# matthiasverstraete/3d_recognizer

Measured on AMD Instinct MI355X. Metric: training clouds/sec, N=40960 pts, bs=8, at 1/2/4/8 GPUs; mIoU parity, higher is better.
Workload: dtype f32 storage/accumulate, bf16x3 MFMA in the wide GEMMs

## Files before the change

### 3d_recognizer_amd/csrc/gemm.hip

```cpp
#include "rl_common.h"
#include <stdlib.h>
#include <string.h>

namespace {

typedef float f32x4 __attribute__((ext_vector_type(4)));

constexpr int GM_BM = 128;
constexpr int GM_BK = 16;
constexpr int GM_AS = 20;

struct AOperand {
    const float* A;
    long lda, a_bstride;
    int a_mode;
    RlLazy lazy;
    const float* xyz;
    long xyz_bstride;
    const int32_t* nbr_idx;
    const float* nbr_d2;
    int nbr_k;
    int n;
    int K;
    long M;
// ... 25 lines not shown
                const int j = a.nbr_idx[R];
                const float* xb = a.xyz + (long)b * a.xyz_bstride * 3;
                const float xi = xb[(long)i * 3 + 0], yi = xb[(long)i * 3 + 1], zi = xb[(long)i * 3 + 2];
                const float xj = xb[(long)j * 3 + 0], yj = xb[(long)j * 3 + 1], zj = xb[(long)j * 3 + 2];
                v[0] = xi; v[1] = yi; v[2] = zi;
                v[3] = xj; v[4] = yj; v[5] = zj;
                v[6] = xi - xj; v[7] = yi - yj; v[8] = zi - zj;
                v[9] = __fsqrt_rn(a.nbr_d2[R]);
            }
            float* dst = As + r * stride;
#pragma unroll
            for (int c = 0; c < 10; ++c) dst[c] = v[c];
            for (int c = 10; c < kw; ++c) dst[c] = 0.f;
        }
        return;
    }
    if (a.vec4) {
        const int qpr = kw >> 2;
        for (int e = tid; e < nrows * qpr; e += 256) {
            const int r = e / qpr, q = e - r * qpr;
            const long R = row0 + r;
            const int kc = k0 + q * 4;
            float4 v = make_float4(0.f, 0.f, 0.f, 0.f);
            if (R < row_limit && kc < a.K) {
                v = *reinterpret_cast<const float4*>(a.A + a_row_offset(a, R) + kc);
                if (a.lazy.scale) {
                    v.x = rl_lazy(a.lazy, v.x, kc + 0);
                    v.y = rl_lazy(a.lazy, v.y, kc + 1);
                    v.z = rl_lazy(a.lazy, v.z, kc + 2);
                    v.w = rl_lazy(a.lazy, v.w, kc + 3);
                }
            }
            *reinterpret_cast<float4*>(As + r * stride + q * 4) = v;
        }
        return;
    }
    for (int e = tid; e < nrows * kw; e += 256) {
        const int r = e / kw, c = e - r * kw;
        const long R = row0 + r;
        const int kc = k0 + c;
        float v = 0.f;
        if (R < row_limit && kc < a.K) v = rl_lazy(a.lazy, a.A[a_row_offset(a, R) + kc], kc);
        As[r * stride + c] = v;
    }
}

struct ConcatSrc {
    const float* A2;
    const int32_t* idx;
    const float* sc2; const float* sh2;
    long a2_bstride;
    int lda2, split, act2;
    float slope2;
};

struct GemmParams {
    AOperand a;
    int N;
    const float* W;
    long w_ks, w_ns;
    const float* bias;
    float* Y;
    long ldy, y_bstride;
    int rows_per_batch;
    int y_contig;
    int accumulate;
    double* stats;
    const float* piv_mean;
    const float* piv_bias;
    int ksplit;
    int kchunk;
    float* kslab;
    int stat_slots;
    int gx, ny;
    const float* addend;
    float* out2;
    const int32_t* out2_index;
    long out2_bstride;
    int split_col;
    const __bf16* wsplit;
    const float* bnb_Y;
    const float* bnb_scale;
    const float* bnb_shift;
    const float* bnb_mean;
    const float* bnb_invstd;
    float bnb_neg;
    int pair_ny1;
    int N2;
    float* Y2;
    double* stats2;
    const float* piv_mean2;
    const float* piv_bias2;
    const __bf16* wsplit2;
};

__device__ __forceinline__ float stat_pivot(const GemmParams& p, int c) {
    if (!p.stats || !p.piv_mean || c >= p.N) return 0.f;
    return p.piv_mean[c] - (p.piv_bias ? p.piv_bias[c] : 0.f);
}

template <int NT>
__global__ __launch_bounds__(256) void gemm_kernel(const GemmParams p) {
    constexpr int BN = 16 * NT;
    constexpr int WS = BN + ((BN % 32 == 0) ? 16 : 0);
    __shared__ __attribute__((aligned(16))) float As[GM_BM * GM_AS];
    __shared__ float Ws[GM_BK * WS];
// ... 254 lines not shown

void wgrad_split(long M, int N, int K, int* nsplit, long* rows_per_block) {
    const int T = wgrad_tile(N, K);
    const int ny = rl_cdiv(N, T), nz = rl_cdiv(K, T);
    long want = 1024 / ((long)ny * nz);
    if (want < 1) want = 1;
    long maxs = (M + 255) / 256;
    const long fill = 256 / ((long)ny * nz) + 1;
    if (maxs < fill) maxs = fill < (M + 63) / 64 ? fill : (M + 63) / 64;
    if (maxs < 1) maxs = 1;
    if (want > maxs) want = maxs;
    if (T == 128) {
        const long round = 512 / ((long)ny * nz);
        if (round >= 1 && want > round) want = round;
    }
    constexpr long share = 2;
    if (T == 128) { want /= share; if (want < 1) want = 1; }
    long rpb = (M + want - 1) / want;
    rpb = ((rpb + 63) / 64) * 64;
    *rows_per_block = rpb;
    *nsplit = (int)((M + rpb - 1) / rpb);
    if (*nsplit < 1) *nsplit = 1;
}

int fill_a(AOperand* a, const char* who, const float* A, long lda, long a_bstride, int a_mode,
           int in_act, float in_slope, const float* in_scale, const float* in_shift,
           const float* xyz, long xyz_bstride, const int32_t* nbr_idx, const float* nbr_d2, int nbr_k,
           int B, int n, int K) {
    RL_REQUIRE(B > 0 && n > 0 && K > 0, RL_ERR_ARGS, "%s: bad sizes B=%d n=%d K=%d", who, B, n, K);
    a->A = A; a->lda = lda; a->a_bstride = a_bstride; a->a_mode = a_mode;
    a->lazy.scale = in_scale; a->lazy.shift = in_shift; a->lazy.act = in_act; a->lazy.slope = in_slope;
    a->xyz = xyz; a->xyz_bstride = xyz_bstride; a->nbr_idx = nbr_idx; a->nbr_d2 = nbr_d2; a->nbr_k = nbr_k;
    a->n = n; a->K = K;
    if (a_mode == 1) {
        RL_REQUIRE(K == 10, RL_ERR_ARGS, "%s: relative position encoding source needs K == 10 (got %d)", who, K);
        RL_REQUIRE(xyz && nbr_idx && nbr_d2 && nbr_k > 0 && xyz_bstride >= n, RL_ERR_ARGS, "%s: incomplete RPE source", who);
        a->M = (long)B * n * nbr_k;
        a->contig = 1; a->vec4 = 0; a->vec4p = 0;
    } else {
        RL_REQUIRE(a_mode == 0, RL_ERR_ARGS, "%s: unknown a_mode %d", who, a_mode);
        RL_REQUIRE(A && lda >= K && a_bstride >= n, RL_ERR_ARGS, "%s: bad A operand", who);
        RL_REQUIRE((in_scale == nullptr) == (in_shift == nullptr), RL_ERR_ARGS, "%s: in_scale/in_shift must come together", who);
        a->M = (long)B * n;
        a->contig = (a_bstride == n);
        a->vec4 = (lda % 4 == 0) && (K % 4 == 0) && (((uintptr_t)A & 15) == 0);
        a->vec4p = (lda % 4 == 0) && ((K + 3) / 4 * 4 <= lda) && (((uintptr_t)A & 15) == 0);
    }
    RL_REQUIRE(a->M < (1l << 31), RL_ERR_ARGS, "%s: too many rows", who);
    return RL_OK;
}



template <int KC, int NT, bool BNB = false>
__global__ __launch_bounds__(256) void sgemm_kernel(const GemmParams p) {
    __shared__ double red[4][2][16 * NT];
    const int tid = threadIdx.x, lane = tid & 63, wave = __builtin_amdgcn_readfirstlane(tid >> 6);
    const int li = lane & 15, lj = lane >> 4;
    const int K = p.a.K, N = p.N;
    const long M = p.a.M;

    float wf[KC][4][NT];
    float sc[KC][4], sh[KC][4];
#pragma unroll
    for (int c = 0; c < KC; ++c)
#pragma unroll
        for (int s = 0; s < 4; ++s) {
            const int k = 16 * c + 4 * lj + s;
            sc[c][s] = (p.a.lazy.scale && k < K) ? p.a.lazy.scale[k] : 1.f;
            sh[c][s] = (p.a.lazy.scale && k < K) ? p.a.lazy.shift[k] : 0.f;
#pragma unroll
            for (int nb = 0; nb < NT; ++nb) {
                const int n = nb * 16 + li;
                wf[c][s][nb] = (k < K && n < N) ? p.W[(long)k * p.w_ks + (long)n * p.w_ns] : 0.f;
            }
        }
    float bias[NT], ssum[NT], ssq[NT], piv[NT];
    float bsc[BNB ? NT : 1], bsh[BNB ? NT : 1], bmu[BNB ? NT : 1], bis[BNB ? NT : 1];
#pragma unroll
    for (int nb = 0; nb < NT; ++nb) {
        const int n = nb * 16 + li;
        bias[nb] = (p.bias && n < N) ? p.bias[n] : 0.f;
        ssum[nb] = ssq[nb] = 0.f;
        piv[nb] = BNB ? 0.f : stat_pivot(p, n);
        if constexpr (BNB) {
            bsc[nb] = n < N ? p.bnb_scale[n] : 1.f; bsh[nb] = n < N ? p.bnb_shift[n] : 0.f;
            bmu[nb] = n < N ? p.bnb_mean[n] : 0.f;  bis[nb] = n < N ? p.bnb_invstd[n] : 0.f;
        }
    }
    const bool lazy = p.a.lazy.scale != nullptr;
    const float es = (!lazy || p.a.lazy.act == RL_ACT_NONE) ? 1.f : (p.a.lazy.act == RL_ACT_RELU ? 0.f : p.a.lazy.slope);
    const bool full = N == 16 * NT;

    const long nblk = (M + 15) >> 4;
    const long bstep = (long)gridDim.x * 4;
    auto fetch = [&](long blk, float4 (&a)[KC]) {
        const long row = blk * 16 + li;
        const bool rvalid = row < M;
        const long aoff = rvalid ? a_row_offset(p.a, row) : 0;
#pragma unroll
        for (int c = 0; c < KC; ++c) {
            a[c] = make_float4(0.f, 0.f, 0.f, 0.f);
            if (rvalid && 16 * c + 4 * lj < K) a[c] = *reinterpret_cast<const float4*>(p.a.A + aoff + 16 * c + 4 * lj);
        }
    };
    float4 a[KC], an[KC];
    long blk = (long)blockIdx.x * 4 + wave;
    if (blk < nblk) fetch(blk, a);
    for (; blk < nblk; blk += bstep) {
        const bool rvalid = blk * 16 + li < M;
        if (blk + bstep < nblk) fetch(blk + bstep, an);
        f32x4 acc[NT];
#pragma unroll
        for (int nb = 0; nb < NT; ++nb) acc[nb] = (f32x4){0.f, 0.f, 0.f, 0.f};
#pragma unroll
        for (int c = 0; c < KC; ++c) {
            float av[4] = {a[c].x, a[c].y, a[c].z, a[c].w};
#pragma unroll
            for (int s = 0; s < 4; ++s) {
                float v = av[s];
                if (lazy) {
                    const float z = v * sc[c][s] + sh[c][s];
                    v = fmaxf(z, z * es);
                }
                if (!rvalid || 16 * c + 4 * lj + s >= K) v = 0.f;
#pragma unroll
                for (int nb = 0; nb < NT; ++nb)
                    acc[nb] = __builtin_amdgcn_mfma_f32_16x16x4f32(v, wf[c][s][nb], acc[nb], 0, 0, 0);
            }
        }
        asm volatile("" ::: "memory");
        __builtin_amdgcn_s_waitcnt(0x0F70);
        asm volatile("" ::: "memory");
#pragma unroll
        for (int r = 0; r < 4; ++r) {
            const long R = blk * 16 + lj * 4 + r;
            if (R < M) {
                long yoff;
                if (p.y_contig) yoff = R * p.ldy;
                else {
                    const int b = (int)((unsigned)R / (unsigned)p.rows_per_batch);
                    const int i = (int)(R - (long)b * p.rows_per_batch);
                    yoff = ((long)b * p.y_bstride + i) * p.ldy;
                }
                float* y = p.Y + yoff + li;
                float v[NT];
#pragma unroll
                for (int nb = 0; nb < NT; ++nb) v[nb] = acc[nb][r] + bias[nb];
                if (p.accumulate) {
                    float o[NT];
#pragma unroll
                    for (int nb = 0; nb < NT; ++nb) o[nb] = (full || nb * 16 + li < N) ? y[nb * 16] : 0.f;
#pragma unroll
                    for (int nb = 0; nb < NT; ++nb) v[nb] += o[nb];
                }
                if constexpr (BNB) {
                    const float* yl = p.bnb_Y + yoff + li;
                    float t[NT];
#pragma unroll
                    for (int nb = 0; nb < NT; ++nb) t[nb] = (full || nb * 16 + li < N) ? yl[nb * 16] : 0.f;
#pragma unroll
                    for (int nb = 0; nb < NT; ++nb) {
                        if (full || nb * 16 + li < N) {
                            y[nb * 16] = v[nb];
                            const float z = t[nb] * bsc[nb] + bsh[nb];
                            const float gp = v[nb] * (z > 0.f ? 1.f : p.bnb_neg);
                            ssum[nb] += gp;
                            ssq[nb] += gp * ((t[nb] - bmu[nb]) * bis[nb]);
                        }
                    }
                } else {
#pragma unroll
                for (int nb = 0; nb < NT; ++nb) {
                    if (full || nb * 16 + li < N) {
                        y[nb * 16] = v[nb];
                        const float dv = v[nb] - piv[nb];
                        ssum[nb] += dv;
                        ssq[nb] += dv * dv;
                    }
                }
                }
            }
        }
#pragma unroll
        for (int c = 0; c < KC; ++c) a[c] = an[c];
    }
    if (p.stats) {
#pragma unroll
        for (int nb = 0; nb < NT; ++nb) {
            float s = ssum[nb], q = ssq[nb];
            s += __shfl_xor(s, 16, 64); s += __shfl_xor(s, 32, 64);
            q += __shfl_xor(q, 16, 64); q += __shfl_xor(q, 32, 64);
            if (lane < 16) {
                red[wave][0][nb * 16 + lane] = (double)s;
                red[wave][1][nb * 16 + lane] = (double)q;
            }
        }
        __syncthreads();
        if (tid < 16 * NT && tid < N) {
            p.stats[((long)blockIdx.x * 2 + 0) * N + tid] = red[0][0][tid] + red[1][0][tid] + red[2][0][tid] + red[3][0][tid];
            p.stats[((long)blockIdx.x * 2 + 1) * N + tid] = red[0][1][tid] + red[1][1][tid] + red[2][1][tid] + red[3][1][tid];
            for (long slot = blockIdx.x + gridDim.x; slot < p.stat_slots; slot += gridDim.x) {
                p.stats[(slot * 2 + 0) * N + tid] = 0.0;
                p.stats[(slot * 2 + 1) * N + tid] = 0.0;
            }
        }
    }
}

constexpr int SW_U = 4;

template <int KT, int NT>
__device__ __forceinline__ void swgrad_body(const WgradParams& p, const int bx, float* red) {
    const int tid = threadIdx.x, lane = tid & 63, wave = __builtin_amdgcn_readfirstlane(tid >> 6);
    const int lc = lane & 15, lr = lane >> 4;
    const int N = p.N, K = p.a.K;
    const AOperand& a = p.a;
    const long r_begin = (long)bx * p.rows_per_block;
    const long r_end = min(a.M, r_begin + p.rows_per_block);

    float sc[KT], sh[KT];
#pragma unroll
    for (int kb = 0; kb < KT; ++kb) {
        const int k = kb * 16 + lc;
        sc[kb] = (a.lazy.scale && k < K) ? a.lazy.scale[k] : 1.f;
        sh[kb] = (a.lazy.scale && k < K) ? a.lazy.shift[k] : 0.f;
    }
    const bool lazy = a.lazy.scale != nullptr;
    const float es = (!lazy || a.lazy.act == RL_ACT_NONE) ? 1.f : (a.lazy.act == RL_ACT_RELU ? 0.f : a.lazy.slope);
    f32x4 acc[NT][KT];
    float bsum[NT];
#pragma unroll
    for (int nb = 0; nb < NT; ++nb) {
        bsum[nb] = 0.f;
#pragma unroll
        for (int kb = 0; kb < KT; ++kb) acc[nb][kb] = (f32x4){0.f, 0.f, 0.f, 0.f};
    }

    auto fetch = [&](long base, float (&dy)[SW_U][NT], float (&av)[SW_U][KT]) {
#pragma unroll
        for (int u = 0; u < SW_U; ++u) {
            const long R = base + u * 4 + lr;
            const bool valid = R < r_end;
            long doff = 0;
            if (valid) {
                if (p.dy_contig) doff = R * p.lddy;
                else {
                    const int b = (int)((unsigned)R / (unsigned)p.rows_per_batch);
                    const int i = (int)(R - (long)b * p.rows_per_batch);
                    doff = ((long)b * p.dy_bstride + i) * p.lddy;
                }
            }
#pragma unroll
            for (int nb = 0; nb < NT; ++nb) {
                const int n = nb * 16 + lc;
                dy[u][nb] = (valid && n < N) ? p.dY[doff + n] : 0.f;
            }
            if (a.a_mode == 1) {
                float v = 0.f;
                if (valid && lc < 10) {
                    if (lc == 9) v = __fsqrt_rn(a.nbr_d2[R]);
                    else {
                        const long pt = (unsigned)R / (unsigned)a.nbr_k;
                        const int b = (int)((unsigned)pt / (unsigned)a.n);
                        const int i = (int)(pt - (long)b * a.n);
                        const int ax = lc % 3;
                        const float* xb = a.xyz + (long)b * a.xyz_bstride * 3;
                        const float xi = xb[(long)i * 3 + ax];
                        if (lc < 3) v = xi;
                        else {
                            const float xj = xb[(long)a.nbr_idx[R] * 3 + ax];
                            v = lc < 6 ? xj : xi - xj;
                        }
                    }
                }
                av[u][0] = v;
#pragma unroll
                for (int kb = 1; kb < KT; ++kb) av[u][kb] = 0.f;
            } else {
                const long aoff = valid ? a_row_offset(a, R) : 0;
#pragma unroll
                for (int kb = 0; kb < KT; ++kb) {
                    const int k = kb * 16 + lc;
                    av[u][kb] = (valid && k < K) ? a.A[aoff + k] : 0.f;
                }
            }
        }
    };
    auto consume = [&](long base, float (&dy)[SW_U][NT], float (&av)[SW_U][KT]) {
        if (a.a_mode != 1 && lazy) {
#pragma unroll
            for (int u = 0; u < SW_U; ++u) {
                const bool valid = base + u * 4 + lr < r_end;
#pragma unroll
                for (int kb = 0; kb < KT; ++kb)
                    if (valid && kb * 16 + lc < K) {
                        const float z = av[u][kb] * sc[kb] + sh[kb];
                        av[u][kb] = fmaxf(z, z * es);
                    }
            }
        }
#pragma unroll
        for (int u = 0; u < SW_U; ++u)
#pragma unroll
            for (int nb = 0; nb < NT; ++nb) {
                bsum[nb] += dy[u][nb];
#pragma unroll
                for (int kb = 0; kb < KT; ++kb)
                    acc[nb][kb] = __builtin_amdgcn_mfma_f32_16x16x4f32(dy[u][nb], av[u][kb], acc[nb][kb], 0, 0, 0);
            }
    };
    {
        float dy0[SW_U][NT], av0[SW_U][KT], dy1[SW_U][NT], av1[SW_U][KT];
        long base = r_begin + (long)wave * 4 * SW_U;
        if (base < r_end) fetch(base, dy0, av0);
        while (base < r_end) {
            const long nb1 = base + 16 * SW_U;
            if (nb1 < r_end) fetch(nb1, dy1, av1);
            consume(base, dy0, av0);
            if (nb1 >= r_end) break;
            const long nb2 = nb1 + 16 * SW_U;
            if (nb2 < r_end) fetch(nb2, dy0, av0);
            consume(nb1, dy1, av1);
            base = nb2;
        }
    }
#pragma unroll
    for (int nb = 0; nb < NT; ++nb) {
        bsum[nb] += __shfl_xor(bsum[nb], 16, 64);
        bsum[nb] += __shfl_xor(bsum[nb], 32, 64);
    }
    float* rb = red + KT * NT * 4 * 64;
    for (int w = 1; w < 4; ++w) {
        __syncthreads();
        if (wave == w) {
#pragma unroll
            for (int nb = 0; nb < NT; ++nb) {
#pragma unroll
                for (int kb = 0; kb < KT; ++kb)
#pragma unroll
                    for (int r = 0; r < 4; ++r) red[((nb * KT + kb) * 4 + r) * 64 + lane] = acc[nb][kb][r];
                rb[nb * 64 + lane] = bsum[nb];
            }
        }
        __syncthreads();
        if (wave == 0) {
#pragma unroll
            for (int nb = 0; nb < NT; ++nb) {
#pragma unroll
                for (int kb = 0; kb < KT; ++kb)
#pragma unroll
                    for (int r = 0; r < 4; ++r) acc[nb][kb][r] += red[((nb * KT + kb) * 4 + r) * 64 + lane];
                bsum[nb] += rb[nb * 64 + lane];
            }
        }
    }
    if (wave == 0) {
        float* out = p.slab + (long)bx * ((long)N * K + N);
#pragma unroll
        for (int nb = 0; nb < NT; ++nb) {
#pragma unroll
            for (int kb = 0; kb < KT; ++kb) {
                const int k = kb * 16 + lc;
#pragma unroll
                for (int r = 0; r < 4; ++r) {
                    const int n = nb * 16 + lr * 4 + r;
                    if (n < N && k < K) out[(long)n * K + k] = acc[nb][kb][r];
                }
            }
            const int n = nb * 16 + lc;
            if (p.has_bias && lr == 0 && n < N) out[(long)N * K + n] = bsum[nb];
        }
    }
}

template <int KT, int NT>
__global__ __launch_bounds__(256) void swgrad_kernel(const WgradParams p) {
    __shared__ float red[KT * NT * 4 * 64 + NT * 64];
    swgrad_body<KT, NT>(p, (int)blockIdx.x, red);
}

void swgrad_split(long M, int* nsplit, long* rows_per_block) {
    constexpr long rows_wg = 256;
    long want = (M + rows_wg - 1) / rows_wg;
    const long fill = (M + 127) / 128 < 256 ? (M + 127) / 128 : 256;
    if (want < fill) want = fill;
    if (want < 1) want = 1;
    if (want > 1024) want = 1024;
    long rpb = (M + want - 1) / want;
    rpb = ((rpb + 63) / 64) * 64;
    *rows_per_block = rpb;
    *nsplit = (int)((M + rpb - 1) / rpb);
    if (*nsplit < 1) *nsplit = 1;
}

inline bool stream_ok(int N, int K) { return (N <= 64 && K <= 64) || (K <= 16 && N <= 128); }

constexpr int swgrad_body_index(int KT, int NT) { return 4 * (KT >= 4 ? 2 : KT - 1) + (NT >= 8 ? 3 : NT >= 4 ? 2 : NT - 1); }

constexpr int PG_BK = 32;
constexpr int PG_AS = 36;

typedef __attribute__((ext_vector_type(8))) __bf16 bf16x8;
typedef __attribute__((ext_vector_type(4))) __bf16 bf16x4;

template <int NT, bool STATS>
__device__ __forceinline__ void tile_rows_epilogue(const GemmParams& p, const f32x4 (&acc)[NT], long Rb, int col0, int lr, int lq,
                                                   float (&ssum)[NT], float (&ssq)[NT]) {
    constexpr int BN = 16 * NT;
    const int N = p.N;
    const long M = p.a.M;
    const bool to_y = !p.out2 || col0 + BN <= p.split_col;
    const bool to_out2 = p.out2 && !p.out2_index && col0 >= p.split_col;
    if (to_y || to_out2) {
        const bool full = col0 + BN <= N;
        const bool has_bias = p.bias != nullptr;
        const bool accumulate = to_y && p.accumulate;
        float bv[NT];
#pragma unroll
        for (int nb = 0; nb < NT; ++nb) {
            const int c = col0 + nb * 16 + lr;
            bv[nb] = (has_bias && c < N) ? p.bias[c] : 0.f;
        }
        float pv[STATS ? NT : 1];
        if constexpr (STATS) {
#pragma unroll
            for (int nb = 0; nb < NT; ++nb) pv[nb] = stat_pivot(p, col0 + nb * 16 + lr);
        }
#pragma unroll
        for (int r = 0; r < 4; ++r) {
            const long R = Rb + lq * 4 + r;
            if (R < M) {
// ... 701 lines not shown
    else { if (PER == 8) asm volatile("s_waitcnt vmcnt(32)" ::: "memory"); else if (PER == 4) asm volatile("s_waitcnt vmcnt(16)" ::: "memory"); else asm volatile("s_waitcnt vmcnt(8)" ::: "memory"); }
}
__device__ __forceinline__ void raw_barrier() {
    __builtin_amdgcn_s_barrier();
    asm volatile("" ::: "memory");
}

#ifndef W2_ABLATE
#define W2_ABLATE 0
#endif
constexpr int W2_KMAX = 1024;
constexpr int W2_THREADS = 768;
template <int TERMS, bool STATS, int AS, int WS, int BM, int BN, bool CAT>
__device__ __forceinline__ void wgemm2_body(const GemmParams& pk, const ConcatSrc& cs) {
    static_assert(AS >= 3 && AS <= 6 && WS >= 2 && WS <= 6, "ring depths vs the wait table");
    static_assert((BM == 128 || BM == 64) && (BN == 128 || BN == 64), "tile shapes");
    constexpr int RB = BM / 16;
    constexpr int CG = 8 / RB;
    constexpr int NT = BN / 16 / CG;
    constexpr bool TR = !STATS;
    constexpr int A_STAGE = BM * 128;
    constexpr int W_PLANE = BN * 64;
    constexpr int W_STAGE = 2 * W_PLANE;
    constexpr int OFF_W = AS * A_STAGE, OFF_SC = OFF_W + WS * W_STAGE, OFF_RED = OFF_SC + 2 * W2_KMAX * 4;
    constexpr int TOTAL = OFF_RED + (STATS ? 8 * 2 * BN * 8 : 0);
    __shared__ __attribute__((aligned(1024))) unsigned char lds[TOTAL];
    const int tid = threadIdx.x, lane = tid & 63, wave = __builtin_amdgcn_readfirstlane(tid >> 6);
    int bx = blockIdx.x, by = 0;
    if (pk.ny > 1) {
        const int xcd = blockIdx.x & 7, s = blockIdx.x >> 3;
        by = s % pk.ny;
        bx = (s / pk.ny) * 8 + xcd;
        if (bx >= pk.gx) return;
    }
    GemmParams p = pk;
    if (pk.pair_ny1 > 0 && by >= pk.pair_ny1) {
        by -= pk.pair_ny1;
        p.N = pk.N2; p.Y = pk.Y2; p.ldy = pk.N2; p.stats = pk.stats2;
        p.piv_mean = pk.piv_mean2; p.piv_bias = pk.piv_bias2; p.wsplit = pk.wsplit2;
        p.split_col = pk.N2;
    }
    const int col0 = by * BN;
    const int K = p.a.K, N = p.N;
    const long M = p.a.M;
    const long ntiles = (M + BM - 1) / BM;
    constexpr bool cat = CAT;
    const bool lazy = cat || p.a.lazy.scale != nullptr;
    float* lsc = reinterpret_cast<float*>(lds + OFF_SC);
    float* lsh = lsc + W2_KMAX;
    double* red = reinterpret_cast<double*>(lds + OFF_RED);
    const unsigned lds0 = lds_address(lds);
    if (cat) {
        for (int k = tid; k < K; k += W2_THREADS) {
            const bool two = k >= cs.split;
            const int c = two ? k - cs.split : k;
            const float* scp = two ? cs.sc2 : p.a.lazy.scale;
            const float* shp = two ? cs.sh2 : p.a.lazy.shift;
            lsc[k] = scp ? scp[c] : 1.f;
            lsh[k] = scp ? shp[c] : 0.f;
        }
    } else if (lazy) {
        for (int k = tid; k < K; k += W2_THREADS) {
            lsc[k] = p.a.lazy.scale[k];
            lsh[k] = p.a.lazy.shift[k];
        }
    }
    if constexpr (STATS) {
        for (int i = tid; i < 8 * 2 * BN; i += W2_THREADS) red[i] = 0.0;
    }
    __syncthreads();

    const int k_begin = (p.ksplit > 1) ? blockIdx.z * p.kchunk : 0;
    const int k_end = (p.ksplit > 1) ? min(K, k_begin + p.kchunk) : K;
    const int nch = (k_end - k_begin) / PG_BK;
    const bool vec_t = (N % 4 == 0) && (p.ldy % 4 == 0) && (p.split_col % 4 == 0) &&
                       (((reinterpret_cast<uintptr_t>(p.Y) | reinterpret_cast<uintptr_t>(p.out2) | reinterpret_cast<uintptr_t>(p.addend) |
                          reinterpret_cast<uintptr_t>(p.bias) | reinterpret_cast<uintptr_t>(p.kslab)) & 15) == 0);
    const int my_tiles = bx < ntiles ? (int)((ntiles - 1 - bx) / p.gx) + 1 : 0;
    const int T = my_tiles * nch;

    if (wave >= 8) __builtin_amdgcn_s_setprio(3);
    if (wave >= 10) {
        constexpr int PPP = BN / 16;
        constexpr int WI = (TERMS == 3 ? 2 : 1) * PPP / 2;
        const int lw = wave - 10;
        const __bf16* wsrc[WI];
        unsigned wdst[WI];
#pragma unroll
        for (int j = 0; j < WI; ++j) {
            const int idx = lw * WI + j, plane = idx / PPP, rg = idx % PPP;
            int col = col0 + rg * 16 + (lane >> 2);
            col = col < N ? col : N - 1;
            wsrc[j] = p.wsplit + (long)plane * N * K + (long)col * K + (lane & 3) * 8 + k_begin;
            wdst[j] = lds0 + OFF_W + plane * W_PLANE + rg * 1024;
        }
        auto issue_w = [&](int q) {
            const int k = (q % nch) * PG_BK;
            const unsigned o = __builtin_amdgcn_readfirstlane((q % WS) * W_STAGE);
            if constexpr (WI % 4 == 0) {
#pragma unroll
                for (int j = 0; j < WI; j += 4)
                    glds16x4(wsrc[j] + k, wsrc[j + 1] + k, wsrc[j + 2] + k, wsrc[j + 3] + k, wdst[j] + o, wdst[j + 1] + o, wdst[j + 2] + o,
                             wdst[j + 3] + o);
            } else {
                glds16x2(wsrc[0] + k, wsrc[1] + k, wdst[0] + o, wdst[1] + o);
            }
        };
        for (int q = 0; q < WS - 1 && q < T; ++q) issue_w(q);
        for (int q = 0; q < T; ++q) {
            wait_vm_chunks<WI>(min(WS - 2, T - 1 - q));
            raw_barrier();
            if (q + WS - 1 < T) issue_w(q + WS - 1);
        }
    } else if (wave >= 8) {
        constexpr int AI = BM / 16;
        const int lw = wave - 8;
        const float* asrc[AI];
        const float* asrc2[AI];
        int nidx[AI];
        auto group_row = [&](int j, int i) {
            long Rg = ((long)bx + (long)j * p.gx) * BM + (lw * AI + i) * 8;
            return Rg < M ? Rg : M - 8;
        };
        auto fetch_idx = [&](int j) {
            const int sub = lane >> 3;
            rl_i32x8 g[AI];
#pragma unroll
            for (int i = 0; i < AI; ++i) g[i] = *(const rl_const_i32x8*)((const rl_const_byte*)cs.idx + group_row(j, i) * 4);
#pragma unroll
            for (int i = 0; i < AI; ++i) {
                int gi = g[i][0];
                gi = sub == 1 ? g[i][1] : gi; gi = sub == 2 ? g[i][2] : gi; gi = sub == 3 ? g[i][3] : gi; gi = sub == 4 ? g[i][4] : gi;
                gi = sub == 5 ? g[i][5] : gi; gi = sub == 6 ? g[i][6] : gi; gi = sub == 7 ? g[i][7] : gi;
                nidx[i] = gi;
            }
        };
        auto tile_sources = [&](int j) {
            const long row0 = ((long)bx + (long)j * p.gx) * BM;
#pragma unroll
            for (int i = 0; i < AI; ++i) {
                const int r = (lw * AI + i) * 8 + (lane >> 3);
                const int seg = ((lane & 7) ^ ((r >> 1) & 7)) << 2;
                long R = row0 + r;
                R = R < M ? R : M - 1;
                const long Rg = group_row(j, i);
                if (cat) R = Rg + (lane >> 3);
                asrc[i] = p.a.A + a_row_offset(p.a, R) + seg + k_begin;
                const unsigned b = cat ? (unsigned)Rg / (unsigned)p.a.n : 0u;
                asrc2[i] = cat ? cs.A2 + ((long)b * cs.a2_bstride + nidx[i]) * cs.lda2 + seg - cs.split : asrc[i];
            }
        };
        int iq = 0, ic = 0;
        auto issue_a = [&]() {
            if (ic == 0) tile_sources(iq / nch);
            const int k = ic * PG_BK;
            const unsigned l = __builtin_amdgcn_readfirstlane(lds0 + (iq % AS) * A_STAGE + lw * AI * 1024);
            const bool two = cat && k >= cs.split;
            const float* s[AI];
#pragma unroll
            for (int i = 0; i < AI; ++i) s[i] = (two ? asrc2[i] : asrc[i]) + k;
            glds16x4(s[0], s[1], s[2], s[3], l, l + 1024, l + 2048, l + 3072);
            if constexpr (AI == 8) glds16x4(s[4], s[5], s[6], s[7], l + 4096, l + 5120, l + 6144, l + 7168);
            if (cat && ic == 0 && iq / nch + 1 < my_tiles) fetch_idx(iq / nch + 1);
            ++iq;
            ic = ic + 1 == nch ? 0 : ic + 1;
        };
#pragma unroll
        for (int i = 0; i < AI; ++i) nidx[i] = 0;
        if (cat && T > 0) fetch_idx(0);
        while (iq < AS - 1 && iq < T) issue_a();
        for (int q = 0; q < T; ++q) {
            wait_vm_chunks<AI>(min(AS - 2, T - 1 - q));
            raw_barrier();
            if (iq < T) issue_a();
        }
    } else {
        const int lr = lane & 15, lq = lane >> 4;
        const bool relu = p.a.lazy.act == RL_ACT_RELU;
        const float nslope = p.a.lazy.act == RL_ACT_NONE ? 1.f : p.a.lazy.slope;
        float e_one = 1.f, e_two = 1.f;
        if (cat) {
            RlLazy t2 = p.a.lazy;
            t2.scale = cs.sc2; t2.shift = cs.sh2; t2.act = cs.act2; t2.slope = cs.slope2;
            e_one = rl_eff_slope(p.a.lazy);
            e_two = rl_eff_slope(t2);
        }
        const int rb = wave % RB, cg = wave / RB;
        const int cg0 = cg * NT * 16;
        const int frow = rb * 16 + lr;
        const int fsw = (frow >> 1) & 7;
        const int a_frag0 = frow * 128 + (((2 * lq) ^ fsw) << 4), a_frag1 = frow * 128 + (((2 * lq + 1) ^ fsw) << 4);
        const int w_frag = lr * 64 + lq * 16 + cg0 * 64;
        auto actf = [&](float z) {
            const float neg = relu ? 0.f : z * nslope;
            return z > 0.f ? z : neg;
        };
        f32x4 acc[NT];
#pragma unroll
        for (int nb = 0; nb < NT; ++nb) acc[nb] = (f32x4){0.f, 0.f, 0.f, 0.f};
        int c = 0;
        long tile = bx;
        for (int q = 0; q < T; ++q) {
            raw_barrier();
            const unsigned char* Ab = lds + (q % AS) * A_STAGE;
            const unsigned char* Wb = lds + OFF_W + (q % WS) * W_STAGE;
            float4 v0 = *reinterpret_cast<const float4*>(Ab + a_frag0);
            float4 v1 = *reinterpret_cast<const float4*>(Ab + a_frag1);
            if (cat) {
                const int kk = c * PG_BK + lq * 8;
                const float e = c * PG_BK >= cs.split ? e_two : e_one;
                const f32x4 x0 = rl_fold_act4((f32x4){v0.x, v0.y, v0.z, v0.w}, *reinterpret_cast<const f32x4*>(lsc + kk),
                                              *reinterpret_cast<const f32x4*>(lsh + kk), e);
                const f32x4 x1 = rl_fold_act4((f32x4){v1.x, v1.y, v1.z, v1.w}, *reinterpret_cast<const f32x4*>(lsc + kk + 4),
                                              *reinterpret_cast<const f32x4*>(lsh + kk + 4), e);
                v0 = make_float4(x0[0], x0[1], x0[2], x0[3]);
                v1 = make_float4(x1[0], x1[1], x1[2], x1[3]);
            } else if (lazy) {
                const int kk = k_begin + c * PG_BK + lq * 8;
                const float4 sc0 = *reinterpret_cast<const float4*>(lsc + kk), sc1 = *reinterpret_cast<const float4*>(lsc + kk + 4);
                const float4 sh0 = *reinterpret_cast<const float4*>(lsh + kk), sh1 = *reinterpret_cast<const float4*>(lsh + kk + 4);
                v0.x = actf(v0.x * sc0.x + sh0.x); v0.y = actf(v0.y * sc0.y + sh0.y);
                v0.z = actf(v0.z * sc0.z + sh0.z); v0.w = actf(v0.w * sc0.w + sh0.w);
                v1.x = actf(v1.x * sc1.x + sh1.x); v1.y = actf(v1.y * sc1.y + sh1.y);
                v1.z = actf(v1.z * sc1.z + sh1.z); v1.w = actf(v1.w * sc1.w + sh1.w);
            }
            bf16x4 h0, l0, h1, l1;
            split_bf16(v0, h0, l0);
            split_bf16(v1, h1, l1);
            const bf16x8 a_h = __builtin_shufflevector(h0, h1, 0, 1, 2, 3, 4, 5, 6, 7);
            const bf16x8 a_l = __builtin_shufflevector(l0, l1, 0, 1, 2, 3, 4, 5, 6, 7);
            bf16x8 b_h[NT], b_l[NT];
#pragma unroll
            for (int nb = 0; nb < NT; ++nb) {
#if W2_ABLATE == 1
                const int nbs = nb & 1;
#else
                const int nbs = nb;
#endif
// ... 524 lines not shown
            }
        }
    }
    float* out = p.slab + (long)blockIdx.x * ((long)N * K + N);
#pragma unroll
    for (int i = 0; i < 2; ++i) {
#pragma unroll
        for (int kb = 0; kb < 8; ++kb) {
            const int k = k0 + kb * 16 + lr;
#pragma unroll
            for (int r = 0; r < 4; ++r) {
                const int n = n0 + (2 * wave + i) * 16 + lq * 4 + r;
                if (n < N && k < K) out[(long)n * K + k] = acc[i][kb][r];
            }
        }
    }
    if (p.has_bias && blockIdx.z == 0 && tid < nvalid) out[(long)N * K + n0 + tid] = bsum;
}

typedef __attribute__((ext_vector_type(4))) short s16x4g;
template <int TERMS, bool RB = false>
__device__ __forceinline__ void pwgrad128w_body(const WgradParams& p, const int bx, const int by, const int bz) {
    constexpr int RP = 144;
    constexpr int NSPL = TERMS == 3 ? 2 : 1;
    __shared__ __attribute__((aligned(16))) __bf16 lds_d[PW2_RB * RP * NSPL];
    __shared__ __attribute__((aligned(16))) __bf16 lds_a[PW2_RB * RP * NSPL];
    __bf16* Dh = lds_d;
    __bf16* Dl = Dh + PW2_RB * RP;
    __bf16* Xh = lds_a;
    __bf16* Xl = Xh + PW2_RB * RP;
    __shared__ __attribute__((aligned(16))) float lz[3][PW2_T];
    const int tid = threadIdx.x, lane = tid & 63, wave = tid >> 6;
    const int lr = lane & 15, lq = lane >> 4;
    const int N = p.N, K = p.a.K;
    const int n0 = by * PW2_T, k0 = bz * PW2_T;
    const bool cat = !RB && p.cat.split > 0;
    const int nvalid = min(PW2_T, N - n0), kvalid = min(PW2_T, K - k0);
    const long r_begin = (long)bx * p.rows_per_block;
    const long r_end = min(p.a.M, r_begin + p.rows_per_block);
    const bool lazy = p.a.lazy.scale != nullptr;
    const bool relu = p.a.lazy.act == RL_ACT_RELU;
    const float nslope = p.a.lazy.act == RL_ACT_NONE ? 1.f : p.a.lazy.slope;
    auto actf = [&](float z) {
        const float neg = relu ? 0.f : z * nslope;
        return z > 0.f ? z : neg;
    };
    int ucol[2], urow[2];
#pragma unroll
    for (int i = 0; i < 2; ++i) {
        const int u = i * 8 + wave;
        ucol[i] = (u & 7) * 16 + (lane & 3) * 4;
        urow[i] = (u >> 3) * 16 + (lane >> 2);
    }
    const bool gat = cat && k0 + ucol[0] >= p.cat.split;
    if (tid < PW2_T) {
        if (cat) {
            const bool two = k0 + tid >= p.cat.split;
            const int c = two ? k0 + tid - p.cat.split : k0 + tid;
            const float* scp = two ? p.cat.sc2 : p.a.lazy.scale;
            const float* shp = two ? p.cat.sh2 : p.a.lazy.shift;
            RlLazy t = p.a.lazy;
            if (two) { t.scale = p.cat.sc2; t.shift = p.cat.sh2; t.act = p.cat.act2; t.slope = p.cat.slope2; }
            const bool in = scp != nullptr && tid < kvalid;
            lz[0][tid] = in ? scp[c] : 1.f;
            lz[1][tid] = in ? shp[c] : 0.f;
            lz[2][tid] = rl_eff_slope(t);
        } else {
            const bool in = lazy && tid < kvalid;
            lz[0][tid] = in ? p.a.lazy.scale[k0 + tid] : 1.f;
            lz[1][tid] = in ? p.a.lazy.shift[k0 + tid] : 0.f;
            lz[2][tid] = 1.f;
        }
    }
    const int nh = wave >> 2, kw = wave & 3;
    f32x4 acc[4][2];
#pragma unroll
    for (int nb = 0; nb < 4; ++nb)
#pragma unroll
        for (int kb = 0; kb < 2; ++kb) acc[nb][kb] = (f32x4){0.f, 0.f, 0.f, 0.f};
    const bool want_bias = p.has_bias && bz == 0;
    f32x4 bs = {0.f, 0.f, 0.f, 0.f};
    float4 rd[2], ra[2];
    int gi[2] = {0, 0};
    auto fetch_idx = [&](long r0) {
#pragma unroll
        for (int i = 0; i < 2; ++i) {
            const unsigned R = (unsigned)min(r0 + urow[i], r_end - 1);
            gi[i] = *reinterpret_cast<const int32_t*>(reinterpret_cast<const char*>(p.cat.idx) + R * 4u);
        }
    };
    int cb = 0, cend = 0;
    if (cat) {
        cb = (int)((unsigned)r_begin / (unsigned)p.a.n);
        cend = (cb + 1) * p.a.n;
    }

    auto fetch = [&](long r0) {
        if (cat) while ((int)r0 >= cend) { ++cb; cend += p.a.n; }
#pragma unroll
        for (int i = 0; i < 2; ++i) {
            const long R = r0 + urow[i];
            rd[i] = make_float4(0.f, 0.f, 0.f, 0.f);
            ra[i] = make_float4(0.f, 0.f, 0.f, 0.f);
            if (R < r_end) {
                if (ucol[i] < nvalid) {
                    long off;
                    if (p.dy_contig) off = R * p.lddy;
                    else {
                        const int b = (int)((unsigned)R / (unsigned)p.rows_per_batch);
                        const int ii = (int)(R - (long)b * p.rows_per_batch);
                        off = ((long)b * p.dy_bstride + ii) * p.lddy;
                    }
                    rd[i] = rl_ldx4<RB>(p.dY, off + n0 + ucol[i]);
                }
                if (ucol[i] < kvalid) {
                    if (gat) {
                        int b = cb;
                        for (int e = cend; (int)R >= e; e += p.a.n) ++b;
                        const unsigned off = ((unsigned)b * (unsigned)p.cat.a2_bstride + (unsigned)gi[i]) * (unsigned)p.cat.lda2 +
                                             (unsigned)(k0 + ucol[i] - p.cat.split);
                        ra[i] = *reinterpret_cast<const float4*>(p.cat.A2 + off);
                    } else ra[i] = rl_ldx4<RB>(p.a.A, a_row_offset(p.a, R) + k0 + ucol[i]);
                }
            }
        }
        if (gat) fetch_idx(r0 + PW2_RB);
    };
    auto commit = [&](long r0) {
#pragma unroll
        for (int i = 0; i < 2; ++i) {
            float4 v = ra[i];
            if (cat) {
                if (r0 + urow[i] < r_end && ucol[i] < kvalid) {
                    const f32x4 x = rl_fold_act4((f32x4){v.x, v.y, v.z, v.w}, *reinterpret_cast<const f32x4*>(&lz[0][ucol[i]]),
                                                 *reinterpret_cast<const f32x4*>(&lz[1][ucol[i]]), lz[2][ucol[i]]);
                    v = make_float4(x[0], x[1], x[2], x[3]);
                }
            } else if (lazy && r0 + urow[i] < r_end && ucol[i] < kvalid) {
                const float4 sc = *reinterpret_cast<const float4*>(&lz[0][ucol[i]]);
                const float4 sh = *reinterpret_cast<const float4*>(&lz[1][ucol[i]]);
                v.x = actf(v.x * sc.x + sh.x);
                v.y = actf(v.y * sc.y + sh.y);
                v.z = actf(v.z * sc.z + sh.z);
                v.w = actf(v.w * sc.w + sh.w);
            }
            bf16x4 dh, dl, xh, xl;
            if (want_bias) bs += (f32x4){rd[i].x, rd[i].y, rd[i].z, rd[i].w};
            split_bf16(rd[i], dh, dl);
            split_bf16(v, xh, xl);
            const int o = urow[i] * RP + ucol[i];
            *reinterpret_cast<bf16x4*>(Dh + o) = dh;
            *reinterpret_cast<bf16x4*>(Xh + o) = xh;
            if constexpr (TERMS == 3) {
                *reinterpret_cast<bf16x4*>(Dl + o) = dl;
                *reinterpret_cast<bf16x4*>(Xl + o) = xl;
            }
        }
    };

    const int tr_off = (lq * 8 + (lr >> 2)) * RP + 4 * (lr & 3);
    const __bf16* dh_frag = Dh + tr_off + nh * 64;
    const __bf16* xh_frag = Xh + tr_off + kw * 32;
    constexpr int LO = PW2_RB * RP;
    auto frag = [&](const __bf16* q) {
        const bf16x4 r0 = __builtin_bit_cast(bf16x4, __builtin_amdgcn_ds_read_tr16_b64_v4i16((__attribute__((address_space(3))) s16x4g*)q));
        const bf16x4 r1 = __builtin_bit_cast(bf16x4, __builtin_amdgcn_ds_read_tr16_b64_v4i16((__attribute__((address_space(3))) s16x4g*)(q + 4 * RP)));
        return __builtin_shufflevector(r0, r1, 0, 1, 2, 3, 4, 5, 6, 7);
    };
    if (gat && r_begin < r_end) fetch_idx(r_begin);
    if (r_begin < r_end) fetch(r_begin);
    for (long r0 = r_begin; r0 < r_end; r0 += PW2_RB) {
        __syncthreads();
        commit(r0);
        __syncthreads();
        if (r0 + PW2_RB < r_end) fetch(r0 + PW2_RB);
// ... 13 lines not shown
                acc[nb][kb] = __builtin_amdgcn_mfma_f32_16x16x32_bf16(a_h, b_h[kb], acc[nb][kb], 0, 0, 0);
            if constexpr (TERMS == 3) {
#pragma unroll
                for (int kb = 0; kb < 2; ++kb)
                    acc[nb][kb] = __builtin_amdgcn_mfma_f32_16x16x32_bf16(a_h, b_l[kb], acc[nb][kb], 0, 0, 0);
#pragma unroll
                for (int kb = 0; kb < 2; ++kb)
                    acc[nb][kb] = __builtin_amdgcn_mfma_f32_16x16x32_bf16(a_l, b_h[kb], acc[nb][kb], 0, 0, 0);
            }
        }
    }
    float* out = p.slab + (long)bx * ((long)N * K + N);
#pragma unroll
    for (int nb = 0; nb < 4; ++nb) {
#pragma unroll
        for (int kb = 0; kb < 2; ++kb) {
            const int k = k0 + kw * 32 + kb * 16 + lr;
#pragma unroll
            for (int r = 0; r < 4; ++r) {
                const int n = n0 + nh * 64 + nb * 16 + lq * 4 + r;
                if (n < N && k < K) out[(long)n * K + k] = acc[nb][kb][r];
            }
        }
    }
    if (want_bias) {
#pragma unroll
        for (int o = 4; o < 64; o <<= 1)
#pragma unroll
            for (int j = 0; j < 4; ++j) bs[j] += __shfl_xor(bs[j], o, 64);
        if (lane < 4 && ucol[0] < nvalid) {
#pragma unroll
            for (int j = 0; j < 4; ++j) out[(long)N * K + n0 + ucol[0] + j] = bs[j];
        }
    }
}

template <int TERMS, bool RB = false>
__global__ __launch_bounds__(512, 4) void pwgrad128w_kernel(const WgradParams p) {
    pwgrad128w_body<TERMS, RB>(p, blockIdx.x, blockIdx.y, blockIdx.z);
}

struct WBItem {
    const float* A; const float* dY; const float* sc; const float* sh; float* slab;
    long lda, a_bstride, lddy, dy_bstride, rows_per_block, M;
    int N, K, n, rows_per_batch, act;
    float slope;
    int first_block;
    int nsplit;
    unsigned short gy, gz;
    unsigned char a_contig, dy_contig, has_bias;
    unsigned char cat;
};
constexpr int WB_MAX = 24;
constexpr int WB_CAT_MAX = 4;
struct WgradBatch {
    WBItem item[WB_MAX];
    ConcatSrc cat[WB_CAT_MAX];
    int count, pad;
};
static_assert(sizeof(WgradBatch) <= 4096, "the grouped launch carries its layer table in the kernel arguments (4 KB)");
template <int TERMS>
__global__ __launch_bounds__(512, 4) void pwgrad128w_batch_kernel(const WgradBatch b) {
    int i = 0;
    while (i + 1 < b.count && (int)blockIdx.x >= b.item[i + 1].first_block) ++i;
    const WBItem& it = b.item[i];
    const int local = (int)blockIdx.x - it.first_block;
    const int per = (int)it.gy * (int)it.gz;
    int bx, t = 0;
    if (per > 1) {
        const int grp = local / (8 * per), rem = local - grp * 8 * per;
        t = rem >> 3;
        bx = grp * 8 + (rem & 7);
    } else bx = local;
    if (bx >= it.nsplit) return;
    const int by = t / (int)it.gz, bz = t - by * (int)it.gz;
    WgradParams p;
    p.a.A = it.A; p.a.lda = it.lda; p.a.a_bstride = it.a_bstride; p.a.a_mode = 0;
    p.a.lazy.scale = it.sc; p.a.lazy.shift = it.sh; p.a.lazy.act = it.act; p.a.lazy.slope = it.slope;
    p.a.xyz = nullptr; p.a.xyz_bstride = 0; p.a.nbr_idx = nullptr; p.a.nbr_d2 = nullptr; p.a.nbr_k = 0;
    p.a.n = it.n; p.a.K = it.K; p.a.M = it.M; p.a.contig = it.a_contig; p.a.vec4 = 1; p.a.vec4p = 1;
    p.N = it.N; p.dY = it.dY; p.lddy = it.lddy; p.dy_bstride = it.dy_bstride; p.rows_per_batch = it.rows_per_batch;
    p.dy_contig = it.dy_contig; p.slab = it.slab; p.rows_per_block = it.rows_per_block; p.has_bias = it.has_bias;
    p.cat = ConcatSrc{};
    if (it.cat) p.cat = b.cat[it.cat - 1];
    pwgrad128w_body<TERMS, false>(p, bx, by, bz);
}

__global__ __launch_bounds__(256) void swgrad_batch_kernel(const WgradBatch b) {
    __shared__ float red[4 * 4 * 4 * 64 + 8 * 64];
    int i = 0;
    while (i + 1 < b.count && (int)blockIdx.x >= b.item[i + 1].first_block) ++i;
    const WBItem& it = b.item[i];
    WgradParams p;
    p.a.A = it.A; p.a.lda = it.lda; p.a.a_bstride = it.a_bstride; p.a.a_mode = 0;
    p.a.lazy.scale = it.sc; p.a.lazy.shift = it.sh; p.a.lazy.act = it.act; p.a.lazy.slope = it.slope;
    p.a.xyz = nullptr; p.a.xyz_bstride = 0; p.a.nbr_idx = nullptr; p.a.nbr_d2 = nullptr; p.a.nbr_k = 0;
    p.a.n = it.n; p.a.K = it.K; p.a.M = it.M; p.a.contig = it.a_contig; p.a.vec4 = 0; p.a.vec4p = 0;
    p.N = it.N; p.dY = it.dY; p.lddy = it.lddy; p.dy_bstride = it.dy_bstride; p.rows_per_batch = it.rows_per_batch;
    p.dy_contig = it.dy_contig; p.slab = it.slab; p.rows_per_block = it.rows_per_block; p.has_bias = it.has_bias;
    p.cat = ConcatSrc{};
    const int bx = (int)blockIdx.x - it.first_block;
    if (bx >= it.nsplit) return;
    switch (it.gy) {
        case swgrad_body_index(1, 1): swgrad_body<1, 1>(p, bx, red); break;
        case swgrad_body_index(1, 2): swgrad_body<1, 2>(p, bx, red); break;
        case swgrad_body_index(1, 4): swgrad_body<1, 4>(p, bx, red); break;
        case swgrad_body_index(1, 8): swgrad_body<1, 8>(p, bx, red); break;
        case swgrad_body_index(2, 1): swgrad_body<2, 1>(p, bx, red); break;
        case swgrad_body_index(2, 2): swgrad_body<2, 2>(p, bx, red); break;
        case swgrad_body_index(2, 4): swgrad_body<2, 4>(p, bx, red); break;
        case swgrad_body_index(4, 1): swgrad_body<4, 1>(p, bx, red); break;
        case swgrad_body_index(4, 2): swgrad_body<4, 2>(p, bx, red); break;
        default: swgrad_body<4, 4>(p, bx, red); break;
    }
}

inline bool pwgrad_ok(const WgradParams& p) {
    if (p.a.a_mode != 0 || !p.a.vec4) return false;
    if ((p.N % 4) || (p.lddy % 4) || (((uintptr_t)p.dY) & 15)) return false;
    if (p.a.lazy.scale && ((((uintptr_t)p.a.lazy.scale) | ((uintptr_t)p.a.lazy.shift)) & 15)) return false;
    return true;
}


typedef void (*GemmFn)(const GemmParams);
typedef void (*GemmCatFn)(const GemmParams, const ConcatSrc);
typedef void (*WgradFn)(const WgradParams);
enum GemmKernel { GK_NONE, GK_SGEMM, GK_PGEMM, GK_WGEMM, GK_WGEMM2, GK_GEMM };

struct GemmFacts {
    long M; int N, K;
    bool streamable;
    bool pgemm, wgemm, wgemm2;
    bool split, stats, bnb;
    int64_t kslab_floats;
    int cat_split;
    int rows_per_cloud;
};

struct GemmPlan {
    GemmKernel kernel;
    GemmFn fn;
    GemmCatFn catfn;
    int threads; dim3 grid;
    WidePlan wide;
    int gx, ny, ksplit, kchunk;
    GemmFn reduce;
    dim3 reduce_grid;
    const char* name;
    const char* refusal;
};

template <int KC, bool BNB>
GemmFn sgemm_fn(int N) {
    if constexpr (KC == 1 && !BNB) if (N > 64) return sgemm_kernel<1, 8>;
    return N <= 16 ? sgemm_kernel<KC, 1, BNB> : N <= 32 ? sgemm_kernel<KC, 2, BNB> : sgemm_kernel<KC, 4, BNB>;
}
template <int NT>
GemmFn pgemm_fn(int terms) { return terms == 0 ? pgemm_kernel<NT, 0> : terms == 1 ? pgemm_kernel<NT, 1> : pgemm_kernel<NT, 3>; }
template <int TERMS, bool STATS>
GemmFn wide_inst(bool dma, WidePlan w) {
    if (!dma) return wgemm_kernel<TERMS, STATS>;
    return w.bm == 128 ? wgemm2_kernel<TERMS, STATS, W2_AS, W2_WS, 128, 128>
         : w.bn == 128 ? wgemm2_kernel<TERMS, STATS, W2_AS, W2_WS, 64, 128> : wgemm2_kernel<TERMS, STATS, W2_AS, W2_WS, 64, 64>;
}
template <int TERMS, bool STATS>
GemmCatFn wide_cat_inst(WidePlan w) {
    return w.bm == 128 ? wgemm2_cat_kernel<TERMS, STATS, W2_AS, W2_WS, 128, 128>
         : w.bn == 128 ? wgemm2_cat_kernel<TERMS, STATS, W2_AS, W2_WS, 64, 128> : wgemm2_cat_kernel<TERMS, STATS, W2_AS, W2_WS, 64, 64>;
}
inline GemmCatFn wide_cat_fn(bool stats, WidePlan w) {
    if (wide_gemm_terms() == 1) return stats ? wide_cat_inst<1, true>(w) : wide_cat_inst<1, false>(w);
    return stats ? wide_cat_inst<3, true>(w) : wide_cat_inst<3, false>(w);
}
inline GemmFn wide_fn(bool stats, bool dma, WidePlan w) {
    if (wide_gemm_terms() == 1) return stats ? wide_inst<1, true>(dma, w) : wide_inst<1, false>(dma, w);
    return stats ? wide_inst<3, true>(dma, w) : wide_inst<3, false>(dma, w);
}

inline dim3 xcd_grid(int gx, int ny, int z) { return dim3(ny > 1 ? (unsigned)(8 * rl_cdiv(gx, 8) * ny) : (unsigned)gx, 1, z); }

inline void persistent_grid(GemmPlan& pl, long M, int ny, int z) {
    int cap = cu_count() / ny / 8 * 8;
    if (cap < 8) cap = 8;
    pl.gx = rl_cdiv(M, pl.wide.bm);
    if (pl.gx > cap) pl.gx = cap;
    pl.ny = ny;
    pl.grid = xcd_grid(pl.gx, ny, z);
}

inline void plan_wide(GemmPlan& pl, const GemmFacts& f, int z, bool splitk) {
    const bool dma = f.wgemm2;
    pl.fn = wide_fn(f.stats && pl.ksplit <= 1, dma, pl.wide);
    pl.kernel = dma ? GK_WGEMM2 : GK_WGEMM;
    pl.threads = dma ? W2_THREADS : 512;
    if (dma) persistent_grid(pl, f.M, rl_cdiv(f.N, pl.wide.bn), z);
    else     pl.grid = xcd_grid(pl.gx, pl.ny, z);
    pl.name = dma ? (splitk ? "wgemm2_kernel+splitk" : "wgemm2_kernel") : (splitk ? "wgemm_kernel+splitk" : "wgemm_kernel");
}

GemmPlan plan_gemm(const GemmFacts& f);
GemmPlan plan_gemm_concat(GemmFacts f) {
    const int split = f.cat_split, n = f.rows_per_cloud;
    f.cat_split = 0;
    f.streamable = true;
    GemmPlan pl = plan_gemm(f);
    if (pl.kernel == GK_NONE) return pl;
    if (!(pl.kernel == GK_WGEMM2 && pl.ksplit == 1 && pl.wide.ksplit == 1 && !pl.reduce && f.K == 2 * split && split % PG_BK == 0 &&
          f.K <= W2_KMAX && n % 16 == 0 && f.M % 16 == 0)) {
        pl.kernel = GK_NONE;
        pl.fn = nullptr;
        pl.refusal = "rl_gemm: a concat-gather A operand (a2_split) needs the LDS-DMA wide kernel in one pass (bf16x3 / bf16 arithmetic, "
                     "pre-split weight, dma staging, no K split), fp32 rows, K == 2 * a2_split <= 1024, a2_split % 32 == 0 and rows per "
                     "cloud a multiple of 16";
        return pl;
    }
    pl.catfn = wide_cat_fn(f.stats, pl.wide);
    pl.name = "wgemm2_kernel<cat>";
    return pl;
}

GemmPlan plan_gemm(const GemmFacts& f) {
    if (f.cat_split != 0) return plan_gemm_concat(f);
    const int N = f.N, K = f.K, nt = N <= 16 ? 1 : N <= 32 ? 2 : N <= 64 ? 4 : 8;
    GemmPlan pl{};
    pl.threads = 256; pl.ksplit = 1;
    pl.gx = rl_row_blocks_host(f.M, GM_BM);
    pl.ny = N > 64 ? rl_cdiv(N, 128) : 1;
    if (f.split && K <= 64 && N <= 64) { pl.refusal = "rl_gemm: split-scatter epilogue needs K or N > 64"; return pl; }
    if (f.split && !f.pgemm) { pl.refusal = "rl_gemm: split-scatter epilogue needs the LDS-tiled kernel (aligned operands, K % 4 == 0)"; return pl; }
    const bool streams = !f.split && f.streamable && stream_ok(N, K);
    if (!f.split && f.bnb && !(streams && N <= 64)) {
        pl.refusal = "rl_gemm: the BatchNorm-backward sums are a by-product of the streaming kernel only (K, N <= 64; ask rl_gemm_streams)";
        return pl;
    }
    if (streams) {
        int sg = pl.gx;
        if ((long)K * N >= 2048) sg = sg > 512 ? 512 : (sg > 256 ? 256 : sg);
        if (g_sgemm_grid_div > 1) sg = sg / g_sgemm_grid_div > 0 ? sg / g_sgemm_grid_div : 1;
        if (f.bnb) pl.fn = K <= 16 ? sgemm_fn<1, true>(N) : K <= 32 ? sgemm_fn<2, true>(N) : sgemm_fn<4, true>(N);
        else       pl.fn = K <= 16 ? sgemm_fn<1, false>(N) : K <= 32 ? sgemm_fn<2, false>(N) : sgemm_fn<4, false>(N);
        pl.kernel = GK_SGEMM;
        pl.grid = dim3(sg);
        pl.name = "sgemm_kernel";
        return pl;
    }
    if (f.pgemm) pl.wide = wide_plan(f.M, N, K, N > 64 && f.wgemm && f.wgemm2);
    const int terms = wide_gemm_terms();
    if (!f.split && f.pgemm && N > 64 && pl.wide.ksplit > 1 && f.kslab_floats >= (int64_t)pl.wide.ksplit * f.M * N) {
        pl.kchunk = ((K + pl.wide.ksplit - 1) / pl.wide.ksplit + 31) / 32 * 32;
        pl.ksplit = (K + pl.kchunk - 1) / pl.kchunk;
        const bool cb64 = (long)pl.gx * rl_cdiv(N, 64) >= 256;
        pl.reduce = cb64 ? gemm_splitk_reduce_kernel<64> : gemm_splitk_reduce_kernel<16>;
        pl.reduce_grid = dim3(pl.gx, rl_cdiv(N, cb64 ? 64 : 16));
        if (f.wgemm) {
            plan_wide(pl, f, pl.ksplit, true);
        } else {
            pl.kernel = GK_PGEMM;
            pl.fn = pgemm_fn<8>(terms);
            pl.grid = xcd_grid(pl.gx, pl.ny, pl.ksplit);
            pl.name = "pgemm_kernel<8>+splitk";
        }
    } else if (!f.split && f.pgemm && N > 16 && N <= 64 && wgemm_small_tiles() && f.wgemm && f.wgemm2) {
        pl.wide = WidePlan{64, 64, 1};
        plan_wide(pl, f, 1, false);
    } else if (!f.pgemm) {
        pl.kernel = GK_GEMM;
        pl.fn = nt == 1 ? gemm_kernel<1> : nt == 2 ? gemm_kernel<2> : nt == 4 ? gemm_kernel<4> : gemm_kernel<8>;
        pl.grid = dim3(pl.gx, pl.ny);
        pl.name = "gemm_kernel";
    } else if (N > 64 && f.wgemm) {
        plan_wide(pl, f, 1, false);
    } else {
        pl.kernel = GK_PGEMM;
        pl.fn = nt == 1 ? pgemm_fn<1>(terms) : nt == 2 ? pgemm_fn<2>(terms) : nt == 4 ? pgemm_fn<4>(terms) : pgemm_fn<8>(terms);
        pl.grid = xcd_grid(pl.gx, pl.ny, 1);
        pl.name = N > 64 ? "pgemm_kernel<8>" : f.split ? "pgemm_kernel" : nt == 1 ? "pgemm_kernel<1>" : nt == 2 ? "pgemm_kernel<2>" : "pgemm_kernel<4>";
    }
    return pl;
}

inline GemmFacts aligned_facts(long M, int N, int K, bool dma) {
    return GemmFacts{M, N, K, true, true, wide_gemm_terms() != 0 && K % 8 == 0,
                     dma && wgemm_staging() == 1 && K % PG_BK == 0 && K <= W2_KMAX, false, true, false, 0, 0, 0};
}

int launch_gemm(const GemmPlan& pl, hipStream_t st, GemmParams p, const char* who, const ConcatSrc* cat = nullptr) {
    p.gx = pl.gx; p.ny = pl.ny; p.ksplit = pl.ksplit; p.kchunk = pl.kchunk;
    if (pl.catfn && cat) hipLaunchKernelGGL(pl.catfn, pl.grid, dim3(pl.threads), 0, st, p, *cat);
    else hipLaunchKernelGGL(pl.fn, pl.grid, dim3(pl.threads), 0, st, p);
    rl_note_kernel(pl.name);
    RL_LAUNCH_CHECK(who);
    if (!pl.reduce) return RL_OK;
    hipLaunchKernelGGL(pl.reduce, pl.reduce_grid, dim3(256), 0, st, p);
    RL_LAUNCH_CHECK("rl_gemm(split-K reduce)");
    return RL_OK;
}

struct WgradPlan {
    WgradFn fn;
    int threads; dim3 grid;
    int nsplit; long rows_per_block;
    int batch;
    int body;
    const char* name;
    const char* refusal;
};

template <int KT>
WgradFn swgrad_fn(int N) {
    if constexpr (KT == 1) if (N > 64) return swgrad_kernel<1, 8>;
    return N <= 16 ? swgrad_kernel<KT, 1> : N <= 32 ? swgrad_kernel<KT, 2> : swgrad_kernel<KT, 4>;
}

WgradPlan plan_wgrad(long M, int N, int K, int a_mode, bool pwgrad, bool rows_bf16, int cat_split = 0) {
    if (cat_split != 0) {
        WgradPlan pl = plan_wgrad(M, N, K, a_mode, pwgrad, rows_bf16);
        const bool w = pl.fn == (WgradFn)pwgrad128w_kernel<1> || pl.fn == (WgradFn)pwgrad128w_kernel<3>;
        if (!(w && !rows_bf16 && K == 2 * cat_split && cat_split % 16 == 0)) {
            pl.fn = nullptr;
            pl.batch = 0;
            pl.refusal = "rl_wgrad: a concat-gather A operand (a2_split) needs the wide (128 x 128 tile) kernel outside the fp32 "
                         "arithmetic mode, fp32 rows, K == 2 * a2_split and a2_split % 16 == 0";
        }
        return pl;
    }
    WgradPlan pl{};
    pl.threads = 256;
    const int terms = wide_gemm_terms();
    if (stream_ok(N, K)) {
        swgrad_split(M, &pl.nsplit, &pl.rows_per_block);
        if (!rows_bf16) pl.fn = K <= 16 ? swgrad_fn<1>(N) : K <= 32 ? swgrad_fn<2>(N) : swgrad_fn<4>(N);
        pl.refusal = "rl_wgrad: bf16 rows are supported by the wide weight-gradient kernel only";
        pl.grid = dim3(pl.nsplit);
        pl.batch = a_mode == 0 && !rows_bf16 ? 2 : 0;
        pl.body = swgrad_body_index(K <= 16 ? 1 : K <= 32 ? 2 : 4, N <= 16 ? 1 : N <= 32 ? 2 : N <= 64 ? 4 : 8);
        pl.name = "swgrad_kernel";
        return pl;
    }
    wgrad_split(M, N, K, &pl.nsplit, &pl.rows_per_block);
    const int T = pwgrad ? wgrad_tile(N, K) : WG_T;
    const bool wide = pwgrad && T == 128;
    pl.grid = dim3(pl.nsplit, rl_cdiv(N, T), rl_cdiv(K, T));
    if (rows_bf16)  pl.fn = wide && terms != 0 ? pwgrad128w_kernel<1, true> : nullptr;
    else if (wide)  pl.fn = terms == 0 ? pwgrad128_kernel : terms == 1 ? pwgrad128w_kernel<1> : pwgrad128w_kernel<3>;
    else            pl.fn = pwgrad ? pwgrad_kernel : wgrad_kernel;
    pl.threads = wide && terms != 0 ? 512 : 256;
    pl.refusal = "rl_wgrad: bf16 rows are supported by the wide (128 x 128 tile) weight-gradient kernel only";
    pl.batch = !rows_bf16 && wide && terms != 0 && rl_cdiv(N, 128) < 65536 && rl_cdiv(K, 128) < 65536 ? 1 : 0;
    pl.name = wide ? (terms != 0 ? "pwgrad128w_kernel" : "pwgrad128_kernel") : pwgrad ? "pwgrad_kernel" : "wgrad_kernel";
    return pl;
}

void launch_wgrad_batch(int batch, long blocks, hipStream_t st, const WgradBatch& b) {
    if (batch == 2)                   hipLaunchKernelGGL(swgrad_batch_kernel, dim3((unsigned)blocks), dim3(256), 0, st, b);
    else if (wide_gemm_terms() == 1)  hipLaunchKernelGGL(pwgrad128w_batch_kernel<1>, dim3((unsigned)blocks), dim3(512), 0, st, b);
    else                              hipLaunchKernelGGL(pwgrad128w_batch_kernel<3>, dim3((unsigned)blocks), dim3(512), 0, st, b);
}

}

int rl_wide_terms() { return wide_gemm_terms(); }

extern "C" int rl_set_wide_gemm(const char* mode) {
    const int t = parse_wide(mode);
    RL_REQUIRE(mode != nullptr && t >= 0, RL_ERR_ARGS, "rl_set_wide_gemm: mode must be \"fp32\", \"bf16x3\" or \"bf16\"");
    g_wide_terms = t;
    return RL_OK;
}
extern "C" int rl_set_wgemm_staging(const char* how) {
    RL_REQUIRE(how != nullptr && (!strcmp(how, "registers") || !strcmp(how, "dma")), RL_ERR_ARGS,
               "rl_set_wgemm_staging: \"registers\" or \"dma\"");
    g_wgemm_staging = !strcmp(how, "dma");
    return RL_OK;
}
extern "C" int rl_set_wgemm_tile(const char* how) {
    RL_REQUIRE(how && (!strcmp(how, "auto") || !strcmp(how, "128") || !strcmp(how, "64x128") || !strcmp(how, "64x64")), RL_ERR_ARGS,
               "rl_set_wgemm_tile: expected auto | 128 | 64x128 | 64x64");
    g_wgemm_force = !strcmp(how, "64x128") ? 1 : !strcmp(how, "64x64") ? 2 : 0;
    g_wgemm_small = strcmp(how, "128") ? 1 : 0;
    return RL_OK;
}
extern "C" int rl_set_gemm_ksplit(int enable) {
    g_gemm_no_ksplit = enable ? 0 : 1;
    return RL_OK;
}
extern "C" int rl_set_sgemm_grid_div(int div) {
    RL_REQUIRE(div >= 1 && div <= 64, RL_ERR_ARGS, "rl_set_sgemm_grid_div: 1 .. 64");
    g_sgemm_grid_div = div;
    return RL_OK;
}
extern "C" const char* rl_get_wide_gemm(void) {
    const int t = wide_gemm_terms();
    return t == 0 ? "fp32" : t == 1 ? "bf16" : "bf16x3";
}

static int gemm_fill(const rl_gemm_desc* d, GemmParams* pp, GemmPlan* plan, ConcatSrc* cs) {
    RL_REQUIRE(d != nullptr, RL_ERR_ARGS, "rl_gemm: null descriptor");
    GemmParams& p = *pp;
    p = GemmParams{};
    *cs = ConcatSrc{};
    const int cat = d->a2_split;
    RL_REQUIRE(cat == 0 || (cat > 0 && cat < d->K && d->a_mode == 0), RL_ERR_ARGS,
               "rl_gemm: a2_split must lie inside (0, K), on a tensor operand");
    int rc = fill_a(&p.a, "rl_gemm", d->A, d->lda, d->a_bstride, d->a_mode, d->in_act, d->in_slope,
                    d->in_scale, d->in_shift, d->xyz, d->xyz_bstride, d->nbr_idx, d->nbr_d2, d->nbr_k,
                    d->B, d->n, cat ? cat : d->K);
    if (rc) return rc;
    p.a.K = d->K;
    if (cat) {
        RL_REQUIRE(d->A2 && d->a2_idx && d->a2_bstride > 0 && (d->a2_scale == nullptr) == (d->a2_shift == nullptr), RL_ERR_ARGS,
                   "rl_gemm: incomplete second source (A2, a2_idx, a2_bstride; a2_scale / a2_shift come together)");
        RL_REQUIRE((((uintptr_t)d->A2) & 15) == 0 && d->lda2 % 4 == 0 && d->lda2 >= d->K - cat && d->lda2 < (1l << 31) &&
                   (((uintptr_t)d->a2_idx) & 3) == 0, RL_ERR_ARGS,
                   "rl_gemm: A2 must be 16-byte aligned with lda2 a multiple of 4 and >= K - a2_split");
        cs->A2 = d->A2; cs->idx = d->a2_idx; cs->sc2 = d->a2_scale; cs->sh2 = d->a2_shift;
        cs->a2_bstride = d->a2_bstride; cs->lda2 = (int)d->lda2; cs->split = cat; cs->act2 = d->a2_act; cs->slope2 = d->a2_slope;
    }
    RL_REQUIRE(d->N > 0 && d->W && d->Y && d->ldy > 0, RL_ERR_ARGS, "rl_gemm: bad W/Y");
    p.N = d->N; p.W = d->W; p.w_ks = d->w_ks; p.w_ns = d->w_ns; p.bias = d->bias;
    p.Y = d->Y; p.ldy = d->ldy; p.y_bstride = d->y_bstride;
    p.rows_per_batch = (d->a_mode == 1) ? d->n * d->nbr_k : d->n;
    RL_REQUIRE(d->y_bstride >= p.rows_per_batch, RL_ERR_ARGS, "rl_gemm: y_bstride smaller than rows per cloud");
    p.y_contig = (d->y_bstride == p.rows_per_batch);
    p.accumulate = d->accumulate; p.stats = d->stats;
    p.piv_mean = d->stats ? d->stats_pivot_mean : nullptr; p.piv_bias = d->stats ? d->stats_pivot_bias : nullptr;
    p.addend = d->addend; p.out2 = d->out2; p.out2_index = d->out2_index; p.out2_bstride = d->out2_bstride;
    RL_REQUIRE(!d->out2_index || rl_float_atomics_allowed(), RL_ERR_UNSUPPORTED,
               "rl_gemm: out2_index scatters with fp32 atomics (order-dependent); the deterministic path is a dense out2 + "
               "rl_segment_sum_rows (set RL_ALLOW_FLOAT_ATOMICS=1 to use it anyway)");
    p.split_col = d->out2 ? d->split_col : d->N;
    p.wsplit = reinterpret_cast<const __bf16*>(d->W_split);
    const bool split = d->addend != nullptr || d->out2 != nullptr;
    if (split) {
        RL_REQUIRE(!d->out2 || (d->split_col > 0 && d->split_col < d->N && (!d->out2_index || d->out2_bstride > 0)), RL_ERR_ARGS,
                   "rl_gemm: bad split-scatter fields");
        RL_REQUIRE(d->ldy >= (d->out2 ? d->split_col : d->N), RL_ERR_ARGS, "rl_gemm: ldy smaller than the columns stored to Y");
        RL_REQUIRE(d->stats == nullptr, RL_ERR_UNSUPPORTED, "rl_gemm: split-scatter epilogue has no statistics");
    } else {
        RL_REQUIRE(d->ldy >= d->N, RL_ERR_ARGS, "rl_gemm: bad W/Y");
    }
    p.stat_slots = (int)rl_gemm_stat_slots(p.a.M, d->N, d->K);
    const GemmPlan pl = plan_gemm(GemmFacts{p.a.M, d->N, d->K, p.a.a_mode == 0 && p.a.vec4p, pgemm_ok(p), wgemm_ok(p), wgemm2_usable(p),
                                            split, d->stats != nullptr, d->bnb_Y != nullptr, d->kslab ? d->kslab_floats : 0, cat, d->n});
    RL_REQUIRE(pl.kernel != GK_NONE, RL_ERR_UNSUPPORTED, "%s", pl.refusal);
    if (!split && d->bnb_Y) {
        RL_REQUIRE(d->stats && d->bnb_scale && d->bnb_shift && d->bnb_mean && d->bnb_invstd && !d->stats_pivot_mean, RL_ERR_ARGS,
                   "rl_gemm: bnb_Y needs stats, the layer's scale / shift / mean / invstd and no pivot");
        p.bnb_Y = d->bnb_Y; p.bnb_scale = d->bnb_scale; p.bnb_shift = d->bnb_shift; p.bnb_mean = d->bnb_mean; p.bnb_invstd = d->bnb_invstd;
        p.bnb_neg = d->bnb_act == RL_ACT_RELU ? 0.f : (d->bnb_act == RL_ACT_LRELU ? d->bnb_slope : 1.f);
        p.piv_mean = p.piv_bias = nullptr;
    }
    p.kslab = pl.reduce ? d->kslab : nullptr;
    *plan = pl;
    return RL_OK;
}

extern "C" int rl_gemm(const rl_gemm_desc* d, void* stream) {
    GemmParams p;
    GemmPlan pl;
    ConcatSrc cs;
    const int rc = gemm_fill(d, &p, &pl, &cs);
    return rc ? rc : launch_gemm(pl, (hipStream_t)stream, p, "rl_gemm", cs.split > 0 ? &cs : nullptr);
}

extern "C" int rl_gemm_concat_supported(const rl_gemm_desc* d) {
    GemmParams p;
    GemmPlan pl;
    ConcatSrc cs;
    return gemm_fill(d, &p, &pl, &cs);
}

extern "C" int rl_gemm_streams(const rl_gemm_desc* d) {
    if (!d) return 0;
    const bool vec4p = (d->lda % 4 == 0) && ((d->K + 3) / 4 * 4 <= d->lda) && (((uintptr_t)d->A & 15) == 0);
    const GemmFacts f{(long)d->B * d->n, d->N, d->K, d->a_mode == 0 && vec4p, false, false, false, d->addend || d->out2, false, false, 0, 0, 0};
    return (plan_gemm(f).kernel == GK_SGEMM && d->N <= 64) ? 1 : 0;
}

static bool gemm_pair_fits(const rl_gemm_desc* a, const rl_gemm_desc* b) {
    if (!a || !b) return false;
    if (a->A != b->A || a->lda != b->lda || a->a_bstride != b->a_bstride || a->a_mode != 0 || b->a_mode != 0) return false;
    if (a->B != b->B || a->n != b->n || a->K != b->K) return false;
    if (a->in_scale != b->in_scale || a->in_shift != b->in_shift || a->in_act != b->in_act || a->in_slope != b->in_slope) return false;
    if (!a->W_split || !b->W_split || wide_gemm_terms() == 0 || wgemm_staging() != 1) return false;
    if (a->K % PG_BK || a->K > W2_KMAX || a->N <= 0 || b->N <= 0) return false;
    if ((a->K <= 64 && a->N <= 64) || (b->K <= 64 && b->N <= 64)) return false;
    if (a->bias || b->bias || a->accumulate || b->accumulate || a->addend || b->addend || a->out2 || b->out2) return false;
    if ((a->stats == nullptr) != (b->stats == nullptr)) return false;
    if (a->ldy != a->N || b->ldy != b->N || a->y_bstride != a->n || b->y_bstride != b->n || !a->Y || !b->Y) return false;
    if ((((uintptr_t)a->A | (uintptr_t)(a->lda * 4) | (uintptr_t)a->W_split | (uintptr_t)b->W_split | (uintptr_t)a->Y | (uintptr_t)b->Y) & 15) != 0)
        return false;
    if (a->N % 4 || b->N % 4) return false;
    return true;
}
extern "C" int rl_gemm_pair_supported(const rl_gemm_desc* a, const rl_gemm_desc* b) { return gemm_pair_fits(a, b) ? 1 : 0; }
extern "C" int rl_gemm_pair(const rl_gemm_desc* a, const rl_gemm_desc* b, void* stream) {
// ... 17 lines not shown
    GemmPlan pl{};
    pl.kernel = GK_WGEMM2; pl.wide = WidePlan{128, 128, 1}; pl.threads = W2_THREADS; pl.ksplit = 1; pl.name = "wgemm2_kernel";
    pl.fn = wide_fn(p.stats != nullptr, true, pl.wide);
    persistent_grid(pl, p.a.M, p.pair_ny1 + rl_cdiv(b->N, 128), 1);
    return launch_gemm(pl, (hipStream_t)stream, p, "rl_gemm_pair");
}

extern "C" int rl_split_weights(const rl_wsplit_item* items, int count, void* stream) {
    RL_REQUIRE(items != nullptr && count >= 0, RL_ERR_ARGS, "rl_split_weights: bad arguments");
    hipStream_t st = (hipStream_t)stream;
    for (int base = 0; base < count; base += WS_MAX) {
        SplitBatch b;
        b.count = count - base < WS_MAX ? count - base : WS_MAX;
        long blocks = 0;
        for (int i = 0; i < b.count; ++i) {
            const rl_wsplit_item& it = items[base + i];
            RL_REQUIRE(it.W && it.out && it.K > 0 && it.N > 0, RL_ERR_ARGS, "rl_split_weights: bad item %d", base + i);
            RL_REQUIRE(((uintptr_t)it.out & 15) == 0, RL_ERR_ARGS, "rl_split_weights: item %d: out must be 16-byte aligned", base + i);
            RL_REQUIRE(it.K % 8 == 0 && (long)it.N * it.K < (1l << 31), RL_ERR_ARGS, "rl_split_weights: item %d: K %% 8 == 0, N * K < 2^31", base + i);
            b.item[i] = it;
            b.first_block[i] = (int)blocks;
            blocks += rl_cdiv((long)it.N * (it.K / 8), 256);
        }
        b.first_block[b.count] = (int)blocks;
        if (blocks > 0) hipLaunchKernelGGL(split_weights_kernel, dim3((unsigned)blocks), dim3(256), 0, st, b);
        RL_LAUNCH_CHECK("rl_split_weights");
    }
    rl_note_kernel("split_weights_kernel");
    return RL_OK;
}

extern "C" int64_t rl_gemm_stat_slots(int64_t M, int N, int K) {
    const GemmPlan pl = plan_gemm(aligned_facts(M, N, K, true));
    return rl_row_blocks_host(M, pl.kernel == GK_WGEMM2 ? pl.wide.bm : GM_BM);
}

extern "C" int64_t rl_gemm_kslab_floats(int64_t M, int N, int K) {
    const int ks = plan_gemm(aligned_facts(M, N, K, false)).wide.ksplit;
    return ks > 1 ? (int64_t)ks * M * N : 0;
}

extern "C" int64_t rl_wgrad_slab_floats(int64_t M, int N, int K) {
    return (int64_t)plan_wgrad(M, N, K, 0, true, false).nsplit * ((int64_t)N * K + N);
}

static int wgrad_fill(const rl_wgrad_desc* d, WgradParams* pp, WgradPlan* plan) {
    RL_REQUIRE(d != nullptr, RL_ERR_ARGS, "rl_wgrad: null descriptor");
    WgradParams& p = *pp;
    const int split = d->a2_split;
    RL_REQUIRE(split == 0 || (split > 0 && split < d->K && d->a_mode == 0), RL_ERR_ARGS,
               "rl_wgrad: a2_split must lie inside (0, K), on a tensor operand");
    int rc = fill_a(&p.a, "rl_wgrad", d->A, d->lda, d->a_bstride, d->a_mode, d->in_act, d->in_slope,
                    d->in_scale, d->in_shift, d->xyz, d->xyz_bstride, d->nbr_idx, d->nbr_d2, d->nbr_k,
                    d->B, d->n, split ? split : d->K);
    if (rc) return rc;
    p.a.K = d->K;
    p.cat = ConcatSrc{};
    if (split) {
        RL_REQUIRE(d->A2 && d->a2_idx && d->a2_bstride > 0 && (d->a2_scale == nullptr) == (d->a2_shift == nullptr), RL_ERR_ARGS,
                   "rl_wgrad: incomplete second source (A2, a2_idx, a2_bstride; a2_scale / a2_shift come together)");
        RL_REQUIRE((((uintptr_t)d->A2) & 15) == 0 && d->lda2 % 4 == 0 && d->lda2 >= d->K - split && d->lda2 < (1l << 31), RL_ERR_ARGS,
                   "rl_wgrad: A2 must be 16-byte aligned with lda2 a multiple of 4 and >= K - a2_split");
        RL_REQUIRE((int64_t)d->B * d->a2_bstride * d->lda2 < (1l << 31) && p.a.M < (1l << 30), RL_ERR_ARGS,
                   "rl_wgrad: a concat-gather operand needs a second source below 2^31 elements and fewer than 2^30 rows");
        p.cat.A2 = d->A2; p.cat.idx = d->a2_idx; p.cat.sc2 = d->a2_scale; p.cat.sh2 = d->a2_shift;
        p.cat.a2_bstride = d->a2_bstride; p.cat.lda2 = (int)d->lda2; p.cat.split = split; p.cat.act2 = d->a2_act; p.cat.slope2 = d->a2_slope;
    }
    RL_REQUIRE(d->N > 0 && d->dY && d->dW && d->slab && d->lddy >= d->N, RL_ERR_ARGS, "rl_wgrad: bad dY/dW/slab");
    p.N = d->N; p.dY = d->dY; p.lddy = d->lddy; p.dy_bstride = d->dy_bstride;
    p.rows_per_batch = (d->a_mode == 1) ? d->n * d->nbr_k : d->n;
    RL_REQUIRE(d->dy_bstride >= p.rows_per_batch, RL_ERR_ARGS, "rl_wgrad: dy_bstride smaller than rows per cloud");
    p.dy_contig = (d->dy_bstride == p.rows_per_batch);
    p.slab = d->slab; p.has_bias = d->dbias != nullptr;
    const WgradPlan pl = plan_wgrad(p.a.M, d->N, d->K, d->a_mode, pwgrad_ok(p), d->rows_bf16 != 0, split);
    RL_REQUIRE(pl.fn != nullptr, RL_ERR_UNSUPPORTED, "%s", pl.refusal);
    RL_REQUIRE(d->slab_floats >= (int64_t)pl.nsplit * ((int64_t)d->N * d->K + d->N), RL_ERR_ARGS,
               "rl_wgrad: slab too small (%ld floats)", (long)d->slab_floats);
    RL_REQUIRE(!d->rows_bf16 || (d->lda % 4 == 0 && d->lddy % 4 == 0), RL_ERR_ARGS,
               "rl_wgrad: bf16 rows need leading dimensions that are multiples of 4");
    p.rows_per_block = pl.rows_per_block;
    *plan = pl;
    return RL_OK;
}

extern "C" int rl_wgrad_batchable(const rl_wgrad_desc* d) {
    WgradParams p;
    WgradPlan pl;
    return wgrad_fill(d, &p, &pl) == RL_OK ? pl.batch : 0;
}

extern "C" int rl_wgrad_batch(const rl_wgrad_desc* descs, int count, void* stream) {
    RL_REQUIRE(descs != nullptr && count >= 0, RL_ERR_ARGS, "rl_wgrad_batch: bad arguments");
    hipStream_t st = (hipStream_t)stream;
    bool any[3] = {false, false, false};
    for (int kind = 1; kind <= 2; ++kind) {
        WgradBatch b;
        b.count = 0; b.pad = 0;
        for (int c = 0; c < WB_CAT_MAX; ++c) b.cat[c] = ConcatSrc{};
        int ncat = 0;
        long blocks = 0;
        auto flush = [&]() -> int {
            if (b.count == 0 || blocks == 0) { b.count = 0; blocks = 0; ncat = 0; return RL_OK; }
            launch_wgrad_batch(kind, blocks, st, b);
            RL_LAUNCH_CHECK("rl_wgrad_batch");
            b.count = 0; blocks = 0; ncat = 0;
            return RL_OK;
        };
        for (int i = 0; i < count; ++i) {
            const rl_wgrad_desc* d = descs + i;
            WgradParams p;
            WgradPlan pl;
            int rc = wgrad_fill(d, &p, &pl);
            if (rc) return rc;
            RL_REQUIRE(pl.batch != 0, RL_ERR_UNSUPPORTED,
                       "rl_wgrad_batch: layer %d (N = %d, K = %d) cannot join a grouped launch - check rl_wgrad_batchable first", i, d->N, d->K);
            RL_REQUIRE(d->defer_reduce, RL_ERR_ARGS, "rl_wgrad_batch: the layers' slabs are summed by rl_wgrad_reduce_batch (defer_reduce must be set)");
            if (pl.batch != kind) continue;
            any[kind] = true;
            if (p.cat.split > 0 && ncat == WB_CAT_MAX) {
                rc = flush();
                if (rc) return rc;
            }
            WBItem& it = b.item[b.count];
            it.A = p.a.A; it.dY = p.dY; it.sc = p.a.lazy.scale; it.sh = p.a.lazy.shift; it.slab = p.slab;
            it.lda = p.a.lda; it.a_bstride = p.a.a_bstride; it.lddy = p.lddy; it.dy_bstride = p.dy_bstride;
            it.rows_per_block = p.rows_per_block; it.M = p.a.M;
            it.N = p.N; it.K = p.a.K; it.n = p.a.n; it.rows_per_batch = p.rows_per_batch; it.act = p.a.lazy.act; it.slope = p.a.lazy.slope;
            it.nsplit = pl.nsplit;
            if (kind == 2) {
                it.gy = (unsigned short)pl.body; it.gz = 1;
                it.first_block = (int)blocks;
                blocks += pl.nsplit;
            } else {
                it.gy = (unsigned short)pl.grid.y; it.gz = (unsigned short)pl.grid.z;
                const int per = (int)it.gy * (int)it.gz;
                if (per > 1) blocks = (blocks + 7) / 8 * 8;
                it.first_block = (int)blocks;
                blocks += per > 1 ? (long)((pl.nsplit + 7) / 8 * 8) * per : (long)pl.nsplit;
            }
            it.a_contig = (unsigned char)p.a.contig; it.dy_contig = (unsigned char)p.dy_contig; it.has_bias = (unsigned char)p.has_bias;
            it.cat = 0;
            if (p.cat.split > 0) {
                b.cat[ncat] = p.cat;
                it.cat = (unsigned char)++ncat;
            }
            RL_REQUIRE(blocks < (1l << 30), RL_ERR_ARGS, "rl_wgrad_batch: too many workgroups");
            if (++b.count == WB_MAX) {
                rc = flush();
                if (rc) return rc;
            }
        }
        const int rc = flush();
        if (rc) return rc;
    }
    rl_note_kernel(any[2] && !any[1] ? "swgrad_batch_kernel" : "pwgrad128w_batch_kernel");
    return RL_OK;
}

extern "C" int rl_wgrad(const rl_wgrad_desc* d, void* stream) {
    WgradParams p;
    WgradPlan pl;
    int rc = wgrad_fill(d, &p, &pl);
    if (rc) return rc;
    hipStream_t st = (hipStream_t)stream;
    hipLaunchKernelGGL(pl.fn, pl.grid, dim3(pl.threads), 0, st, p);
    rl_note_kernel(pl.name);
    RL_LAUNCH_CHECK("rl_wgrad");
    if (d->defer_reduce) return RL_OK;
    const long per = (long)d->N * d->K + d->N;
    hipLaunchKernelGGL(wgrad_reduce_kernel, dim3(rl_cdiv(per, WR_E)), dim3(256), 0, st, d->slab, pl.nsplit,
                       d->N, d->K, d->dW, (long)d->w_ks, (long)d->w_ns, d->dbias);
// ... 41 lines not shown
```

### 3d_recognizer_amd/csrc/rows.hip

```cpp
#include <string.h>

#include "rl_common.h"

namespace {

struct RowsParams {
    const float* src;
    long lds, src_bstride;
    float* dst;
    long ldd;
    long rows, rows_per_batch;
    int C;
    const int32_t* i32;
    const int64_t* i64;
    int shared;
    int accumulate;
    RlLazy lazy;
};

template <typename I>
__device__ __forceinline__ long src_row(const RowsParams& p, I r) {
    const I b = r / (I)p.rows_per_batch;
    const I i = r - b * (I)p.rows_per_batch;
    long j = i;
// ... 521 lines not shown
    RL_REQUIRE(x && x->U && x->G && x->idx && x->n > 0 && x->h > 0 && x->g_bstride > 0, RL_ERR_ARGS, "%s: incomplete sources", who);
    RL_REQUIRE((x->u_scale == nullptr) == (x->u_shift == nullptr) && (x->g_scale == nullptr) == (x->g_shift == nullptr), RL_ERR_ARGS,
               "%s: scale / shift come together", who);
    RL_REQUIRE(x->ldu >= x->h && x->ldg >= x->h && (((uintptr_t)x->idx) & 3) == 0, RL_ERR_ARGS, "%s: bad leading dimensions", who);
    RL_REQUIRE(K == 16 && C == 2 * x->h && x->h % 64 == 0 && fits32(P * C) && P * 16 < (1l << 31), RL_ERR_UNSUPPORTED,
               "%s: the in-place X needs K == 16, C == 2 * h, h %% 64 == 0 and fewer than 2^32 elements", who);
    RlLazy lu{x->u_scale, x->u_shift, x->u_act, x->u_slope}, lg{x->g_scale, x->g_shift, x->g_act, x->g_slope};
    *q = AttCat{x->U, x->G, x->idx, x->u_scale, x->u_shift, x->g_scale, x->g_shift, (long)x->ldu, (long)x->ldg, (long)x->g_bstride,
                x->h, x->n, rl_eff_slope_host(lu), rl_eff_slope_host(lg)};
    return RL_OK;
}

extern "C" int rl_attpool_cat_supported(const rl_attpool_src* x, int64_t P, int K, int C) {
    AttCat q;
    return attcat_fill(x, P, K, C, &q, "rl_attpool_cat_supported");
}

extern "C" int rl_attpool_fwd_cat(const rl_attpool_src* x, const float* S, int64_t P, int K, int C, float* Pout, void* stream) {
    RL_REQUIRE(S && Pout && P >= 0 && C > 0, RL_ERR_ARGS, "rl_attpool_fwd_cat: bad arguments");
    AttCat q;
    const int rc = attcat_fill(x, P, K, C, &q, "rl_attpool_fwd_cat");
    if (rc) return rc;
    if (P == 0) return RL_OK;
    hipLaunchKernelGGL((attpool_fwd16_kernel<uint32_t, true>), dim3(grid_for(P * C)), dim3(256), 0, (hipStream_t)stream,
                       (const float*)nullptr, S, (long)P, C, Pout, q);
    rl_note_kernel("attpool_fwd_kernel");
    RL_LAUNCH_CHECK("rl_attpool_fwd_cat");
    return RL_OK;
}

extern "C" int rl_attpool_bwd_cat(const rl_attpool_src* x, const float* S, const float* Pout, const float* dP, int64_t P, int K,
                                  int C, float* dS, float* dXa, void* stream) {
    RL_REQUIRE(S && Pout && dP && dS && dXa && P >= 0 && C > 0, RL_ERR_ARGS, "rl_attpool_bwd_cat: bad arguments");
    AttCat q;
    const int rc = attcat_fill(x, P, K, C, &q, "rl_attpool_bwd_cat");
    if (rc) return rc;
    if (P == 0) return RL_OK;
    hipLaunchKernelGGL((attpool_bwd16_kernel<uint32_t, true>), dim3(grid_for(P * C)), dim3(256), 0, (hipStream_t)stream,
                       (const float*)nullptr, S, Pout, dP, (long)P, C, dS, dXa, q);
    rl_note_kernel("attpool_bwd_kernel");
    RL_LAUNCH_CHECK("rl_attpool_bwd_cat");
    return RL_OK;
}

static int g_pool256_x_in_place = 1;
extern "C" int rl_set_pool256_x(const char* mode) {
    const bool in_place = mode && !strcmp(mode, "in_place"), stored = mode && !strcmp(mode, "stored");
    RL_REQUIRE(in_place || stored, RL_ERR_ARGS, "rl_set_pool256_x: mode must be \"in_place\" or \"stored\"");
    g_pool256_x_in_place = in_place ? 1 : 0;
    return RL_OK;
}
extern "C" const char* rl_get_pool256_x(void) { return g_pool256_x_in_place ? "in_place" : "stored"; }

extern "C" int rl_add_act_fwd(const float* Y1, const float* s1, const float* b1, const float* Y2, const float* s2,
                              const float* b2, int64_t rows, int C, float slope, float* O, void* stream) {
    RL_REQUIRE(Y1 && s1 && b1 && Y2 && s2 && b2 && O && rows >= 0 && C > 0, RL_ERR_ARGS, "rl_add_act_fwd: bad arguments");
    if (rows == 0) return RL_OK;
    const bool vec = C % 4 == 0 && ((((uintptr_t)Y1) | ((uintptr_t)Y2) | ((uintptr_t)O) | ((uintptr_t)s1) | ((uintptr_t)b1) |
                                      ((uintptr_t)s2) | ((uintptr_t)b2)) & 15) == 0;
    if (vec) {
        const long quads = (long)rows * (C / 4);
        hipLaunchKernelGGL(add_act_fwd_vec_kernel, dim3(grid_for((quads + 1) / 2)), dim3(256), 0, (hipStream_t)stream, Y1, s1, b1, Y2,
                           s2, b2, quads, C, slope, O);
    } else if (fits32(rows * C))
        hipLaunchKernelGGL(add_act_fwd_kernel<uint32_t>, dim3(grid_for(rows * C)), dim3(256), 0, (hipStream_t)stream, Y1, s1, b1, Y2,
                           s2, b2, (long)rows * C, C, slope, O);
    else
        hipLaunchKernelGGL(add_act_fwd_kernel<int64_t>, dim3(grid_for(rows * C)), dim3(256), 0, (hipStream_t)stream, Y1, s1, b1, Y2,
                           s2, b2, (long)rows * C, C, slope, O);
    rl_note_kernel("add_act_fwd_kernel");
    RL_LAUNCH_CHECK("rl_add_act_fwd");
    return RL_OK;
}

extern "C" int rl_add_act_bwd(float* G, const float* O, int64_t rows, int C, float slope, void* stream) {
    RL_REQUIRE(G && O && rows >= 0 && C > 0, RL_ERR_ARGS, "rl_add_act_bwd: bad arguments");
    if (rows == 0) return RL_OK;
    hipLaunchKernelGGL(add_act_bwd_kernel, dim3(grid_for(rows * C)), dim3(256), 0, (hipStream_t)stream, G, O,
                       (long)rows * C, slope);
    rl_note_kernel("add_act_bwd_kernel");
    RL_LAUNCH_CHECK("rl_add_act_bwd");
    return RL_OK;
}

static int rpe_build_impl(const float* xyz, int64_t xyz_bstride, const int32_t* nbr_idx, const float* nbr_d2, int B,
                          int n, int k, float* out, int is_distance, void* stream) {
    RL_REQUIRE(xyz && nbr_idx && nbr_d2 && out && B > 0 && n > 0 && k > 0 && xyz_bstride >= n, RL_ERR_ARGS,
               "rl_rpe_build: bad arguments");
    RL_REQUIRE((((uintptr_t)out) & 15) == 0, RL_ERR_ARGS, "rl_rpe_build: out must be 16-byte aligned");
    const long rows = (long)B * n * k;
    RL_REQUIRE(rows < (1l << 31), RL_ERR_ARGS, "rl_rpe_build: too many rows");
    hipLaunchKernelGGL(rpe_build_kernel, dim3(grid_for(rows)), dim3(256), 0, (hipStream_t)stream, xyz, (long)xyz_bstride,
                       nbr_idx, nbr_d2, (unsigned)n, (unsigned)k, rows, out, is_distance);
    rl_note_kernel("rpe_build_kernel");
    RL_LAUNCH_CHECK("rl_rpe_build");
    return RL_OK;
}

extern "C" int rl_rpe_build(const float* xyz, int64_t xyz_bstride, const int32_t* nbr_idx, const float* nbr_d2, int B,
                            int n, int k, float* out, void* stream) {
    return rpe_build_impl(xyz, xyz_bstride, nbr_idx, nbr_d2, B, n, k, out, 0, stream);
}

extern "C" int rl_rpe_build_dist(const float* xyz, int64_t xyz_bstride, const int32_t* nbr_idx, const float* nbr_dist, int B,
                                 int n, int k, float* out, void* stream) {
    return rpe_build_impl(xyz, xyz_bstride, nbr_idx, nbr_dist, B, n, k, out, 1, stream);
// ... 98 lines not shown
```

### 3d_recognizer_amd/randlanet/_engine.py

```python
from dataclasses import dataclass, field
from typing import ClassVar, Dict, List, Optional

import torch

from . import _hip as H
from . import _ops as ops
from ._ops import Lazy, Rpe

BN_EPS = 1e-6
BN_MOMENTUM = 0.99
BN_PIVOT = True
BAND_SORT_MIN_POINTS = 4096
POOL_X_IN_PLACE_MIN_ROWS = 2048


@dataclass(slots=True, eq=False)
class _Record:
    kind: ClassVar[str] = ""
    level: int = field(default=-1, init=False)


@dataclass(slots=True, eq=False)
class LinearRec(_Record):
    kind: ClassVar[str] = "linear"
    a: object
    out: Lazy
    wname: str
    bname: Optional[str]
    ks: int
    ns: int
    a_grad: bool
    last_consumer_of_input: int


@dataclass(slots=True, eq=False)
class PoolRec(_Record):
    kind: ClassVar[str] = "pool"
    name: str
    u: Lazy
    g: Lazy
    csr: object
    X: object
    S: torch.Tensor
    pooled: Lazy
    n: int
    d: int


@dataclass(slots=True, eq=False)
class PoolFusedRec(_Record):
    kind: ClassVar[str] = "pool_fused"
    name: str
    u: object
    g: Lazy
    csr: object
    idx: torch.Tensor
    pooled: Lazy
    n: int
    d: int
    stage: int


@dataclass(slots=True, eq=False)
class AddActRec(_Record):
    kind: ClassVar[str] = "add_act"
    m2: Lazy
# ... 28 lines not shown
    seed: int
    first_row: int


@dataclass(slots=True, eq=False)
class DropoutRec(_Record):
    kind: ClassVar[str] = "dropout"
    src: Lazy
    dropped: Lazy
    mask: torch.Tensor
    scale: float


@dataclass(slots=True, eq=False)
class GradSlot:
    buf: torch.Tensor
    written: bool = False
    split: bool = False


class Context:

    def __init__(self):
        self.tape: List[_Record] = []
        self.keep: List[torch.Tensor] = []
        self.training = False
        self.B = self.N = 0
        self.perm: Optional[torch.Tensor] = None
        self.logits_perm: Optional[Lazy] = None
        self.wsplit = None
        self.xyz4: Optional[torch.Tensor] = None
        self.bn_defer: Optional[list] = None
        self.next_stats = (None, 1)
        self.eval_folds: Optional[dict] = None
        self.eval_sig: Optional[tuple] = None

    def record(self, rec: _Record) -> None:
        rec.level = ops.LEVEL
        self.tape.append(rec)


class _Backward:

    def __init__(self, ctx: Context, grads: Dict[str, torch.Tensor]):
        self.perm, self.wsplit = ctx.perm, ctx.wsplit
        self.grads = grads
        self.slots: Dict[object, GradSlot] = {}
        self.bn_pre = {}
        self.bn_done = set()
        self.fin_queue, self.rpe_after = [], []
        self.pending = []
        self.wbatch = []

    def slot(self, lz: Lazy) -> GradSlot:
        ent = self.slots.get(id(lz.raw))
        if ent is None:
            ent = self.slots[id(lz.raw)] = GradSlot(torch.empty_like(lz.raw))
        return ent

    def arrived(self, lz: Lazy) -> GradSlot:
        ent = self.slot(lz)
        assert ent.written
        return ent

    def put(self, lz: Lazy, buf: torch.Tensor, split: bool = False) -> None:
        self.slots[id(lz.raw)] = GradSlot(buf, True, split)

    def flush_rpe(self) -> None:
        if self.fin_queue:
            first = self.fin_queue.pop(0)
            ops._bn_bwd_finalize(*first, None, also=self.fin_queue)
        for fn in self.rpe_after:
            fn()
        self.rpe_after.clear()


class Prep:

    def __init__(self):
        self.B = self.N = 0
        self.training = False
        self.inp_p = self.xyz = self.xyz4 = None
        self.searches = self.csrs = None


class Engine:
    def __init__(self, layer_sizes, n_neighbors: int, decimation: int, n_classes: int, n_features: int,
                 params: Dict[str, torch.Tensor], buffers: Dict[str, torch.Tensor]):
        self.layers = list(layer_sizes)
        self.K = int(n_neighbors)
        self.dec = int(decimation)
        self.C = int(n_classes)
        self.F = int(n_features)
        self.P = params
        self.Bf = buffers
        self.Pv: Dict[str, torch.Tensor] = {k[:-len(".running_mean")]: torch.zeros_like(v) for k, v in buffers.items()
                                             if k.endswith(".running_mean")}
        self._eval_specs: Dict[tuple, dict] = {}
        self._eval_spec_build = {}
        self.sync: Optional[ops.SyncGroup] = None
        self._drop_seed = int(torch.initial_seed()) & 0x7FFFFFFFFFFFFFFF
        dev = next(iter(params.values())).device
        self._drop_counter: Optional[torch.Tensor] = torch.zeros(1, dtype=torch.int64, device=dev) if dev.type == "cuda" else None
        self.drop_stream = 0

    def _w2(self, name: str) -> torch.Tensor:
        w = self.P[name]
        return w.view(w.shape[0], w.shape[1])

    def _pivot(self, ctx: Context, bn_name: str):
        if not (ctx.training and BN_PIVOT):
            return None
        return self.Pv[bn_name]

    def reset_pivots(self) -> None:
        for t in self.Pv.values():
            t.zero_()

    def _fold(self, ctx: Context, bn_name: str, stats, rows: int, C: int, folded_bias=None, nslots=None):
# ... 65 lines not shown
        for Y, (wname, bname, bn, n_out, act, slope, ks, ns, stats), last in zip(res, metas, (first_is_last_consumer, 0)):
            out = Lazy(Y, a.B, a.n, a.n, n_out)
            self._bn(ctx, out, stats, bn, act, slope, folded_bias=self.P[bname],
                     nslots=H.row_blocks(out.rows, 128) if stats is not None else None)
            ctx.record(LinearRec(a, out, wname, bname, ks, ns, True, last))
            outs.append(out)
        return outs[0], outs[1]

    def _mlp(self, ctx, a, name: str, n_out: int, act: int = H.ACT_NONE, slope: float = 0.0, *, transposed=False,
             bn=True, a_grad=True, last_consumer_of_input: int = 0) -> Lazy:
        return self._linear(ctx, a, f"{name}.conv.weight", f"{name}.conv.bias", n_out, transposed=transposed,
                            bn=f"{name}.batch_norm" if bn else None, act=act, slope=slope, a_grad=a_grad,
                            last_consumer_of_input=last_consumer_of_input)

    def _pool(self, ctx, name: str, u, g: Lazy, idx: torch.Tensor, csr, n: int, d: int, n_out: int, stage: int = 0,
              next_stats: bool = False) -> Lazy:
        B, K, h = u.B, self.K, d // 2
        rows = B * n * K
        Ws = self.P[f"{name}.score_fn.0.weight"]
        if ops.pool_supported(d, K):
            if next_stats:
                res, st2, ns2 = ops.pool_fwd(u, g, idx, Ws, n, d, stage, next_stats=True)
                ctx.next_stats = (st2, ns2)
            else:
                res = ops.pool_fwd(u, g, idx, Ws, n, d, stage)
            pooled = ops.plain(res, B, n)
            ctx.record(PoolFusedRec(name, u, g, csr, idx, pooled, n, d, stage))
            return self._mlp(ctx, pooled, f"{name}.mlp", n_out, H.ACT_RELU)
        X = self._pool_x_in_place(ctx, u, g, idx, Ws, n, d)
        if X is None:
            X = torch.empty((rows, d), dtype=torch.float32, device=u.raw.device)
            ops.copy_rows_pair(((u.raw, (0, h), n * K, X, (0, h), rows, n * K), dict(lazy=u)),
                               ((g.raw, (0, h), g.bstride, X, (h, h), rows, n * K), dict(index=idx, lazy=g)))
            S = ops.gemm(ops.plain(X, B, n * K), Ws, 1, d, d, None, wsplit=ctx.wsplit)
        else:
            S = ops.gemm(X, Ws, 1, d, d, None, wsplit=ctx.wsplit)
        Pt = ops.attpool_fwd(X, S, B * n, K)
        pooled = ops.plain(Pt, B, n)
        ctx.record(PoolRec(name, u, g, csr, X, S, pooled, n, d))
        return self._mlp(ctx, pooled, f"{name}.mlp", n_out, H.ACT_RELU)

    def _pool_x_in_place(self, ctx, u, g: Lazy, idx: torch.Tensor, Ws: torch.Tensor, n: int, d: int):
        K = self.K
        if (ops.get_pool256_x() != "in_place" or not isinstance(u, Lazy) or u.rows <= POOL_X_IN_PLACE_MIN_ROWS
                or u.raw.dtype != torch.float32 or g.raw.dtype != torch.float32 or ops.row_dtype() != torch.float32 or u.bstride != u.n):
            return None
        x = ops.ConcatGather(u, g, idx)
        if not ops.attpool_concat_supported(x, u.B * n, K) or not ops.gemm_concat_supported(x, Ws, 1, d, d, ctx.wsplit):
            return None
        if ctx.training and not ops.wgrad_supported(x, Ws, n * K, d):
            return None
        return x

    def _virtual_bn(self, ctx: Context, vr, stage: int, bn_name: str, stats=None, nslots: int = 1) -> Lazy:
        if ctx.training and stats is None:
            stats, nslots = ops.rpe_stats(vr, stage)
        scale, shift, mean, invstd = self._fold(ctx, bn_name, stats, vr.rows, vr.h, None, nslots)
        rec = Lazy(vr.d2, vr.B, vr.n * 16, vr.n * 16, vr.h, scale, shift, H.ACT_RELU, 0.0, mean, invstd, bn_name)
        return rec

    def _lfa(self, ctx, l: int, xin: Lazy, xyz: torch.Tensor, n: int, d: int, idx, d2, csr=None) -> Lazy:
        e = f"encoder.{l}"
        B, K, h = xin.B, self.K, d // 2
        ctx.keep += [idx, d2]
        ctx.bn_defer = [] if self.sync is None else None
        f0, sc = self._mlp_pair(ctx, xin, (f"{e}.mlp1", h, H.ACT_LRELU, 0.2), (f"{e}.shortcut", 2 * d, H.ACT_NONE, 0.0),
                                first_is_last_consumer=2 if l == 0 else 0)
        if ops.virtual_rpe_supported(d, K, B * n, n):
            vr = ops.VirtualRpe(ctx.xyz4 if ctx.xyz4 is not None else xyz, idx, d2, B, n, h, self.P[f"{e}.mlp_rpe1.conv.weight"], self.P[f"{e}.mlp_rpe1.conv.bias"],
                                self.P[f"{e}.mlp_rpe2.conv.weight"], self.P[f"{e}.mlp_rpe2.conv.bias"])
            vr.piv1, vr.piv2 = self._pivot(ctx, f"{e}.mlp_rpe1.batch_norm"), self._pivot(ctx, f"{e}.mlp_rpe2.batch_norm")
            vr.bn1 = self._virtual_bn(ctx, vr, 1, f"{e}.mlp_rpe1.batch_norm")
            ops.bn_finalize_flush(ctx.bn_defer)
            q1 = self._pool(ctx, f"{e}.pool1", vr, f0, idx, csr, n, d, h, stage=1, next_stats=ctx.training)
            vr.bn2 = self._virtual_bn(ctx, vr, 2, f"{e}.mlp_rpe2.batch_norm", *ctx.next_stats)
            ctx.next_stats = (None, 1)
            ops.bn_finalize_flush(ctx.bn_defer)
            ctx.bn_defer = None
            q2 = self._pool(ctx, f"{e}.pool2", vr, q1, idx, csr, n, d, d, stage=2)
        else:
            rpe = Rpe(xyz, idx, d2, B, n, K)
            if h <= 128:
                rpe = ops.rpe_build(rpe)
            u1 = self._mlp(ctx, rpe, f"{e}.mlp_rpe1", h, H.ACT_RELU, a_grad=False)
            ops.bn_finalize_flush(ctx.bn_defer)
            q1 = self._pool(ctx, f"{e}.pool1", u1, f0, idx, csr, n, d, h)
            u2 = self._mlp(ctx, u1, f"{e}.mlp_rpe2", h, H.ACT_RELU)
            ops.bn_finalize_flush(ctx.bn_defer)
            ctx.bn_defer = None
            q2 = self._pool(ctx, f"{e}.pool2", u2, q1, idx, csr, n, d, d)
        m2 = self._mlp(ctx, q2, f"{e}.mlp2", 2 * d, last_consumer_of_input=1)
        O = ops.plain(ops.add_act_fwd(m2, sc, 0.01), B, n)
        ctx.record(AddActRec(m2, sc, O))
        return O

    def _wide_weight_uses(self, training: bool):
        uses = []
        for name, W in self.P.items():
            if not name.endswith(("conv.weight", "score_fn.0.weight")) or W.dim() < 2:
                continue
            a, b = int(W.shape[0]), int(W.shape[1])
            if max(a, b) <= 64:
                if name.endswith(".mlp1.conv.weight") and b % 32 == 0 and b > 64:
                    sc = self.P.get(name.replace(".mlp1.", ".shortcut."))
                    if sc is not None and int(sc.shape[0]) > 64:
                        uses.append((W.view(a, b), 1, b, b, a, True))
# ... 62 lines not shown
            self._drop_counter = torch.zeros(1, dtype=torch.int64, device=dev)
        return ops.dropout_tick(self._drop_counter), (self._drop_seed + 0x9E3779B97F4A7C15 * self.drop_stream) & 0x7FFFFFFFFFFFFFFF

    def forward(self, inp: torch.Tensor, perm: torch.Tensor, training: bool, dropout_p: float = 0.5,
                keep_mask: Optional[torch.Tensor] = None, logits_out: Optional[torch.Tensor] = None,
                prep: Optional["Prep"] = None, head: Optional[ops.Head] = None):
        B, N, cin = inp.shape
        assert cin == 3 + self.F and inp.dtype == torch.float32 and inp.is_cuda and inp.is_contiguous()
        assert perm.dtype == torch.int64 and perm.numel() == N and perm.is_cuda
        assert N >= self.min_points()
        dev = inp.device
        ctx = Context()
        ctx.training, ctx.B, ctx.N, ctx.perm = training, B, N, perm
        L, dec = len(self.layers), self.dec
        ctx.eval_sig = tuple(ops.virtual_rpe_supported(d, self.K, B * (N // dec ** l), N // dec ** l) for l, d in enumerate(self.layers))
        if not training:
            self._eval_spec_build = {}
            spec = self._eval_specs.get(ctx.eval_sig)
            if spec is not None and self.sync is None:
                ctx.eval_folds = self._eval_folds(spec)

        ctx.wsplit = ops.split_weights(self._wide_weight_uses(training))
        if prep is None:
            prep = self.prepare(inp, perm, training)
        perm = prep.perm
        ctx.perm = perm
        assert prep.B == B and prep.N == N and prep.training >= training
        inp_p, xyz, searches, csrs = prep.inp_p, prep.xyz, prep.searches, prep.csrs
        ctx.keep += [inp_p, xyz]
        if prep.xyz4 is not None:
            ctx.keep.append(prep.xyz4)
        ctx.xyz4 = prep.xyz4

        a0 = ops.plain(inp_p, B, N)
        if cin == 3 and prep.xyz4 is not None:
            a0 = Lazy(prep.xyz4.view(B * N, 4), B, N, N, 3)
        x = self._linear(ctx, a0, "fc_start.weight", "fc_start.bias", 8, bn="bn_start.0",
                         act=H.ACT_LRELU, slope=0.2, a_grad=False)
        skips: List[Lazy] = []
        ratio = 1
        for l, d in enumerate(self.layers):
            n_l = N // ratio
            with ops.level(l):
                x = self._lfa(ctx, l, x.prefix(n_l), xyz, n_l, d, *searches[l], csr=csrs[l])
            skips.append(x)
            ratio *= dec
        x = self._mlp(ctx, x.prefix(N // ratio), "mlp", x.C, H.ACT_RELU)
        for j in range(L):
            n_c, n_f = N // ratio, dec * N // ratio
            nn = searches[L + j][0]
            assert nn.shape == (B, n_f, 1)
            skip = skips.pop()
            assert skip.n == n_f and x.n == n_c
            cat = torch.empty((B * n_f, x.C + skip.C), dtype=torch.float32, device=dev)
            ops.copy_rows_pair(((x.raw, (0, x.C), x.bstride, cat, (0, x.C), B * n_f, n_f), dict(index=nn, lazy=x)),
                               ((skip.raw, (0, skip.C), skip.bstride, cat, (x.C, skip.C), B * n_f, n_f), {}))
            catl = ops.plain(cat, B, n_f)
            catl.concat = (x, skip)
            ctx.record(InterpConcatRec(x, skip, csrs[L + j], catl))
            n_out = 8 if j == L - 1 else 2 * self.layers[L - 2 - j]
            x = self._mlp(ctx, catl, f"decoder.{j}", n_out, H.ACT_RELU, transposed=True)
            ratio //= dec
        x = self._mlp(ctx, x, "fc_end.0", 64, H.ACT_RELU, last_consumer_of_input=1)
        x = self._mlp(ctx, x, "fc_end.1", 32, H.ACT_RELU, last_consumer_of_input=1)
        if (head is not None and training and self.sync is None and keep_mask is None
                and head.kind < ops.SORTED_KIND and ops.head_supported(x, self.C)):
            key, seed, first_row = None, 0, 0
            if dropout_p > 0.0:
                key, seed = self._dropout_key(dev)
            drop = (key, seed, dropout_p, first_row)
            ops.head_fwd(x, self._w2("fc_end.3.conv.weight"), self.P["fc_end.3.conv.bias"], perm, head, drop)
            ctx.record(HeadRec(x, head, drop))
            ctx.logits_perm = None
            return None, ctx
        if training and dropout_p > 0.0:
            if keep_mask is None:
                key, seed = self._dropout_key(dev)
                first_row = self.sync.cloud_offset * N if self.sync is not None else 0
                dropped = ops.plain(ops.dropout_fwd(x, key, seed, dropout_p, first_row), B, N)
                ctx.record(DropoutPhiloxRec(x, dropped, key, dropout_p, seed, first_row))
            else:
                t = torch.empty((B * N, 32), dtype=torch.float32, device=dev)
                ops.copy_rows(x.raw, (0, 32), N, t, (0, 32), B * N, N, lazy=x)
                ops.scale_mask(t, keep_mask, 1.0 / (1.0 - dropout_p))
                dropped = ops.plain(t, B, N)
                ctx.record(DropoutRec(x, dropped, keep_mask, 1.0 / (1.0 - dropout_p)))
            x = dropped
        lp = self._mlp(ctx, x, "fc_end.3", self.C, bn=False)
        ctx.logits_perm = lp
        if not training and ctx.eval_folds is None and self._eval_spec_build:
            self._eval_specs[ctx.eval_sig] = dict(self._eval_spec_build)
        logits = ops.logits_unpermute(lp.raw, perm, B, N, out=logits_out)
        return logits, ctx

    def backward(self, ctx: Context, dlogits: torch.Tensor, grads: Dict[str, torch.Tensor]) -> None:
        if not ctx.training:
            raise H.HipKernelError("backward is implemented for training-mode forwards (batch statistics)")
        B, N = ctx.B, ctx.N
        st = _Backward(ctx, grads)
        fused_head = bool(ctx.tape) and ctx.tape[-1].kind == "head"
        if not fused_head:
            assert dlogits.shape == (B, self.C, N) and dlogits.is_cuda
            dlogits = dlogits.contiguous().float()
            st.put(ctx.logits_perm, ops.logits_permute_grad(dlogits, ctx.perm))
        for rec in reversed(ctx.tape):
            with ops.level(rec.level):
                if rec.kind != "linear":
                    st.flush_rpe()
                self._BWD[rec.kind](self, st, rec)
        st.flush_rpe()
        ops.wgrad_batch_flush(st.wbatch)
        ops.wgrad_flush(st.pending)
        ctx.tape.clear()
        ctx.keep.clear()

    def _bwd_linear(self, st: _Backward, r: LinearRec):
        a, out, wname, bname, ks, ns, grads = r.a, r.out, r.wname, r.bname, r.ks, r.ns, st.grads
        s = st.slot(out)
        assert s.written, f"no gradient reached {wname}"
        G = s.buf
        if out.scale is not None and id(out.raw) not in st.bn_done:
            ops.bn_backward(G, out, grads[f"{out.bn}.weight"], grads[f"{out.bn}.bias"], True, sync=self.sync,
                            stats=st.bn_pre.pop(id(out.raw), None), also=st.fin_queue)
            st.flush_rpe()
        n_out = out.C
        ops.wgrad(a, G, out.bstride, n_out, grads[wname], ks, ns, grads[bname] if bname else None, pending=st.pending,
                  batch=st.wbatch)
        halves = getattr(a, "concat", None) if (r.a_grad and isinstance(a, Lazy)) else None
        if (halves is not None and (n_out > 64 or a.C > 64) and id(a.raw) not in st.slots
                and halves[1].bstride == halves[1].n and halves[1].raw.shape[0] == a.rows
                and halves[1].raw.shape[1] == halves[1].C and halves[0].C % 4 == 0
                and not st.slot(halves[1]).written):
            prev, skip = halves
            gs = st.slot(skip)
            Gp = torch.empty((a.rows, prev.C), dtype=torch.float32, device=G.device)
            gl = Lazy(G, out.B, out.n, out.bstride, n_out)
            ops.gemm(gl, self._w2(wname), ns, ks, a.C, None, out=Gp, out_bstride=a.bstride, out2=gs.buf, split_col=prev.C,
                     wsplit=st.wsplit)
            gs.written = True
            st.put(a, Gp, split=True)
            return
        if r.a_grad and isinstance(a, Lazy):
            ga = st.slot(a)
            if not ga.written:
                assert a.n == a.bstride and a.raw.shape[0] == a.B * a.n, "first writer must cover the tensor"
            gl = Lazy(G, out.B, out.n, out.bstride, n_out)
            if r.last_consumer_of_input:
                assert ga.written == (r.last_consumer_of_input == 2), wname
            complete = (bool(r.last_consumer_of_input) and self.sync is None and a.scale is not None and a.mean is not None
                        and a.rows == a.raw.shape[0])
            res = ops.gemm(gl, self._w2(wname), ns, ks, a.C, None, out=ga.buf, out_bstride=a.bstride, accumulate=ga.written,
                           wsplit=st.wsplit, bnb=a if complete else None)
            if complete and res[1] is not None:
                st.bn_pre[id(a.raw)] = res[1]
            ga.written = True

    def _bwd_pool_fused(self, st: _Backward, r: PoolFusedRec):
        if r.stage:
            return self._bwd_pool_virtual(st, r)
        u, g, n, d = r.u, r.g, r.n, r.d
        GP = st.arrived(r.pooled).buf
        gu, gg = st.slot(u), st.slot(g)
        DG = ops.pool_bwd(u, g, r.idx, self.P[f"{r.name}.score_fn.0.weight"], n, d, GP, gu.buf, gu.written,
                          st.grads[f"{r.name}.score_fn.0.weight"], pending=st.pending, batch=st.wbatch)
        gu.written = True
        ops.segment_sum_rows(DG, (0, d // 2), n * self.K, r.csr, gg.buf, g.bstride, accumulate=gg.written)
        gg.written = True

    def _bwd_add_act(self, st: _Backward, r: AddActRec):
        m2, sc, O, grads = r.m2, r.sc, r.O, st.grads
        G = st.arrived(O).buf
        if ops.resid_bn_supported(m2, sc):
            g2 = ops.resid_bn_backward(G, O.raw, 0.01, m2, sc, grads[f"{m2.bn}.weight"], grads[f"{m2.bn}.bias"],
                                       grads[f"{sc.bn}.weight"], grads[f"{sc.bn}.bias"], sync=self.sync)
            st.bn_done.update((id(m2.raw), id(sc.raw)))
        else:
            ops.add_act_bwd(G, O.raw, 0.01)
            g2 = torch.empty_like(G)
            ops.copy_rows(G, (0, O.C), O.n, g2, (0, O.C), O.rows, O.n)
        st.put(m2, G)
        st.put(sc, g2)

    def _bwd_interp_concat(self, st: _Backward, r: InterpConcatRec):
        prev, skip, catl = r.prev, r.skip, r.catl
        s = st.arrived(catl)
        gp = st.slot(prev)
        ops.segment_sum_rows(s.buf, (0, prev.C), catl.n, r.csr, gp.buf, prev.bstride, accumulate=gp.written)
        gp.written = True
        if not s.split:
            gs = st.slot(skip)
            ops.copy_rows(s.buf, (prev.C, skip.C), catl.n, gs.buf, (0, skip.C), catl.rows, catl.n, accumulate=gs.written)
            gs.written = True

# ... 78 lines not shown
```

### 3d_recognizer_amd/randlanet/_hip.py

```python
import ctypes as C
import os
from typing import Optional

import torch

_LIB: Optional[C.CDLL] = None
_LIB_PATH = os.path.join(os.path.dirname(os.path.dirname(os.path.abspath(__file__))), "csrc",
                         "librandla_hip.so")
_LIB_PATH = os.environ.get("RL_HIP_LIB", _LIB_PATH)

ABI_VERSION = 110
MAX_SLOTS = 1024
KNN_MAX_K = 64
ACT_NONE, ACT_RELU, ACT_LRELU = 0, 1, 2

ERR_ARGS, ERR_FEW_SUPPORT, ERR_LAUNCH, ERR_UNSUPPORTED = -1, -2, -3, -4


class HipKernelError(RuntimeError):
    pass


class GemmDesc(C.Structure):
    _fields_ = [
        ("A", C.c_void_p), ("lda", C.c_int64), ("a_bstride", C.c_int64),
        ("a_mode", C.c_int32), ("in_act", C.c_int32), ("in_slope", C.c_float),
        ("in_scale", C.c_void_p), ("in_shift", C.c_void_p),
        ("xyz", C.c_void_p), ("xyz_bstride", C.c_int64),
        ("nbr_idx", C.c_void_p), ("nbr_d2", C.c_void_p), ("nbr_k", C.c_int32),
        ("B", C.c_int32), ("n", C.c_int32), ("N", C.c_int32), ("K", C.c_int32),
        ("W", C.c_void_p), ("w_ks", C.c_int64), ("w_ns", C.c_int64),
        ("bias", C.c_void_p),
        ("Y", C.c_void_p), ("ldy", C.c_int64), ("y_bstride", C.c_int64),
        ("accumulate", C.c_int32),
        ("stats", C.c_void_p),
        ("kslab", C.c_void_p), ("kslab_floats", C.c_int64),
        ("addend", C.c_void_p), ("out2", C.c_void_p), ("out2_index", C.c_void_p), ("out2_bstride", C.c_int64),
        ("split_col", C.c_int32),
        ("W_split", C.c_void_p),
        ("stats_pivot_mean", C.c_void_p), ("stats_pivot_bias", C.c_void_p),
        ("bnb_Y", C.c_void_p), ("bnb_scale", C.c_void_p), ("bnb_shift", C.c_void_p), ("bnb_mean", C.c_void_p),
        ("bnb_invstd", C.c_void_p), ("bnb_act", C.c_int32), ("bnb_slope", C.c_float),
        ("a2_split", C.c_int32), ("a2_act", C.c_int32), ("A2", C.c_void_p), ("lda2", C.c_int64), ("a2_bstride", C.c_int64),
        ("a2_idx", C.c_void_p), ("a2_scale", C.c_void_p), ("a2_shift", C.c_void_p), ("a2_slope", C.c_float),
    ]


class AttpoolSrc(C.Structure):
    _fields_ = [
        ("U", C.c_void_p), ("ldu", C.c_int64), ("u_scale", C.c_void_p), ("u_shift", C.c_void_p), ("u_act", C.c_int32),
        ("u_slope", C.c_float),
        ("G", C.c_void_p), ("ldg", C.c_int64), ("g_bstride", C.c_int64), ("g_scale", C.c_void_p), ("g_shift", C.c_void_p),
        ("g_act", C.c_int32), ("g_slope", C.c_float),
        ("idx", C.c_void_p), ("n", C.c_int32), ("h", C.c_int32),
    ]


class WsplitItem(C.Structure):
    _fields_ = [("W", C.c_void_p), ("w_ks", C.c_int64), ("w_ns", C.c_int64), ("K", C.c_int32), ("N", C.c_int32),
                ("out", C.c_void_p)]


class WgradDesc(C.Structure):
    _fields_ = [
        ("A", C.c_void_p), ("lda", C.c_int64), ("a_bstride", C.c_int64),
        ("a_mode", C.c_int32), ("in_act", C.c_int32), ("in_slope", C.c_float),
        ("in_scale", C.c_void_p), ("in_shift", C.c_void_p),
        ("xyz", C.c_void_p), ("xyz_bstride", C.c_int64),
        ("nbr_idx", C.c_void_p), ("nbr_d2", C.c_void_p), ("nbr_k", C.c_int32),
        ("B", C.c_int32), ("n", C.c_int32), ("N", C.c_int32), ("K", C.c_int32),
        ("dY", C.c_void_p), ("lddy", C.c_int64), ("dy_bstride", C.c_int64),
        ("dW", C.c_void_p), ("w_ks", C.c_int64), ("w_ns", C.c_int64),
        ("dbias", C.c_void_p),
        ("slab", C.c_void_p), ("slab_floats", C.c_int64),
        ("defer_reduce", C.c_int32), ("rows_bf16", C.c_int32),
        ("a2_split", C.c_int32), ("a2_act", C.c_int32), ("A2", C.c_void_p), ("lda2", C.c_int64), ("a2_bstride", C.c_int64),
        ("a2_idx", C.c_void_p), ("a2_scale", C.c_void_p), ("a2_shift", C.c_void_p), ("a2_slope", C.c_float),
    ]


class WgradReduceItem(C.Structure):
    _fields_ = [
        ("slab", C.c_void_p), ("dW", C.c_void_p), ("dbias", C.c_void_p),
        ("w_ks", C.c_int64), ("w_ns", C.c_int64),
        ("nsplit", C.c_int32), ("N", C.c_int32), ("K", C.c_int32), ("reserved", C.c_int32),
    ]


class CloudJob(C.Structure):
    _fields_ = [
        ("xyz", C.c_void_p), ("features", C.c_void_p), ("labels", C.c_void_p), ("n_points", C.c_int64),
        ("xyz_f64", C.c_int32), ("normalization", C.c_int32), ("augment", C.c_int32), ("normal_col", C.c_int32),
        ("jitter_variance", C.c_double), ("jitter_limit", C.c_double), ("scale", C.c_double),
        ("R", C.c_double * 9), ("shift", C.c_double * 3),
    ]


class HeadDesc(C.Structure):
    _fields_ = [
        ("X", C.c_void_p), ("scale", C.c_void_p), ("shift", C.c_void_p), ("act", C.c_int32), ("slope", C.c_float),
        ("mean", C.c_void_p), ("invstd", C.c_void_p), ("W", C.c_void_p), ("bias", C.c_void_p),
        ("perm", C.c_void_p), ("labels", C.c_void_p), ("B", C.c_int32), ("N", C.c_int32), ("C", C.c_int32),
        ("loss_kind", C.c_int32), ("alpha", C.c_float), ("gamma", C.c_float), ("neglect_background", C.c_int32),
        ("drop_p", C.c_float), ("drop_key", C.c_void_p), ("drop_seed", C.c_uint64), ("drop_first_row", C.c_int64),
        ("work", C.c_void_p), ("G", C.c_void_p), ("bn_bwd_stats", C.c_void_p), ("slab", C.c_void_p),
        ("slab_floats", C.c_int64), ("grad_scale", C.c_float), ("reserved", C.c_int32), ("drop_mask", C.c_void_p), ("perm_bstride", C.c_int64),
        ("class_weight", C.c_void_p), ("masked", C.c_int32),
    ]


class BnBwdDesc(C.Structure):
    _fields_ = [
        ("G", C.c_void_p), ("Y", C.c_void_p), ("ld", C.c_int64), ("bstride", C.c_int64),
        ("B", C.c_int32), ("n", C.c_int32), ("C", C.c_int32), ("act", C.c_int32),
        ("slope", C.c_float),
        ("scale", C.c_void_p), ("shift", C.c_void_p), ("mean", C.c_void_p), ("invstd", C.c_void_p),
        ("stats", C.c_void_p), ("coef", C.c_void_p),
    ]


class KnnTask(C.Structure):
    _fields_ = [
        ("support", C.c_void_p), ("support_bstride", C.c_int64), ("query", C.c_void_p), ("query_bstride", C.c_int64),
        ("Ns", C.c_int32), ("Nq", C.c_int32), ("k", C.c_int32),
        ("idx_out", C.c_void_p), ("d2_out", C.c_void_p),
    ]


KNN_MAX_TASKS = 8

# ... 105 lines not shown
    "rl_get_wide_gemm": (C.c_char_p, []),
    "rl_set_wgemm_staging": (_i, [C.c_char_p]),
    "rl_set_wgemm_tile": (_i, [C.c_char_p]),
    "rl_set_gemm_ksplit": (_i, [_i]),
    "rl_set_sgemm_grid_div": (_i, [_i]),
    "rl_wgrad": (_i, [C.POINTER(WgradDesc), _vp]),
    "rl_wgrad_plan": (_i, [C.POINTER(WgradDesc), C.POINTER(C.c_int32), C.POINTER(C.c_int32), C.POINTER(C.c_char_p)]),
    "rl_wgrad_nsplit": (_i, [_l, _i, _i]),
    "rl_wgrad_batchable": (_i, [C.POINTER(WgradDesc)]),
    "rl_wgrad_batch": (_i, [C.POINTER(WgradDesc), _i, _vp]),
    "rl_wgrad_reduce_batch": (_i, [C.POINTER(WgradReduceItem), _i, _vp]),
    "rl_bn_finalize": (_i, [_vp, _i, _l, _i, _vp, _vp, _vp, _vp, _vp, _f, _f, _i, _vp, _vp, _vp, _vp, _vp, _i, _vp, _vp]),
    "rl_bn_finalize_batch": (_i, [C.POINTER(BnFinalizeItem), _i, _vp]),
    "rl_bn_bwd_finalize_batch": (_i, [C.POINTER(BnBwdFinalizeItem), _i, _vp]),
    "rl_head_supported": (_i, [_i, _i]),
    "rl_head_grid": (_i, [_l]),
    "rl_head_fwd": (_i, [C.POINTER(HeadDesc), _vp, _vp]),
    "rl_head_bwd": (_i, [C.POINTER(HeadDesc), _vp]),
    "rl_bn_bwd_finalize_pair": (_i, [_vp, _vp, _i, _l, _i, _vp, _vp, _vp, _vp, _vp, _vp, _vp]),
    "rl_bn_reduce_slots": (_i, [_vp, _i, _i, _vp, _vp]),
    "rl_bn_bwd_slots": (_i, [_l]),
    "rl_bn_bwd_reduce": (_i, [C.POINTER(BnBwdDesc), _vp]),
    "rl_bn_bwd_finalize": (_i, [_vp, _i, _l, _i, _vp, _vp, _vp, _vp]),
    "rl_bn_bwd_apply": (_i, [C.POINTER(BnBwdDesc), _vp]),
    "rl_bn_bwd_fused_supported": (_i, [_l, _i, _l]),
    "rl_bn_bwd_fused": (_i, [C.POINTER(BnBwdDesc), _l, _vp, _vp, _vp, _vp]),
    "rl_resid_bn_bwd_supported": (_i, [_l, _i]),
    "rl_resid_bn_bwd_reduce": (_i, [C.POINTER(ResidBnBwdDesc), _vp]),
    "rl_resid_bn_bwd_apply": (_i, [C.POINTER(ResidBnBwdDesc), _vp]),
    "rl_resid_bn_bwd_fused_supported": (_i, [_l, _i]),
    "rl_resid_bn_bwd_fused": (_i, [C.POINTER(ResidBnBwdDesc), _vp, _vp, _vp, _vp, _vp]),
    "rl_copy_rows": (_i, [C.POINTER(RowsDesc), _vp]),
    "rl_copy_rows_pair": (_i, [C.POINTER(RowsDesc), C.POINTER(RowsDesc), _vp]),
    "rl_scatter_add_rows": (_i, [C.POINTER(RowsDesc), _vp]),
    "rl_csr_workspace_bytes": (_l, [C.POINTER(CsrTask), _i, _i]),
    "rl_csr_build": (_i, [C.POINTER(CsrTask), _i, _i, _vp, _l, _vp]),
    "rl_segment_sum_rows": (_i, [C.POINTER(SegsumDesc), _vp]),
    "rl_pool_supported": (_i, [_i, _i]),
    "rl_pool_slab_floats": (_l, [_l, _i]),
    "rl_pool_bwd_slots": (_i, [_l, _i]),
    "rl_pool_bwd_grid": (_i, [_l, _i, _i]),
    "rl_pool_fwd_slots": (_i, [_l, _i]),
    "rl_pool_fwd": (_i, [C.POINTER(PoolDesc), _vp]),
    "rl_rpe_stats_slots": (_i, [_l]),
    "rl_rpe_stats": (_i, [C.POINTER(PoolDesc), _vp, _vp]),
    "rl_rpe_bn_reduce": (_i, [C.POINTER(PoolDesc), _vp, _vp, _vp]),
    "rl_rpe_wgrad_slab_floats": (_l, [_l, _i, _i]),
    "rl_rpe_wgrad": (_i, [C.POINTER(PoolDesc), _vp, _vp, _vp, _l, _vp, _vp]),
    "rl_pool_bwd": (_i, [C.POINTER(PoolDesc), _vp]),
    "rl_set_pool128_x": (_i, [C.c_char_p]),
    "rl_get_pool128_x": (C.c_char_p, []),
    "rl_set_pool256_x": (_i, [C.c_char_p]),
    "rl_get_pool256_x": (C.c_char_p, []),
    "rl_gemm_concat_supported": (_i, [C.POINTER(GemmDesc)]),
    "rl_attpool_cat_supported": (_i, [C.POINTER(AttpoolSrc), _l, _i, _i]),
    "rl_attpool_fwd_cat": (_i, [C.POINTER(AttpoolSrc), _vp, _l, _i, _i, _vp, _vp]),
    "rl_attpool_bwd_cat": (_i, [C.POINTER(AttpoolSrc), _vp, _vp, _vp, _l, _i, _i, _vp, _vp, _vp]),
    "rl_attpool_fwd": (_i, [_vp, _vp, _l, _i, _i, _vp, _vp]),
    "rl_attpool_bwd": (_i, [_vp, _vp, _vp, _vp, _l, _i, _i, _vp, _vp, _vp]),
    "rl_add_act_fwd": (_i, [_vp, _vp, _vp, _vp, _vp, _vp, _l, _i, _f, _vp, _vp]),
    "rl_add_act_bwd": (_i, [_vp, _vp, _l, _i, _f, _vp]),
    "rl_rpe_build": (_i, [_vp, _l, _vp, _vp, _i, _i, _i, _vp, _vp]),
    "rl_rpe_build_dist": (_i, [_vp, _l, _vp, _vp, _i, _i, _i, _vp, _vp]),
    "rl_batch_assemble": (_i, [_vp, _i, _i, _i, _vp, _vp, _vp, _vp, _vp, _vp]),
    "rl_batch_assemble_scratch_doubles": (_l, [_i, _i]),
    "rl_batch_assemble_flag_u32": (_l, [_i, _i, _i]),
    "rl_batch_draw": (_i, [_vp, _i, _i, C.c_uint64, _vp, _vp, _vp]),
    "rl_scale_mask": (_i, [_vp, _vp, _f, _l, _vp]),
    "rl_dropout_tick": (_i, [_vp, _vp, _vp]),
    "rl_dropout_fwd": (_i, [_vp, _vp, _vp, _i, _f, _vp, _l, _l, _i, _vp, C.c_uint64, _f, _vp]),
    "rl_dropout_bwd": (_i, [_vp, _l, _l, _i, _vp, C.c_uint64, _f, _vp]),
    "rl_upsample_cf": (_i, [_vp, _vp, _vp, _i, _i, _i, _i, _i, _i, _vp, _vp]),
    "rl_logits_unpermute": (_i, [_vp, _vp, _i, _i, _i, _vp, _vp]),
    "rl_logits_permute_grad": (_i, [_vp, _vp, _i, _i, _i, _vp, _vp]),
    "rl_logits_unpermute_b": (_i, [_vp, _vp, C.c_int64, _i, _i, _i, _vp, _vp]),
    "rl_logits_permute_grad_b": (_i, [_vp, _vp, C.c_int64, _i, _i, _i, _vp, _vp]),
    "rl_band_sort_workspace_bytes": (C.c_int64, [_i, _i, _vp, _i]),
    "rl_band_sort": (_i, [_vp, C.c_int64, _vp, _i, _i, _vp, _i, _vp, _vp, C.c_int64, _vp]),
    "rl_loss_max_classes": (_i, []),
    "rl_loss_work_doubles": (_l, [_l, _i]),
    "rl_loss_forward": (_i, [_vp, _vp, _i, _i, _i, _i, _f, _f, _i, _vp, _vp, _vp]),
    "rl_loss_backward": (_i, [_vp, _vp, _i, _i, _i, _i, _f, _f, _i, _vp, _f, _vp, _vp]),
    "rl_loss_forward_masked": (_i, [_vp, _vp, _i, _i, _i, _i, _f, _f, _i, _vp, _i, _vp, _vp, _vp]),
    "rl_loss_backward_masked": (_i, [_vp, _vp, _i, _i, _i, _i, _f, _f, _i, _vp, _f, _vp, _i, _vp, _vp]),
    "rl_loss_partials": (_i, [_vp, _vp, _i, _i, _i, _i, _f, _vp, _vp]),
    "rl_loss_totals_offset": (_l, [_i]),
    "rl_loss_from_totals": (_i, [_l, _i, _i, _f, _f, _i, _vp, _vp, _vp]),
    "rl_loss_backward_global": (_i, [_vp, _vp, _i, _i, _i, _i, _f, _f, _i, _vp, _f, _l, _vp, _vp]),
    "rl_lovasz_workspace_bytes": (_l, [_i, _i, _i]),
    "rl_lovasz_coef_offset": (_l, [_i, _i, _i]),
    "rl_lovasz_forward": (_i, [_vp, _vp, _i, _i, _i, _i, _vp, _vp, _l, _vp, _vp]),
    "rl_lovasz_backward": (_i, [_vp, _vp, _i, _i, _i, _i, _vp, _vp, _l, _f, _vp, _vp]),
    "rl_softmax_cf": (_i, [_vp, _i, _i, _i, _vp, _vp]),
    "rl_adam_step": (_i, [_vp, _vp, _vp, _vp, _l, _vp, _f, _f, _f, _f, _vp, _vp]),
    "rl_scene_workspace_bytes": (_l, [_l, _i]),
    "rl_scene_crop": (_i, [_vp, _l, _i, _vp, _i, _vp, _l, _vp, _vp, _l, _vp]),
    "rl_scene_accumulate": (_i, [_vp, _i, _i, _vp, _f, _f, _vp, _vp, _l, _vp]),
    "rl_scene_min_count": (_i, [_vp, _l, _vp, _vp, _vp]),
    "rl_scene_crop_padded": (_i, [_vp, _l, _i, _vp, _i, _vp, _l, _vp, _vp, _l, _vp]),
    "rl_scene_accumulate_first": (_i, [_vp, _i, _i, _vp, _f, _f, _vp, _vp, _l, _l, _i, _vp]),
    "rl_scenes_workspace_bytes": (_l, [_i, _l, _i]),
    "rl_scenes_init": (_i, [_vp, _i, _l, _vp, _vp, _l, _vp]),
    "rl_scenes_crop": (_i, [_vp, _i, _i, _l, _vp, _i, _i, _vp, _vp, _vp, _vp, _l, _vp]),
    "rl_scenes_crop_padded": (_i, [_vp, _i, _i, _l, _vp, _i, _i, _vp, _vp, _vp, _vp, _l, _vp]),
    "rl_scenes_vote_crop": (_i, [_vp, _i, _i, _l, _vp, _vp, _vp, _i, _i, _i, _i, _vp, _l, _l, _vp, _vp, _vp, _vp, _vp, _l, _vp]),
    "rl_scenes_vote_accumulate": (_i, [_vp, _i, _i, _l, _l, _i, _vp, _vp, _f, _f, _vp, _l, _vp]),
# ... 92 lines not shown
```

### 3d_recognizer_amd/randlanet/_ops.py

```python
import contextlib
import ctypes as C
import os
from dataclasses import dataclass
from typing import Optional, Tuple

import torch

from . import _hip as H

F32 = torch.float32
BF16 = torch.bfloat16

_STORAGE = os.environ.get("RL_STORAGE", "f32")


def set_storage(mode: str) -> None:
    global _STORAGE
    if mode not in ("f32", "bf16"):
        raise ValueError(f"storage must be 'f32' or 'bf16', got {mode!r}")
    if mode == "bf16" and get_wide_gemm() == "fp32":
        raise H.HipKernelError("bf16 storage needs the bf16x3 / bf16 arithmetic mode (RL_WIDE_GEMM)")
    _STORAGE = mode


# ... 179 lines not shown


@dataclass
class Rpe:
    xyz: torch.Tensor
    idx: torch.Tensor
    d2: torch.Tensor
    B: int
    n: int
    K: int

    @property
    def rows(self) -> int:
        return self.B * self.n * self.K


def set_wide_gemm(mode: str) -> None:
    H.check(H.lib().rl_set_wide_gemm(mode.encode()), "rl_set_wide_gemm")


def get_wide_gemm() -> str:
    return H.lib().rl_get_wide_gemm().decode()


def set_wgemm_staging(how: str) -> None:
    H.check(H.lib().rl_set_wgemm_staging(how.encode()), "rl_set_wgemm_staging")


def set_wgemm_tile(how: str) -> None:
    H.check(H.lib().rl_set_wgemm_tile(how.encode()), "rl_set_wgemm_tile")


def set_gemm_ksplit(enable: bool) -> None:
    H.check(H.lib().rl_set_gemm_ksplit(int(bool(enable))), "rl_set_gemm_ksplit")


def rpe_build(a: "Rpe", distances: bool = False) -> Lazy:
    _dev_check(a.xyz, a.idx, a.d2)
    assert a.idx.dtype == torch.int32 and a.idx.shape == (a.B, a.n, a.K) and a.d2.shape == a.idx.shape
    assert a.xyz.shape[0] == a.B and a.xyz.shape[1] >= a.n and a.xyz.shape[2] == 3
    out = torch.empty((a.rows, 12), dtype=F32, device=a.xyz.device)
    with _rec("rpe_build", (a.rows,), (48 + 8) * a.rows, 0):
        fn = H.lib().rl_rpe_build_dist if distances else H.lib().rl_rpe_build
        H.check(fn(a.xyz.data_ptr(), a.xyz.shape[1], a.idx.data_ptr(), a.d2.data_ptr(), a.B, a.n, a.K,
                   out.data_ptr(), _st()), "rl_rpe_build")
    return Lazy(out, a.B, a.n * a.K, a.n * a.K, 10)


@dataclass
class ConcatGather:
    u: Lazy
    g: Lazy
    idx: torch.Tensor

    @property
    def B(self) -> int:
        return self.u.B

    @property
    def n(self) -> int:
        return self.u.n

    @property
    def C(self) -> int:
        return self.u.C + self.g.C

    @property
    def rows(self) -> int:
        return self.u.rows


def set_pool128_x(mode: str) -> None:
    H.check(H.lib().rl_set_pool128_x(mode.encode()), "rl_set_pool128_x")


def get_pool128_x() -> str:
    return H.lib().rl_get_pool128_x().decode()


def set_pool256_x(mode: str) -> None:
    H.check(H.lib().rl_set_pool256_x(mode.encode()), "rl_set_pool256_x")


def get_pool256_x() -> str:
    return H.lib().rl_get_pool256_x().decode()


def _fill_a(d, a):
    if isinstance(a, ConcatGather):
        u, g, idx = a.u, a.g, a.idx
        _dev_check(g.raw, g.scale, g.shift, idx)
        assert idx.dtype == torch.int32 and idx.numel() == u.rows and u.bstride == u.n and g.B == u.B
        assert g.raw.dtype == F32 and g.raw.dim() == 2 and g.raw.shape[1] >= g.C
        assert g.raw.shape[0] >= (g.B - 1) * g.bstride + g.n, "second source rows out of range"
        M, _ = _fill_a(d, u)
        d.K = u.C + g.C
        d.a2_split, d.A2, d.lda2, d.a2_bstride, d.a2_idx = u.C, g.raw.data_ptr(), g.raw.shape[1], g.bstride, idx.data_ptr()
        if g.scale is not None:
            assert g.scale.numel() == g.C and g.shift.numel() == g.C
            d.a2_scale, d.a2_shift, d.a2_act, d.a2_slope = g.scale.data_ptr(), g.shift.data_ptr(), g.act, g.slope
        return M, u.C + g.C
    if isinstance(a, Rpe):
        _dev_check(a.xyz, a.idx, a.d2)
        assert a.idx.dtype == torch.int32 and a.idx.shape == (a.B, a.n, a.K) and a.d2.shape == a.idx.shape
        assert a.xyz.shape[0] == a.B and a.xyz.shape[1] >= a.n and a.xyz.shape[2] == 3
        d.a_mode = 1
        d.xyz, d.xyz_bstride = a.xyz.data_ptr(), a.xyz.shape[1]
        d.nbr_idx, d.nbr_d2, d.nbr_k = a.idx.data_ptr(), a.d2.data_ptr(), a.K
        d.B, d.n, d.K = a.B, a.n, 10
        return a.rows, 10
    _dev_check(a.raw, a.scale, a.shift)
    assert a.raw.dtype in (F32, BF16) and a.raw.dim() == 2 and a.raw.shape[1] >= a.C
    assert a.raw.shape[0] >= (a.B - 1) * a.bstride + a.n, "A operand rows out of range"
    d.a_mode = 0
    d.A, d.lda, d.a_bstride = a.raw.data_ptr(), a.raw.shape[1], a.bstride
    if a.scale is not None:
        assert a.scale.numel() == a.C and a.shift.numel() == a.C
        d.in_scale, d.in_shift, d.in_act, d.in_slope = a.scale.data_ptr(), a.shift.data_ptr(), a.act, a.slope
    d.B, d.n, d.K = a.B, a.n, a.C
    return a.rows, a.C


def weight_strides(W: torch.Tensor, transposed: bool, K: int, N: int) -> Tuple[int, int]:
    if transposed:
        assert W.shape[0] == K and W.shape[1] == N, (tuple(W.shape), K, N)
        return N, 1
    assert W.shape[0] == N and W.shape[1] == K, (tuple(W.shape), K, N)
    return 1, K




def split_weights(entries) -> dict:
    out_map = {}
    if get_wide_gemm() == "fp32" or not entries:
        return out_map
    entries = [e[:5] for e in entries if e[3] % 8 == 0 and (e[4] > 64 or e[3] > 64 or len(e) > 5)]
    if not entries:
        return out_map
    total = sum(2 * K * N + 8 for _, _, _, K, N in entries)
    buf = torch.empty(total, dtype=torch.bfloat16, device=entries[0][0].device)
    arr = (H.WsplitItem * len(entries))()
    off = 0
    for it, (W, ks, ns, K, N) in zip(arr, entries):
        _dev_check(W)
        assert W.dtype == F32 and W.numel() == K * N
        out = buf[off:off + 2 * K * N]
        it.W, it.w_ks, it.w_ns, it.K, it.N, it.out = W.data_ptr(), ks, ns, K, N, out.data_ptr()
        out_map[(W.data_ptr(), ks, ns, K, N)] = out
        off += (2 * K * N + 7) // 8 * 8
    with _rec("split_weights", (len(entries),), 6 * sum(K * N for _, _, _, K, N in entries), 0):
        H.check(H.lib().rl_split_weights(arr, len(entries), _st()), "rl_split_weights")
    return out_map


def gemm_stat_slots(M: int, N: int, K: int) -> int:
    return int(H.lib().rl_gemm_stat_slots(M, N, K))


def gemm(a, W: torch.Tensor, w_ks: int, w_ns: int, N: int, bias: Optional[torch.Tensor] = None, *,
         out: Optional[torch.Tensor] = None, out_bstride: Optional[int] = None,
         accumulate: bool = False, stats: Optional[torch.Tensor] = None,
         addend: Optional[torch.Tensor] = None, out2: Optional[torch.Tensor] = None,
         out2_index: Optional[torch.Tensor] = None, out2_bstride: int = 0, split_col: int = 0,
         wsplit: Optional[dict] = None, pivot: Optional[tuple] = None, bnb: Optional[Lazy] = None):
    d = H.GemmDesc()
    M, K = _fill_a(d, a)
    cat = isinstance(a, ConcatGather)
    assert isinstance(a, Rpe) or (a.u.raw if cat else a.raw).dtype == F32, "rl_gemm reads fp32 rows"
    rows_per_batch = a.n * a.K if isinstance(a, Rpe) else a.n
    _dev_check(W, bias, out, stats)
    assert W.dtype == F32 and W.numel() == K * N
    if out is None:
        out = torch.empty((M, N), dtype=F32, device=W.device)
        out_bstride = rows_per_batch
    else:
        assert out.dtype == F32 and out.dim() == 2 and out.shape[1] >= (split_col if out2 is not None else N)
        out_bstride = rows_per_batch if out_bstride is None else out_bstride
        assert out.shape[0] >= (d.B - 1) * out_bstride + rows_per_batch, "Y rows out of range"
    if bias is not None:
        assert bias.numel() == N
    if stats is not None:
        assert stats.dtype == torch.float64 and stats.numel() >= gemm_stat_slots(M, N, K) * 2 * N
    d.N, d.W, d.w_ks, d.w_ns, d.bias = N, W.data_ptr(), w_ks, w_ns, H.ptr(bias)
    planes = wsplit.get((W.data_ptr(), w_ks, w_ns, K, N)) if wsplit else None
    if planes is not None:
        d.W_split = planes.data_ptr()
    d.Y, d.ldy, d.y_bstride, d.accumulate = out.data_ptr(), out.shape[1], out_bstride, int(accumulate)
    d.stats = H.ptr(stats)
    if pivot is not None:
        assert stats is not None and pivot[0].numel() == N and (pivot[1] is None or pivot[1].numel() == N)
        _dev_check(*pivot)
        d.stats_pivot_mean, d.stats_pivot_bias = pivot[0].data_ptr(), H.ptr(pivot[1])
    if addend is not None or out2 is not None:
        _dev_check(addend, out2, out2_index)
        assert addend is None or (addend.dtype == F32 and addend.shape == (M, N))
        if out2 is not None:
            assert out2.dtype == F32 and 0 < split_col < N and out2.shape[1] == N - split_col
            if out2_index is None:
                assert out2.shape[0] >= M
            else:
                assert out2_index.dtype == torch.int32 and out2_index.numel() == M
                assert out2.shape[0] >= (d.B - 1) * out2_bstride + 1
        d.addend, d.out2, d.out2_index = H.ptr(addend), H.ptr(out2), H.ptr(out2_index)
        d.out2_bstride, d.split_col = out2_bstride, split_col
    bnb_pre = None
    if bnb is not None:
        if (stats is None and pivot is None and bnb.mean is not None and bnb.scale is not None and bnb.raw.dtype == F32
                and bnb.raw.shape[1] == out.shape[1] and bnb.bstride == out_bstride and bnb.C == N
                and 4 * M * N <= BNB_MAX_BYTES and H.lib().rl_gemm_streams(C.byref(d))):
            _dev_check(bnb.raw, bnb.scale, bnb.shift, bnb.mean, bnb.invstd)
            st_b = new_stats(W.device, N)
            d.stats = st_b.data_ptr()
            d.bnb_Y, d.bnb_scale, d.bnb_shift = bnb.raw.data_ptr(), bnb.scale.data_ptr(), bnb.shift.data_ptr()
            d.bnb_mean, d.bnb_invstd, d.bnb_act, d.bnb_slope = bnb.mean.data_ptr(), bnb.invstd.data_ptr(), bnb.act, bnb.slope
            bnb_pre = (st_b, gemm_stat_slots(M, N, K))
    kfloats = H.lib().rl_gemm_kslab_floats(M, N, K) if (N > 64 and not isinstance(a, Rpe) and not cat and out2 is None and addend is None) else 0
    if kfloats > 0:
        kslab = _slab(W.device, kfloats)
        d.kslab, d.kslab_floats = kslab.data_ptr(), kslab.numel()
    nbytes = 4 * (M * (K if not isinstance(a, Rpe) else 6) + M * N * (2 if accumulate else 1) + K * N)
    if cat:
        nbytes = 4 * (M * a.u.C + a.g.rows * a.g.C + M) + 4 * (M * N * (2 if accumulate else 1) + K * N)
    with _rec("gemm_rpe" if isinstance(a, Rpe) else "gemm", (M, K, N), nbytes, 2 * M * K * N):
        H.check(H.lib().rl_gemm(C.byref(d), _st()), "rl_gemm")
    return (out, bnb_pre) if bnb is not None else out


def gemm_concat_supported(a: ConcatGather, W: torch.Tensor, w_ks: int, w_ns: int, N: int, wsplit: Optional[dict]) -> bool:
    if a.u.raw.dtype != F32 or a.g.raw.dtype != F32:
        return False
    d = H.GemmDesc()
    M, K = _fill_a(d, a)
    d.N, d.W, d.w_ks, d.w_ns = N, W.data_ptr(), w_ks, w_ns
    planes = wsplit.get((W.data_ptr(), w_ks, w_ns, K, N)) if wsplit else None
    if planes is not None:
        d.W_split = planes.data_ptr()
    d.Y, d.ldy, d.y_bstride = W.data_ptr(), N, a.n
    rc = H.lib().rl_gemm_concat_supported(C.byref(d))
    if rc not in (0, H.ERR_UNSUPPORTED):
        H.check(rc, "rl_gemm_concat_supported")
    return rc == 0


BNB_MAX_BYTES = 32 << 20


def gemm_pair(a, first: tuple, second: tuple, wsplit: Optional[dict]):
    if not wsplit or isinstance(a, Rpe) or a.raw.dtype != F32:
        return None
    descs, outs = [], []
    M = K = None
    for (W, w_ks, w_ns, N, stats, pivot) in (first, second):
        d = H.GemmDesc()
        M, K = _fill_a(d, a)
        planes = wsplit.get((W.data_ptr(), w_ks, w_ns, K, N))
        if planes is None:
            return None
        _dev_check(W, stats)
        out = torch.empty((M, N), dtype=F32, device=W.device)
        d.N, d.W, d.w_ks, d.w_ns, d.W_split = N, W.data_ptr(), w_ks, w_ns, planes.data_ptr()
        d.Y, d.ldy, d.y_bstride = out.data_ptr(), N, a.n
        if stats is not None:
            assert stats.dtype == torch.float64 and stats.numel() >= H.row_blocks(M, 128) * 2 * N
            d.stats = stats.data_ptr()
            if pivot is not None:
                _dev_check(*pivot)
                d.stats_pivot_mean, d.stats_pivot_bias = pivot[0].data_ptr(), H.ptr(pivot[1])
        descs.append(d)
        outs.append(out)
    if not H.lib().rl_gemm_pair_supported(C.byref(descs[0]), C.byref(descs[1])):
        return None
    N1, N2 = first[3], second[3]
    with _rec("gemm", (M, K, N1 + N2), 4 * (M * K + M * (N1 + N2) + K * (N1 + N2)), 2 * M * K * (N1 + N2)):
        H.check(H.lib().rl_gemm_pair(C.byref(descs[0]), C.byref(descs[1]), _st()), "rl_gemm_pair")
    return outs[0], outs[1]


_SLAB = {}


def _slab(device, floats: int) -> torch.Tensor:
    key = (device, torch.cuda.current_stream(device).cuda_stream)
    buf = _SLAB.get(key)
    if buf is None or buf.numel() < floats:
        buf = torch.empty(max(floats, 1 << 20), dtype=F32, device=device)
        _SLAB[key] = buf
    return buf


WGRAD_BATCH_BYTES = 3 << 30


def wgrad(a, dY: torch.Tensor, dy_bstride: int, N: int, dW: torch.Tensor, w_ks: int, w_ns: int,
          dbias: Optional[torch.Tensor] = None, pending: Optional[list] = None, batch: Optional[list] = None) -> None:
    d = H.WgradDesc()
    M, K = _fill_a(d, a)
    rows_per_batch = a.n * a.K if isinstance(a, Rpe) else a.n
    _dev_check(dY, dW, dbias)
    rows_bf16 = dY.dtype == BF16
    assert dY.dtype in (F32, BF16) and dY.dim() == 2 and dY.shape[1] >= N
    adt = F32 if isinstance(a, Rpe) else a.u.raw.dtype if isinstance(a, ConcatGather) else a.raw.dtype
    assert isinstance(a, Rpe) or adt == dY.dtype, "A and dY must share their storage type"
    d.rows_bf16 = int(rows_bf16)
    assert dY.shape[0] >= (d.B - 1) * dy_bstride + rows_per_batch
    assert dW.numel() == K * N and (dbias is None or dbias.numel() == N)
    floats = H.lib().rl_wgrad_slab_floats(M, N, K)
    slab = _slab(dY.device, floats) if pending is None else torch.empty(floats, dtype=F32, device=dY.device)
    d.N, d.dY, d.lddy, d.dy_bstride = N, dY.data_ptr(), dY.shape[1], dy_bstride
    d.dW, d.w_ks, d.w_ns, d.dbias = dW.data_ptr(), w_ks, w_ns, H.ptr(dbias)
    d.slab, d.slab_floats = slab.data_ptr(), slab.numel()
    d.defer_reduce = 0 if pending is None else 1
    es = 2 if rows_bf16 else 4
    nbytes, flops = es * (M * (K if not isinstance(a, Rpe) else 6) + M * N) + 4 * K * N, 2 * M * K * N
    if isinstance(a, ConcatGather):
        nbytes = 4 * (M * a.u.C + a.g.rows * a.g.C + M) + 4 * M * N + 4 * K * N
    kind = H.lib().rl_wgrad_batchable(C.byref(d)) if (batch is not None and pending is not None) else 0
    if kind:
        batch.append((d, nbytes, flops, a, dY, slab, kind))
        if sum(b[1] for b in batch) > WGRAD_BATCH_BYTES:
            wgrad_batch_flush(batch)
    else:
        with _rec("wgrad_rpe" if isinstance(a, Rpe) else "wgrad", (M, K, N), nbytes, flops):
            H.check(H.lib().rl_wgrad(C.byref(d), _st()), "rl_wgrad")
    if pending is not None:
        it = H.WgradReduceItem()
        it.slab, it.dW, it.dbias, it.w_ks, it.w_ns = slab.data_ptr(), dW.data_ptr(), H.ptr(dbias), w_ks, w_ns
        it.nsplit, it.N, it.K = H.lib().rl_wgrad_nsplit(M, N, K), N, K
        pending.append((it, slab, dW, dbias))


def wgrad_supported(a, dY: torch.Tensor, dy_bstride: int, N: int) -> bool:
    d = H.WgradDesc()
    _fill_a(d, a)
    d.rows_bf16 = int(dY.dtype == BF16)
    d.N, d.dY, d.lddy, d.dy_bstride = N, dY.data_ptr(), dY.shape[1], dy_bstride
    d.dW = d.slab = dY.data_ptr()
    d.slab_floats, d.defer_reduce = 1 << 62, 1
    rc = H.lib().rl_wgrad_plan(C.byref(d), None, None, None)
    if rc not in (0, H.ERR_UNSUPPORTED):
        H.check(rc, "rl_wgrad_plan")
    return rc == 0


def wgrad_batch_flush(batch: list) -> None:
    for kind, name in ((1, "wgrad_batch"), (2, "swgrad_batch")):
        part = [b for b in batch if b[6] == kind]
        if not part:
            continue
        arr = (H.WgradDesc * len(part))(*[b[0] for b in part])
        with _rec(name, (len(part),), sum(b[1] for b in part), sum(b[2] for b in part)):
            H.check(H.lib().rl_wgrad_batch(arr, len(part), _st()), "rl_wgrad_batch")
    batch.clear()


def wgrad_flush(pending: list) -> None:
    if not pending:
        return
    arr = (H.WgradReduceItem * len(pending))(*[p[0] for p in pending])
    nbytes = sum(4 * p[1].numel() for p in pending)
    with _rec("wgrad_reduce_batch", (len(pending),), nbytes, 0):
        H.check(H.lib().rl_wgrad_reduce_batch(arr, len(pending), _st()), "rl_wgrad_reduce_batch")
    pending.clear()


def new_stats(device, C: int) -> torch.Tensor:
    return torch.empty((H.MAX_SLOTS, 2, C), dtype=torch.float64, device=device)

# ... 1397 lines not shown
```

### include/rl_randlanet.h

```cpp
#ifndef RL_RANDLANET_H
#define RL_RANDLANET_H

#include <stdint.h>

#ifdef __cplusplus
extern "C" {
#endif

#define RL_VERSION 110

#define RL_OK 0
#define RL_ERR_ARGS (-1)
#define RL_ERR_FEW_SUPPORT (-2)
#define RL_ERR_LAUNCH (-3)
#define RL_ERR_UNSUPPORTED (-4)

#define RL_MAX_SLOTS 1024
#define RL_KNN_MAX_K 64
#define RL_MAX_CLASSES 256

const char* rl_last_error(void);
const char* rl_last_kernel(void);
int rl_version(void);
int64_t rl_launch_count(void);
// ... 23 lines not shown
    float* d2_out;
} rl_knn_task;

int64_t rl_knn_multi_workspace_bytes(const rl_knn_task* tasks, int ntasks, int B);
int rl_knn_multi(const rl_knn_task* tasks, int ntasks, int B, void* workspace, int64_t workspace_bytes,
                 void* stream);

typedef struct rl_gemm_desc {
    const float* A;
    int64_t lda, a_bstride;
    int32_t a_mode;
    int32_t in_act;
    float in_slope;
    const float* in_scale;
    const float* in_shift;
    const float* xyz;
    int64_t xyz_bstride;
    const int32_t* nbr_idx;
    const float* nbr_d2;
    int32_t nbr_k;
    int32_t B, n, N, K;
    const float* W;
    int64_t w_ks, w_ns;
    const float* bias;
    float* Y;
    int64_t ldy, y_bstride;
    int32_t accumulate;
    double* stats;
    float* kslab;
    int64_t kslab_floats;
    const float* addend;
    float* out2;
    const int32_t* out2_index;
    int64_t out2_bstride;
    int32_t split_col;
    const void* W_split;
    const float* stats_pivot_mean;
    const float* stats_pivot_bias;
    const float* bnb_Y;
    const float* bnb_scale;
    const float* bnb_shift;
    const float* bnb_mean;
    const float* bnb_invstd;
    int32_t bnb_act;
    float bnb_slope;
    int32_t a2_split;
    int32_t a2_act;
    const float* A2;
    int64_t lda2, a2_bstride;
    const int32_t* a2_idx;
    const float* a2_scale;
    const float* a2_shift;
    float a2_slope;
} rl_gemm_desc;

int rl_gemm_streams(const rl_gemm_desc* d);
int rl_gemm_concat_supported(const rl_gemm_desc* d);
int rl_gemm_pair_supported(const rl_gemm_desc* a, const rl_gemm_desc* b);
int rl_gemm_pair(const rl_gemm_desc* a, const rl_gemm_desc* b, void* stream);

typedef struct rl_wsplit_item {
    const float* W;
    int64_t w_ks, w_ns;
    int32_t K, N;
    void* out;
} rl_wsplit_item;

int rl_split_weights(const rl_wsplit_item* items, int count, void* stream);

int64_t rl_gemm_kslab_floats(int64_t M, int N, int K);
int64_t rl_gemm_stat_slots(int64_t M, int N, int K);

int rl_set_wide_gemm(const char* mode);
const char* rl_get_wide_gemm(void);
int rl_set_wgemm_staging(const char* how);
int rl_set_wgemm_tile(const char* how);
int rl_set_gemm_ksplit(int enable);
int rl_set_sgemm_grid_div(int div);
int rl_gemm(const rl_gemm_desc* d, void* stream);

typedef struct rl_wgrad_desc {
    const float* A;
    int64_t lda, a_bstride;
    int32_t a_mode;
    int32_t in_act;
    float in_slope;
    const float* in_scale;
    const float* in_shift;
    const float* xyz;
    int64_t xyz_bstride;
    const int32_t* nbr_idx;
    const float* nbr_d2;
    int32_t nbr_k;
    int32_t B, n, N, K;
    const float* dY;
    int64_t lddy, dy_bstride;
    float* dW;
    int64_t w_ks, w_ns;
    float* dbias;
    float* slab;
    int64_t slab_floats;
    int32_t defer_reduce;
    int32_t rows_bf16;
    int32_t a2_split;
    int32_t a2_act;
    const float* A2;
    int64_t lda2, a2_bstride;
    const int32_t* a2_idx;
    const float* a2_scale;
    const float* a2_shift;
    float a2_slope;
} rl_wgrad_desc;

int64_t rl_wgrad_slab_floats(int64_t M, int N, int K);
int rl_wgrad(const rl_wgrad_desc* d, void* stream);
int rl_wgrad_plan(const rl_wgrad_desc* d, int32_t* grid_xyz, int32_t* threads, const char** kernel);

typedef struct rl_wgrad_reduce_item {
    const float* slab;
    float* dW;
    float* dbias;
    int64_t w_ks, w_ns;
    int32_t nsplit, N, K;
    int32_t reserved;
} rl_wgrad_reduce_item;

int rl_wgrad_nsplit(int64_t M, int N, int K);
int rl_wgrad_batchable(const rl_wgrad_desc* d);
int rl_wgrad_batch(const rl_wgrad_desc* descs, int count, void* stream);
int rl_wgrad_reduce_batch(const rl_wgrad_reduce_item* items, int count, void* stream);

int rl_bn_finalize(const double* stats, int nslots, int64_t count, int C, const float* gamma,
                   const float* beta, float* running_mean, float* running_var, int64_t* nbt,
                   float momentum, float eps, int training, float* scale, float* shift,
                   float* save_mean, float* save_invstd, const float* folded_bias, int pivoted, float* pivot, void* stream);

typedef struct rl_bn_finalize_item {
    const double* stats;
    int64_t count;
    const float* gamma;
    const float* beta;
    float* running_mean;
    float* running_var;
    int64_t* num_batches_tracked;
    float* scale;
    float* shift;
    float* save_mean;
    float* save_invstd;
    const float* folded_bias;
    int32_t nslots, C, training;
    float momentum, eps;
    int32_t pivoted;
    float* pivot;
} rl_bn_finalize_item;
int rl_bn_finalize_batch(const rl_bn_finalize_item* items, int count, void* stream);

typedef struct rl_bn_bwd_desc {
    float* G;
    const float* Y;
    int64_t ld, bstride;
    int32_t B, n, C;
    int32_t act;
    float slope;
    const float* scale;
// ... 69 lines not shown
    const int32_t* idx;
    int32_t n_src, k, n_dst;
    int32_t* offsets;
    int32_t* entries;
} rl_csr_task;

int64_t rl_csr_workspace_bytes(const rl_csr_task* tasks, int ntasks, int B);
int rl_csr_build(const rl_csr_task* tasks, int ntasks, int B, void* workspace, int64_t workspace_bytes,
                 void* stream);

typedef struct rl_segsum_desc {
    const float* src;
    int64_t lds, src_bstride;
    float* dst;
    int64_t ldd, dst_bstride;
    const int32_t* offsets;
    const int32_t* entries;
    int64_t entries_per_cloud;
    int32_t B, n_dst, C;
    int32_t accumulate;
    int32_t src_bf16;
} rl_segsum_desc;

int rl_segment_sum_rows(const rl_segsum_desc* d, void* stream);

int rl_attpool_fwd(const float* X, const float* S, int64_t P, int K, int C, float* Pout,
                   void* stream);
int rl_attpool_bwd(const float* X, const float* S, const float* Pout, const float* dP, int64_t P,
                   int K, int C, float* dS, float* dXa, void* stream);

typedef struct rl_attpool_src {
    const float* U;
    int64_t ldu;
    const float* u_scale;
    const float* u_shift;
    int32_t u_act;
    float u_slope;
    const float* G;
    int64_t ldg, g_bstride;
    const float* g_scale;
    const float* g_shift;
    int32_t g_act;
    float g_slope;
    const int32_t* idx;
    int32_t n;
    int32_t h;
} rl_attpool_src;
int rl_attpool_cat_supported(const rl_attpool_src* x, int64_t P, int K, int C);
int rl_attpool_fwd_cat(const rl_attpool_src* x, const float* S, int64_t P, int K, int C, float* Pout, void* stream);
int rl_attpool_bwd_cat(const rl_attpool_src* x, const float* S, const float* Pout, const float* dP, int64_t P, int K, int C,
                       float* dS, float* dXa, void* stream);
int rl_set_pool256_x(const char* mode);
const char* rl_get_pool256_x(void);

typedef struct rl_pool_desc {
    const float* U;
    const float* u_scale;
    const float* u_shift;
    int32_t u_act;
    float u_slope;
    const float* G;
    int64_t g_bstride;
    const float* g_scale;
    const float* g_shift;
    int32_t g_act;
    float g_slope;
    const int32_t* idx;
    const float* W;
    int64_t points;
    int32_t n, d, nbr_k;
    float* Pout;
    const float* dP;
    float* GU;
    int32_t gu_accumulate;
    float* DG;
    float* dW;
    float* slab;
    int64_t slab_floats;
    float* X_out;
    float* dS_out;
    int32_t u_source;
    const float* xyz;
    int64_t xyz_bstride;
    const float* nbr_d2;
    const float* W1;
    const float* b1;
    const float* scale1;
    const float* shift1;
    const float* W2;
    const float* b2;
    const float* scale2;
    const float* shift2;
    const float* mean1;
    const float* invstd1;
    const float* mean2;
    const float* invstd2;
    int32_t xyz_width;
    double* bn_bwd_stats;
    double* bn_fwd_stats2;
    int32_t rows_bf16;
    const float* pivot_mean1;
    const float* pivot_mean2;
    int32_t x_optional;
} rl_pool_desc;

int rl_pool_supported(int d, int nbr_k);
// ... 249 lines not shown
```

Baseline: 1303.

## Fuse decoder nearest-upsample concat into GEMM A-operand gather and add split epilogue

Adds an InterpConcat A-operand so decoder layers read the upsampled coarse features through a nearest-neighbour index gather plus the skip features directly inside the GEMM and wgrad kernels, with a 'first' flag that puts the gathered half first. The upsampled, concatenated tensor no longer has to be built in memory. It also lets the small streaming sgemm write a split-scatter epilogue so narrow GEMMs can write two outputs. Concat support is extended across the sgemm, swgrad and wide kernels, which adds template variants and per-row index loads. A new decoder_cat mode setter controls whether the path is used.

Measured after the change: 1316, median of 6. +1.0%, better.

```diff
diff --git a/3d_recognizer_amd/csrc/gemm.hip b/3d_recognizer_amd/csrc/gemm.hip
--- a/3d_recognizer_amd/csrc/gemm.hip
+++ b/3d_recognizer_amd/csrc/gemm.hip
@@ -101,6 +101,7 @@
     long a2_bstride;
     int lda2, split, act2;
     float slope2;
+    int first;
 };
 
 struct GemmParams {
@@ -461,8 +462,13 @@
 
 
 
-template <int KC, int NT, bool BNB = false>
-__global__ __launch_bounds__(256) void sgemm_kernel(const GemmParams p) {
+__device__ __forceinline__ const ConcatSrc* sgemm_cat_arg() { return nullptr; }
+__device__ __forceinline__ const ConcatSrc* sgemm_cat_arg(const ConcatSrc& c) { return &c; }
+template <int KC, int NT, bool BNB = false, bool SPL = false, class... Cat>
+__global__ __launch_bounds__(256) void sgemm_kernel(const GemmParams p, const Cat... cat) {
+    constexpr bool CAT = sizeof...(Cat) == 1;
+    static_assert(sizeof...(Cat) <= 1 && !(BNB && (CAT || SPL)) && !(CAT && SPL), "one variant at a time");
+    [[maybe_unused]] const ConcatSrc& cs = *sgemm_cat_arg(cat...);
     __shared__ double red[4][2][16 * NT];
     const int tid = threadIdx.x, lane = tid & 63, wave = __builtin_amdgcn_readfirstlane(tid >> 6);
     const int li = lane & 15, lj = lane >> 4;
@@ -476,8 +482,18 @@
 #pragma unroll
         for (int s = 0; s < 4; ++s) {
             const int k = 16 * c + 4 * lj + s;
+            if constexpr (CAT) {
+                static_assert(!CAT || KC % 2 == 0, "K == 2 * split == 16 * KC");
+                const bool two = (c >= KC / 2) != (cs.first != 0);
+                const float* scp = two ? cs.sc2 : p.a.lazy.scale;
+                const float* shp = two ? cs.sh2 : p.a.lazy.shift;
+                const int kc = c >= KC / 2 ? k - KC * 8 : k;
+                sc[c][s] = scp ? scp[kc] : 1.f;
+                sh[c][s] = scp ? shp[kc] : 0.f;
+            } else {
             sc[c][s] = (p.a.lazy.scale && k < K) ? p.a.lazy.scale[k] : 1.f;
             sh[c][s] = (p.a.lazy.scale && k < K) ? p.a.lazy.shift[k] : 0.f;
+            }
 #pragma unroll
             for (int nb = 0; nb < NT; ++nb) {
                 const int n = nb * 16 + li;
@@ -500,21 +516,52 @@
     const bool lazy = p.a.lazy.scale != nullptr;
     const float es = (!lazy || p.a.lazy.act == RL_ACT_NONE) ? 1.f : (p.a.lazy.act == RL_ACT_RELU ? 0.f : p.a.lazy.slope);
     const bool full = N == 16 * NT;
+    float e_one = 1.f, e_two = 1.f;
+    if constexpr (CAT) {
+        RlLazy t2 = p.a.lazy;
+        t2.scale = cs.sc2; t2.shift = cs.sh2; t2.act = cs.act2; t2.slope = cs.slope2;
+        e_one = rl_eff_slope(p.a.lazy);
+        e_two = rl_eff_slope(t2);
+    }
 
     const long nblk = (M + 15) >> 4;
     const long bstep = (long)gridDim.x * 4;
+    int gi = 0;
+    auto fetch_idx = [&](long blk) {
+        const long row = blk * 16 + li;
+        gi = cs.idx[row < M ? row : M - 1];
+    };
     auto fetch = [&](long blk, float4 (&a)[KC]) {
         const long row = blk * 16 + li;
         const bool rvalid = row < M;
         const long aoff = rvalid ? a_row_offset(p.a, row) : 0;
+        long goff = 0;
+        if constexpr (CAT) {
+            const int b = (int)((unsigned)(rvalid ? row : 0) / (unsigned)p.a.n);
+            goff = ((long)b * cs.a2_bstride + gi) * cs.lda2;
+        }
+        [[maybe_unused]] const float* plo = nullptr;
+        [[maybe_unused]] const float* phi = nullptr;
+        if constexpr (CAT) {
+            const float* pg = cs.A2 + goff + 4 * lj;
+            const float* pd = p.a.A + aoff + 4 * lj;
+            plo = cs.first ? pg : pd;
+            phi = cs.first ? pd : pg;
+        }
 #pragma unroll
         for (int c = 0; c < KC; ++c) {
             a[c] = make_float4(0.f, 0.f, 0.f, 0.f);
+            if constexpr (CAT) {
+                if (rvalid) a[c] = *reinterpret_cast<const float4*>(c < KC / 2 ? plo + 16 * c : phi + 16 * (c - KC / 2));
+            } else {
             if (rvalid && 16 * c + 4 * lj < K) a[c] = *reinterpret_cast<const float4*>(p.a.A + aoff + 16 * c + 4 * lj);
-        }
+            }
+        }
+        if constexpr (CAT) fetch_idx(blk + bstep);
     };
     float4 a[KC], an[KC];
     long blk = (long)blockIdx.x * 4 + wave;
+    if constexpr (CAT) if (blk < nblk) fetch_idx(blk);
     if (blk < nblk) fetch(blk, a);
     for (; blk < nblk; blk += bstep) {
         const bool rvalid = blk * 16 + li < M;
@@ -525,10 +572,16 @@
 #pragma unroll
         for (int c = 0; c < KC; ++c) {
             float av[4] = {a[c].x, a[c].y, a[c].z, a[c].w};
+            if constexpr (CAT) {
+                const float e = (c >= KC / 2) != (cs.first != 0) ? e_two : e_one;
+                const f32x4 x = rl_fold_act4((f32x4){a[c].x, a[c].y, a[c].z, a[c].w}, (f32x4){sc[c][0], sc[c][1], sc[c][2], sc[c][3]},
+                                             (f32x4){sh[c][0], sh[c][1], sh[c][2], sh[c][3]}, e);
+                av[0] = x[0]; av[1] = x[1]; av[2] = x[2]; av[3] = x[3];
+            }
 #pragma unroll
             for (int s = 0; s < 4; ++s) {
                 float v = av[s];
-                if (lazy) {
+                if (!CAT && lazy) {
                     const float z = v * sc[c][s] + sh[c][s];
                     v = fmaxf(z, z * es);
                 }
@@ -559,7 +612,8 @@
                 if (p.accumulate) {
                     float o[NT];
 #pragma unroll
-                    for (int nb = 0; nb < NT; ++nb) o[nb] = (full || nb * 16 + li < N) ? y[nb * 16] : 0.f;
+                    for (int nb = 0; nb < NT; ++nb)
+                        o[nb] = ((full || nb * 16 + li < N) && (!SPL || nb * 16 < p.split_col)) ? y[nb * 16] : 0.f;
 #pragma unroll
                     for (int nb = 0; nb < NT; ++nb) v[nb] += o[nb];
                 }
@@ -578,6 +632,15 @@
                             ssq[nb] += gp * ((t[nb] - bmu[nb]) * bis[nb]);
                         }
                     }
+                } else if constexpr (SPL) {
+                    float* y2 = p.out2 + R * (N - p.split_col) - p.split_col + li;
+#pragma unroll
+                    for (int nb = 0; nb < NT; ++nb) {
+                        if (full || nb * 16 + li < N) {
+                            if (nb * 16 >= p.split_col) y2[nb * 16] = acc[nb][r] + bias[nb];
+                            else y[nb * 16] = v[nb];
+                        }
+                    }
                 } else {
 #pragma unroll
                 for (int nb = 0; nb < NT; ++nb) {
@@ -619,7 +682,7 @@
 
 constexpr int SW_U = 4;
 
-template <int KT, int NT>
+template <int KT, int NT, bool CAT = false>
 __device__ __forceinline__ void swgrad_body(const WgradParams& p, const int bx, float* red) {
     const int tid = threadIdx.x, lane = tid & 63, wave = __builtin_amdgcn_readfirstlane(tid >> 6);
     const int lc = lane & 15, lr = lane >> 4;
@@ -632,11 +695,34 @@
 #pragma unroll
     for (int kb = 0; kb < KT; ++kb) {
         const int k = kb * 16 + lc;
+        if constexpr (CAT) {
+            static_assert(KT % 2 == 0, "K == 2 * split == 16 * KT");
+            const bool two = (kb >= KT / 2) != (p.cat.first != 0);
+            const float* scp = two ? p.cat.sc2 : a.lazy.scale;
+            const float* shp = two ? p.cat.sh2 : a.lazy.shift;
+            const int kc = kb >= KT / 2 ? k - KT * 8 : k;
+            sc[kb] = scp ? scp[kc] : 1.f;
+            sh[kb] = scp ? shp[kc] : 0.f;
+        } else {
         sc[kb] = (a.lazy.scale && k < K) ? a.lazy.scale[k] : 1.f;
         sh[kb] = (a.lazy.scale && k < K) ? a.lazy.shift[k] : 0.f;
+        }
     }
     const bool lazy = a.lazy.scale != nullptr;
     const float es = (!lazy || a.lazy.act == RL_ACT_NONE) ? 1.f : (a.lazy.act == RL_ACT_RELU ? 0.f : a.lazy.slope);
+    float e_one = 1.f, e_two = 1.f;
+    if constexpr (CAT) {
+        static_assert(SW_U == 4, "the fold takes the four row groups of a lane as one vector");
+        RlLazy t2 = a.lazy;
+        t2.scale = p.cat.sc2; t2.shift = p.cat.sh2; t2.act = p.cat.act2; t2.slope = p.cat.slope2;
+        e_one = rl_eff_slope(a.lazy);
+        e_two = rl_eff_slope(t2);
+    }
+    int gi[SW_U] = {0, 0, 0, 0};
+    auto fetch_idx = [&](long base) {
+#pragma unroll
+        for (int u = 0; u < SW_U; ++u) gi[u] = p.cat.idx[min(base + u * 4 + lr, r_end - 1)];
+    };
     f32x4 acc[NT][KT];
     float bsum[NT];
 #pragma unroll
@@ -686,6 +772,17 @@
                 av[u][0] = v;
 #pragma unroll
                 for (int kb = 1; kb < KT; ++kb) av[u][kb] = 0.f;
+            } else if constexpr (CAT) {
+                const long aoff = valid ? a_row_offset(a, R) : 0;
+                const int b = (int)((unsigned)(valid ? R : 0) / (unsigned)a.n);
+                const long goff = ((long)b * p.cat.a2_bstride + gi[u]) * p.cat.lda2;
+                const float* pg = p.cat.A2 + goff + lc;
+                const float* pd = a.A + aoff + lc;
+                const float* plo = p.cat.first ? pg : pd;
+                const float* phi = p.cat.first ? pd : pg;
+#pragma unroll
+                for (int kb = 0; kb < KT; ++kb)
+                    av[u][kb] = valid ? (kb < KT / 2 ? plo[kb * 16] : phi[(kb - KT / 2) * 16]) : 0.f;
             } else {
                 const long aoff = valid ? a_row_offset(a, R) : 0;
 #pragma unroll
@@ -695,8 +792,20 @@
                 }
             }
         }
+        if constexpr (CAT) fetch_idx(base + 16 * SW_U);
     };
     auto consume = [&](long base, float (&dy)[SW_U][NT], float (&av)[SW_U][KT]) {
+        if constexpr (CAT) {
+#pragma unroll
+            for (int kb = 0; kb < KT; ++kb) {
+                const float e = (kb >= KT / 2) != (p.cat.first != 0) ? e_two : e_one;
+                const f32x4 x = rl_fold_act4((f32x4){av[0][kb], av[1][kb], av[2][kb], av[3][kb]}, (f32x4){sc[kb], sc[kb], sc[kb], sc[kb]},
+                                             (f32x4){sh[kb], sh[kb], sh[kb], sh[kb]}, e);
+#pragma unroll
+                for (int u = 0; u < SW_U; ++u)
+                    if (base + u * 4 + lr < r_end) av[u][kb] = x[u];
+            }
+        } else
         if (a.a_mode != 1 && lazy) {
 #pragma unroll
             for (int u = 0; u < SW_U; ++u) {
@@ -722,6 +831,7 @@
     {
         float dy0[SW_U][NT], av0[SW_U][KT], dy1[SW_U][NT], av1[SW_U][KT];
         long base = r_begin + (long)wave * 4 * SW_U;
+        if constexpr (CAT) if (base < r_end) fetch_idx(base);
         if (base < r_end) fetch(base, dy0, av0);
         while (base < r_end) {
             const long nb1 = base + 16 * SW_U;
@@ -787,6 +897,11 @@
 __global__ __launch_bounds__(256) void swgrad_kernel(const WgradParams p) {
     __shared__ float red[KT * NT * 4 * 64 + NT * 64];
     swgrad_body<KT, NT>(p, (int)blockIdx.x, red);
+}
+template <int KT, int NT>
+__global__ __launch_bounds__(256) void swgrad_cat_kernel(const WgradParams p) {
+    __shared__ float red[KT * NT * 4 * 64 + NT * 64];
+    swgrad_body<KT, NT, true>(p, (int)blockIdx.x, red);
 }
 
 void swgrad_split(long M, int* nsplit, long* rows_per_block) {
@@ -1594,8 +1709,8 @@
     const unsigned lds0 = lds_address(lds);
     if (cat) {
         for (int k = tid; k < K; k += W2_THREADS) {
-            const bool two = k >= cs.split;
-            const int c = two ? k - cs.split : k;
+            const bool two = (k >= cs.split) != (cs.first != 0);
+            const int c = k >= cs.split ? k - cs.split : k;
             const float* scp = two ? cs.sc2 : p.a.lazy.scale;
             const float* shp = two ? cs.sh2 : p.a.lazy.shift;
             lsc[k] = scp ? scp[c] : 1.f;
@@ -1690,6 +1805,11 @@
                 asrc[i] = p.a.A + a_row_offset(p.a, R) + seg + k_begin;
                 const unsigned b = cat ? (unsigned)Rg / (unsigned)p.a.n : 0u;
                 asrc2[i] = cat ? cs.A2 + ((long)b * cs.a2_bstride + nidx[i]) * cs.lda2 + seg - cs.split : asrc[i];
+                if (cat && cs.first) {
+                    const float* gsrc = asrc2[i] + cs.split;
+                    asrc2[i] = asrc[i] - cs.split;
+                    asrc[i] = gsrc;
+                }
             }
         };
         int iq = 0, ic = 0;
@@ -1724,8 +1844,8 @@
         if (cat) {
             RlLazy t2 = p.a.lazy;
             t2.scale = cs.sc2; t2.shift = cs.sh2; t2.act = cs.act2; t2.slope = cs.slope2;
-            e_one = rl_eff_slope(p.a.lazy);
-            e_two = rl_eff_slope(t2);
+            e_one = rl_eff_slope(cs.first ? t2 : p.a.lazy);
+            e_two = rl_eff_slope(cs.first ? p.a.lazy : t2);
         }
         const int rb = wave % RB, cg = wave / RB;
         const int cg0 = cg * NT * 16;
@@ -2356,11 +2476,12 @@
         ucol[i] = (u & 7) * 16 + (lane & 3) * 4;
         urow[i] = (u >> 3) * 16 + (lane >> 2);
     }
-    const bool gat = cat && k0 + ucol[0] >= p.cat.split;
+    const bool gat = cat && (k0 + ucol[0] >= p.cat.split) != (p.cat.first != 0);
+    const int ks0 = cat && k0 + (__builtin_amdgcn_readfirstlane(wave) << 4) >= p.cat.split ? k0 - p.cat.split : k0;
     if (tid < PW2_T) {
         if (cat) {
-            const bool two = k0 + tid >= p.cat.split;
-            const int c = two ? k0 + tid - p.cat.split : k0 + tid;
+            const bool two = (k0 + tid >= p.cat.split) != (p.cat.first != 0);
+            const int c = k0 + tid >= p.cat.split ? k0 + tid - p.cat.split : k0 + tid;
             const float* scp = two ? p.cat.sc2 : p.a.lazy.scale;
             const float* shp = two ? p.cat.sh2 : p.a.lazy.shift;
             RlLazy t = p.a.lazy;
@@ -2422,9 +2543,9 @@
                         int b = cb;
                         for (int e = cend; (int)R >= e; e += p.a.n) ++b;
                         const unsigned off = ((unsigned)b * (unsigned)p.cat.a2_bstride + (unsigned)gi[i]) * (unsigned)p.cat.lda2 +
-                                             (unsigned)(k0 + ucol[i] - p.cat.split);
+                                             (unsigned)(ks0 + ucol[i]);
                         ra[i] = *reinterpret_cast<const float4*>(p.cat.A2 + off);
-                    } else ra[i] = rl_ldx4<RB>(p.a.A, a_row_offset(p.a, R) + k0 + ucol[i]);
+                    } else ra[i] = rl_ldx4<RB>(p.a.A, a_row_offset(p.a, R) + ks0 + ucol[i]);
                 }
             }
         }
@@ -2544,7 +2665,7 @@
     unsigned char cat;
 };
 constexpr int WB_MAX = 24;
-constexpr int WB_CAT_MAX = 4;
+constexpr int WB_CAT_MAX = 8;
 struct WgradBatch {
     WBItem item[WB_MAX];
     ConcatSrc cat[WB_CAT_MAX];
@@ -2628,6 +2749,7 @@
     int64_t kslab_floats;
     int cat_split;
     int rows_per_cloud;
+    bool split_dense16;
 };
 
 struct GemmPlan {
@@ -2648,6 +2770,8 @@
     if constexpr (KC == 1 && !BNB) if (N > 64) return sgemm_kernel<1, 8>;
     return N <= 16 ? sgemm_kernel<KC, 1, BNB> : N <= 32 ? sgemm_kernel<KC, 2, BNB> : sgemm_kernel<KC, 4, BNB>;
 }
+template <int KC>
+GemmFn sgemm_split_fn(int N) { return N <= 32 ? (GemmFn)sgemm_kernel<KC, 2, false, true> : (GemmFn)sgemm_kernel<KC, 4, false, true>; }
 template <int NT>
 GemmFn pgemm_fn(int terms) { return terms == 0 ? pgemm_kernel<NT, 0> : terms == 1 ? pgemm_kernel<NT, 1> : pgemm_kernel<NT, 3>; }
 template <int TERMS, bool STATS>
@@ -2694,10 +2818,23 @@
 GemmPlan plan_gemm(const GemmFacts& f);
 GemmPlan plan_gemm_concat(GemmFacts f) {
     const int split = f.cat_split, n = f.rows_per_cloud;
+    const bool a_rows16 = f.streamable;
     f.cat_split = 0;
     f.streamable = true;
     GemmPlan pl = plan_gemm(f);
     if (pl.kernel == GK_NONE) return pl;
+    if (pl.kernel == GK_SGEMM) {
+        if (!(a_rows16 && !f.bnb && !f.split && f.K == 2 * split && split % 16 == 0 && f.N <= 16)) {
+            pl.kernel = GK_NONE;
+            pl.fn = nullptr;
+            pl.refusal = "rl_gemm: a concat-gather A operand (a2_split) on the streaming kernel (K, N <= 64) needs fp32 rows in 16-byte "
+                         "pieces, K == 2 * a2_split, a2_split % 16 == 0, N <= 16 and no split epilogue or BatchNorm-backward sums";
+            return pl;
+        }
+        pl.catfn = f.K <= 32 ? (GemmCatFn)sgemm_kernel<2, 1, false, false, ConcatSrc> : (GemmCatFn)sgemm_kernel<4, 1, false, false, ConcatSrc>;
+        pl.name = "sgemm_kernel<cat>";
+        return pl;
+    }
     if (!(pl.kernel == GK_WGEMM2 && pl.ksplit == 1 && pl.wide.ksplit == 1 && !pl.reduce && f.K == 2 * split && split % PG_BK == 0 &&
           f.K <= W2_KMAX && n % 16 == 0 && f.M % 16 == 0)) {
         pl.kernel = GK_NONE;
@@ -2719,9 +2856,13 @@
     pl.threads = 256; pl.ksplit = 1;
     pl.gx = rl_row_blocks_host(f.M, GM_BM);
     pl.ny = N > 64 ? rl_cdiv(N, 128) : 1;
-    if (f.split && K <= 64 && N <= 64) { pl.refusal = "rl_gemm: split-scatter epilogue needs K or N > 64"; return pl; }
-    if (f.split && !f.pgemm) { pl.refusal = "rl_gemm: split-scatter epilogue needs the LDS-tiled kernel (aligned operands, K % 4 == 0)"; return pl; }
-    const bool streams = !f.split && f.streamable && stream_ok(N, K);
+    const bool sspl = f.split && f.split_dense16 && f.streamable && K <= 64 && N <= 64 && N > 16;
+    if (f.split && !sspl && K <= 64 && N <= 64) {
+        pl.refusal = "rl_gemm: split-scatter epilogue needs K or N > 64 (K, N <= 64: a dense out2 alone, split_col % 16 == 0, plain fp32 rows)";
+        return pl;
+    }
+    if (f.split && !sspl && !f.pgemm) { pl.refusal = "rl_gemm: split-scatter epilogue needs the LDS-tiled kernel (aligned operands, K % 4 == 0)"; return pl; }
+    const bool streams = (!f.split || sspl) && f.streamable && stream_ok(N, K);
     if (!f.split && f.bnb && !(streams && N <= 64)) {
         pl.refusal = "rl_gemm: the BatchNorm-backward sums are a by-product of the streaming kernel only (K, N <= 64; ask rl_gemm_streams)";
         return pl;
@@ -2730,11 +2871,12 @@
         int sg = pl.gx;
         if ((long)K * N >= 2048) sg = sg > 512 ? 512 : (sg > 256 ? 256 : sg);
         if (g_sgemm_grid_div > 1) sg = sg / g_sgemm_grid_div > 0 ? sg / g_sgemm_grid_div : 1;
-        if (f.bnb) pl.fn = K <= 16 ? sgemm_fn<1, true>(N) : K <= 32 ? sgemm_fn<2, true>(N) : sgemm_fn<4, true>(N);
+        if (sspl)       pl.fn = K <= 16 ? sgemm_split_fn<1>(N) : K <= 32 ? sgemm_split_fn<2>(N) : sgemm_split_fn<4>(N);
+        else if (f.bnb) pl.fn = K <= 16 ? sgemm_fn<1, true>(N) : K <= 32 ? sgemm_fn<2, true>(N) : sgemm_fn<4, true>(N);
         else       pl.fn = K <= 16 ? sgemm_fn<1, false>(N) : K <= 32 ? sgemm_fn<2, false>(N) : sgemm_fn<4, false>(N);
         pl.kernel = GK_SGEMM;
         pl.grid = dim3(sg);
-        pl.name = "sgemm_kernel";
+        pl.name = sspl ? "sgemm_kernel<split>" : "sgemm_kernel";
         return pl;
     }
     if (f.pgemm) pl.wide = wide_plan(f.M, N, K, N > 64 && f.wgemm && f.wgemm2);
@@ -2808,12 +2950,17 @@
 WgradPlan plan_wgrad(long M, int N, int K, int a_mode, bool pwgrad, bool rows_bf16, int cat_split = 0) {
     if (cat_split != 0) {
         WgradPlan pl = plan_wgrad(M, N, K, a_mode, pwgrad, rows_bf16);
+        if (pl.fn && pl.batch == 2 && !rows_bf16 && K == 2 * cat_split && cat_split % 16 == 0 && N <= 16) {
+            pl.fn = K <= 32 ? swgrad_cat_kernel<2, 1> : swgrad_cat_kernel<4, 1>;
+            pl.name = "swgrad_kernel<cat>";
+            return pl;
+        }
         const bool w = pl.fn == (WgradFn)pwgrad128w_kernel<1> || pl.fn == (WgradFn)pwgrad128w_kernel<3>;
         if (!(w && !rows_bf16 && K == 2 * cat_split && cat_split % 16 == 0)) {
             pl.fn = nullptr;
             pl.batch = 0;
             pl.refusal = "rl_wgrad: a concat-gather A operand (a2_split) needs the wide (128 x 128 tile) kernel outside the fp32 "
-                         "arithmetic mode, fp32 rows, K == 2 * a2_split and a2_split % 16 == 0";
+                         "arithmetic mode - or the streaming kernel (K <= 64) with N <= 16 - fp32 rows, K == 2 * a2_split and a2_split % 16 == 0";
         }
         return pl;
     }
@@ -2897,17 +3044,18 @@
                "rl_gemm: a2_split must lie inside (0, K), on a tensor operand");
     int rc = fill_a(&p.a, "rl_gemm", d->A, d->lda, d->a_bstride, d->a_mode, d->in_act, d->in_slope,
                     d->in_scale, d->in_shift, d->xyz, d->xyz_bstride, d->nbr_idx, d->nbr_d2, d->nbr_k,
-                    d->B, d->n, cat ? cat : d->K);
+                    d->B, d->n, cat ? (d->a2_first ? d->K - cat : cat) : d->K);
     if (rc) return rc;
     p.a.K = d->K;
     if (cat) {
         RL_REQUIRE(d->A2 && d->a2_idx && d->a2_bstride > 0 && (d->a2_scale == nullptr) == (d->a2_shift == nullptr), RL_ERR_ARGS,
                    "rl_gemm: incomplete second source (A2, a2_idx, a2_bstride; a2_scale / a2_shift come together)");
-        RL_REQUIRE((((uintptr_t)d->A2) & 15) == 0 && d->lda2 % 4 == 0 && d->lda2 >= d->K - cat && d->lda2 < (1l << 31) &&
+        RL_REQUIRE((((uintptr_t)d->A2) & 15) == 0 && d->lda2 % 4 == 0 && d->lda2 >= (d->a2_first ? cat : d->K - cat) && d->lda2 < (1l << 31) &&
                    (((uintptr_t)d->a2_idx) & 3) == 0, RL_ERR_ARGS,
                    "rl_gemm: A2 must be 16-byte aligned with lda2 a multiple of 4 and >= K - a2_split");
         cs->A2 = d->A2; cs->idx = d->a2_idx; cs->sc2 = d->a2_scale; cs->sh2 = d->a2_shift;
         cs->a2_bstride = d->a2_bstride; cs->lda2 = (int)d->lda2; cs->split = cat; cs->act2 = d->a2_act; cs->slope2 = d->a2_slope;
+        cs->first = d->a2_first ? 1 : 0;
     }
     RL_REQUIRE(d->N > 0 && d->W && d->Y && d->ldy > 0, RL_ERR_ARGS, "rl_gemm: bad W/Y");
     p.N = d->N; p.W = d->W; p.w_ks = d->w_ks; p.w_ns = d->w_ns; p.bias = d->bias;
@@ -2934,7 +3082,8 @@
     }
     p.stat_slots = (int)rl_gemm_stat_slots(p.a.M, d->N, d->K);
     const GemmPlan pl = plan_gemm(GemmFacts{p.a.M, d->N, d->K, p.a.a_mode == 0 && p.a.vec4p, pgemm_ok(p), wgemm_ok(p), wgemm2_usable(p),
-                                            split, d->stats != nullptr, d->bnb_Y != nullptr, d->kslab ? d->kslab_floats : 0, cat, d->n});
+                                            split, d->stats != nullptr, d->bnb_Y != nullptr, d->kslab ? d->kslab_floats : 0, cat, d->n,
+                                            d->out2 && !d->out2_index && !d->addend && d->split_col % 16 == 0});
     RL_REQUIRE(pl.kernel != GK_NONE, RL_ERR_UNSUPPORTED, "%s", pl.refusal);
     if (!split && d->bnb_Y) {
         RL_REQUIRE(d->stats && d->bnb_scale && d->bnb_shift && d->bnb_mean && d->bnb_invstd && !d->stats_pivot_mean, RL_ERR_ARGS,
@@ -3058,19 +3207,20 @@
                "rl_wgrad: a2_split must lie inside (0, K), on a tensor operand");
     int rc = fill_a(&p.a, "rl_wgrad", d->A, d->lda, d->a_bstride, d->a_mode, d->in_act, d->in_slope,
                     d->in_scale, d->in_shift, d->xyz, d->xyz_bstride, d->nbr_idx, d->nbr_d2, d->nbr_k,
-                    d->B, d->n, split ? split : d->K);
+                    d->B, d->n, split ? (d->a2_first ? d->K - split : split) : d->K);
     if (rc) return rc;
     p.a.K = d->K;
     p.cat = ConcatSrc{};
     if (split) {
         RL_REQUIRE(d->A2 && d->a2_idx && d->a2_bstride > 0 && (d->a2_scale == nullptr) == (d->a2_shift == nullptr), RL_ERR_ARGS,
                    "rl_wgrad: incomplete second source (A2, a2_idx, a2_bstride; a2_scale / a2_shift come together)");
-        RL_REQUIRE((((uintptr_t)d->A2) & 15) == 0 && d->lda2 % 4 == 0 && d->lda2 >= d->K - split && d->lda2 < (1l << 31), RL_ERR_ARGS,
+        RL_REQUIRE((((uintptr_t)d->A2) & 15) == 0 && d->lda2 % 4 == 0 && d->lda2 >= (d->a2_first ? split : d->K - split) && d->lda2 < (1l << 31), RL_ERR_ARGS,
                    "rl_wgrad: A2 must be 16-byte aligned with lda2 a multiple of 4 and >= K - a2_split");
         RL_REQUIRE((int64_t)d->B * d->a2_bstride * d->lda2 < (1l << 31) && p.a.M < (1l << 30), RL_ERR_ARGS,
                    "rl_wgrad: a concat-gather operand needs a second source below 2^31 elements and fewer than 2^30 rows");
         p.cat.A2 = d->A2; p.cat.idx = d->a2_idx; p.cat.sc2 = d->a2_scale; p.cat.sh2 = d->a2_shift;
         p.cat.a2_bstride = d->a2_bstride; p.cat.lda2 = (int)d->lda2; p.cat.split = split; p.cat.act2 = d->a2_act; p.cat.slope2 = d->a2_slope;
+        p.cat.first = d->a2_first ? 1 : 0;
     }
     RL_REQUIRE(d->N > 0 && d->dY && d->dW && d->slab && d->lddy >= d->N, RL_ERR_ARGS, "rl_wgrad: bad dY/dW/slab");
     p.N = d->N; p.dY = d->dY; p.lddy = d->lddy; p.dy_bstride = d->dy_bstride;
@@ -3123,6 +3273,11 @@
             RL_REQUIRE(d->defer_reduce, RL_ERR_ARGS, "rl_wgrad_batch: the layers' slabs are summed by rl_wgrad_reduce_batch (defer_reduce must be set)");
             if (pl.batch != kind) continue;
             any[kind] = true;
+            if (kind == 2 && p.cat.split > 0) {
+                hipLaunchKernelGGL(pl.fn, pl.grid, dim3(pl.threads), 0, st, p);
+                RL_LAUNCH_CHECK("rl_wgrad_batch(concat-gather, streaming)");
+                continue;
+            }
             if (p.cat.split > 0 && ncat == WB_CAT_MAX) {
                 rc = flush();
                 if (rc) return rc;
diff --git a/3d_recognizer_amd/csrc/rows.hip b/3d_recognizer_amd/csrc/rows.hip
--- a/3d_recognizer_amd/csrc/rows.hip
+++ b/3d_recognizer_amd/csrc/rows.hip
@@ -597,6 +597,15 @@
 }
 extern "C" const char* rl_get_pool256_x(void) { return g_pool256_x_in_place ? "in_place" : "stored"; }
 
+static int g_decoder_cat_in_place = 1;
+extern "C" int rl_set_decoder_cat(const char* mode) {
+    const bool in_place = mode && !strcmp(mode, "in_place"), stored = mode && !strcmp(mode, "stored");
+    RL_REQUIRE(in_place || stored, RL_ERR_ARGS, "rl_set_decoder_cat: mode must be \"in_place\" or \"stored\"");
+    g_decoder_cat_in_place = in_place ? 1 : 0;
+    return RL_OK;
+}
+extern "C" const char* rl_get_decoder_cat(void) { return g_decoder_cat_in_place ? "in_place" : "stored"; }
+
 extern "C" int rl_add_act_fwd(const float* Y1, const float* s1, const float* b1, const float* Y2, const float* s2,
                               const float* b2, int64_t rows, int C, float slope, float* O, void* stream) {
     RL_REQUIRE(Y1 && s1 && b1 && Y2 && s2 && b2 && O && rows >= 0 && C > 0, RL_ERR_ARGS, "rl_add_act_fwd: bad arguments");
diff --git a/3d_recognizer_amd/randlanet/_engine.py b/3d_recognizer_amd/randlanet/_engine.py
--- a/3d_recognizer_amd/randlanet/_engine.py
+++ b/3d_recognizer_amd/randlanet/_engine.py
@@ -12,6 +12,7 @@
 BN_PIVOT = True
 BAND_SORT_MIN_POINTS = 4096
 POOL_X_IN_PLACE_MIN_ROWS = 2048
+DECODER_CAT_IN_PLACE_MIN_ROWS = 8192
 
 
 @dataclass(slots=True, eq=False)
@@ -146,8 +147,12 @@
         self.pending = []
         self.wbatch = []
 
+    @staticmethod
+    def _key(lz) -> int:
+        return id(getattr(lz, "raw", lz))
+
     def slot(self, lz: Lazy) -> GradSlot:
-        ent = self.slots.get(id(lz.raw))
+        ent = self.slots.get(self._key(lz))
         if ent is None:
             ent = self.slots[id(lz.raw)] = GradSlot(torch.empty_like(lz.raw))
         return ent
@@ -157,8 +162,8 @@
         assert ent.written
         return ent
 
-    def put(self, lz: Lazy, buf: torch.Tensor, split: bool = False) -> None:
-        self.slots[id(lz.raw)] = GradSlot(buf, True, split)
+    def put(self, lz, buf: torch.Tensor, split: bool = False) -> None:
+        self.slots[self._key(lz)] = GradSlot(buf, True, split)
 
     def flush_rpe(self) -> None:
         if self.fin_queue:
@@ -330,6 +335,20 @@
             return None
         return x
 
+    def _decoder_cat_in_place(self, ctx, x: Lazy, skip: Lazy, nn: torch.Tensor, name: str, n_out: int):
+        if (ops.get_decoder_cat() != "in_place" or skip.rows <= DECODER_CAT_IN_PLACE_MIN_ROWS
+                or x.raw.dtype != torch.float32 or skip.raw.dtype != torch.float32 or ops.row_dtype() != torch.float32
+                or skip.bstride != skip.n):
+            return None
+        cat = ops.InterpConcat(x, skip, nn)
+        W = self._w2(f"{name}.conv.weight")
+        ks, ns = ops.weight_strides(W, True, cat.C, n_out)
+        if not ops.gemm_concat_supported(cat, W, ks, ns, n_out, ctx.wsplit):
+            return None
+        if ctx.training and not ops.wgrad_supported(cat, W, skip.n, n_out):
+            return None
+        return cat
+
     def _virtual_bn(self, ctx: Context, vr, stage: int, bn_name: str, stats=None, nslots: int = 1) -> Lazy:
         if ctx.training and stats is None:
             stats, nslots = ops.rpe_stats(vr, stage)
@@ -498,13 +517,15 @@
             assert nn.shape == (B, n_f, 1)
             skip = skips.pop()
             assert skip.n == n_f and x.n == n_c
-            cat = torch.empty((B * n_f, x.C + skip.C), dtype=torch.float32, device=dev)
-            ops.copy_rows_pair(((x.raw, (0, x.C), x.bstride, cat, (0, x.C), B * n_f, n_f), dict(index=nn, lazy=x)),
-                               ((skip.raw, (0, skip.C), skip.bstride, cat, (x.C, skip.C), B * n_f, n_f), {}))
-            catl = ops.plain(cat, B, n_f)
-            catl.concat = (x, skip)
+            n_out = 8 if j == L - 1 else 2 * self.layers[L - 2 - j]
+            catl = self._decoder_cat_in_place(ctx, x, skip, nn, f"decoder.{j}", n_out)
+            if catl is None:
+                cat = torch.empty((B * n_f, x.C + skip.C), dtype=torch.float32, device=dev)
+                ops.copy_rows_pair(((x.raw, (0, x.C), x.bstride, cat, (0, x.C), B * n_f, n_f), dict(index=nn, lazy=x)),
+                                   ((skip.raw, (0, skip.C), skip.bstride, cat, (x.C, skip.C), B * n_f, n_f), {}))
+                catl = ops.plain(cat, B, n_f)
+                catl.concat = (x, skip)
             ctx.record(InterpConcatRec(x, skip, csrs[L + j], catl))
-            n_out = 8 if j == L - 1 else 2 * self.layers[L - 2 - j]
             x = self._mlp(ctx, catl, f"decoder.{j}", n_out, H.ACT_RELU, transposed=True)
             ratio //= dec
         x = self._mlp(ctx, x, "fc_end.0", 64, H.ACT_RELU, last_consumer_of_input=1)
@@ -572,19 +593,27 @@
         n_out = out.C
         ops.wgrad(a, G, out.bstride, n_out, grads[wname], ks, ns, grads[bname] if bname else None, pending=st.pending,
                   batch=st.wbatch)
-        halves = getattr(a, "concat", None) if (r.a_grad and isinstance(a, Lazy)) else None
-        if (halves is not None and (n_out > 64 or a.C > 64) and id(a.raw) not in st.slots
+        in_place = r.a_grad and isinstance(a, ops.InterpConcat)
+        halves = (a.x, a.skip) if in_place else getattr(a, "concat", None) if (r.a_grad and isinstance(a, Lazy)) else None
+        gl = Lazy(G, out.B, out.n, out.bstride, n_out)
+        if (halves is not None and st._key(a) not in st.slots
                 and halves[1].bstride == halves[1].n and halves[1].raw.shape[0] == a.rows
                 and halves[1].raw.shape[1] == halves[1].C and halves[0].C % 4 == 0
+                and ((n_out > 64 or a.C > 64) if not in_place
+                     else ops.gemm_split_supported(gl, self._w2(wname), ns, ks, a.C, halves[0].C, st.wsplit))
                 and not st.slot(halves[1]).written):
             prev, skip = halves
             gs = st.slot(skip)
             Gp = torch.empty((a.rows, prev.C), dtype=torch.float32, device=G.device)
-            gl = Lazy(G, out.B, out.n, out.bstride, n_out)
-            ops.gemm(gl, self._w2(wname), ns, ks, a.C, None, out=Gp, out_bstride=a.bstride, out2=gs.buf, split_col=prev.C,
-                     wsplit=st.wsplit)
+            ops.gemm(gl, self._w2(wname), ns, ks, a.C, None, out=Gp, out_bstride=a.n if in_place else a.bstride, out2=gs.buf,
+                     split_col=prev.C, wsplit=st.wsplit)
             gs.written = True
             st.put(a, Gp, split=True)
+            return
+        if in_place:
+            Ga = torch.empty((a.rows, a.C), dtype=torch.float32, device=G.device)
+            ops.gemm(gl, self._w2(wname), ns, ks, a.C, None, out=Ga, out_bstride=a.n, wsplit=st.wsplit)
+            st.put(a, Ga)
             return
         if r.a_grad and isinstance(a, Lazy):
             ga = st.slot(a)
diff --git a/3d_recognizer_amd/randlanet/_hip.py b/3d_recognizer_amd/randlanet/_hip.py
--- a/3d_recognizer_amd/randlanet/_hip.py
+++ b/3d_recognizer_amd/randlanet/_hip.py
@@ -43,6 +43,7 @@
         ("bnb_invstd", C.c_void_p), ("bnb_act", C.c_int32), ("bnb_slope", C.c_float),
         ("a2_split", C.c_int32), ("a2_act", C.c_int32), ("A2", C.c_void_p), ("lda2", C.c_int64), ("a2_bstride", C.c_int64),
         ("a2_idx", C.c_void_p), ("a2_scale", C.c_void_p), ("a2_shift", C.c_void_p), ("a2_slope", C.c_float),
+        ("a2_first", C.c_int32),
     ]
 
 
@@ -76,6 +77,7 @@
         ("defer_reduce", C.c_int32), ("rows_bf16", C.c_int32),
         ("a2_split", C.c_int32), ("a2_act", C.c_int32), ("A2", C.c_void_p), ("lda2", C.c_int64), ("a2_bstride", C.c_int64),
         ("a2_idx", C.c_void_p), ("a2_scale", C.c_void_p), ("a2_shift", C.c_void_p), ("a2_slope", C.c_float),
+        ("a2_first", C.c_int32),
     ]
 
 
@@ -287,6 +289,8 @@
     "rl_get_pool128_x": (C.c_char_p, []),
     "rl_set_pool256_x": (_i, [C.c_char_p]),
     "rl_get_pool256_x": (C.c_char_p, []),
+    "rl_set_decoder_cat": (_i, [C.c_char_p]),
+    "rl_get_decoder_cat": (C.c_char_p, []),
     "rl_gemm_concat_supported": (_i, [C.POINTER(GemmDesc)]),
     "rl_attpool_cat_supported": (_i, [C.POINTER(AttpoolSrc), _l, _i, _i]),
     "rl_attpool_fwd_cat": (_i, [C.POINTER(AttpoolSrc), _vp, _l, _i, _i, _vp, _vp]),
diff --git a/3d_recognizer_amd/randlanet/_ops.py b/3d_recognizer_amd/randlanet/_ops.py
--- a/3d_recognizer_amd/randlanet/_ops.py
+++ b/3d_recognizer_amd/randlanet/_ops.py
@@ -255,6 +255,7 @@
     u: Lazy
     g: Lazy
     idx: torch.Tensor
+    first = False
 
     @property
     def B(self) -> int:
@@ -273,6 +274,45 @@
         return self.u.rows
 
 
+@dataclass
+class InterpConcat:
+    x: Lazy
+    skip: Lazy
+    nn: torch.Tensor
+    first = True
+
+    @property
+    def u(self) -> Lazy:
+        return self.skip
+
+    @property
+    def g(self) -> Lazy:
+        return self.x
+
+    @property
+    def idx(self) -> torch.Tensor:
+        return self.nn
+
+    @property
+    def B(self) -> int:
+        return self.skip.B
+
+    @property
+    def n(self) -> int:
+        return self.skip.n
+
+    @property
+    def C(self) -> int:
+        return self.x.C + self.skip.C
+
+    @property
+    def rows(self) -> int:
+        return self.skip.rows
+
+
+_CONCAT = (ConcatGather, InterpConcat)
+
+
 def set_pool128_x(mode: str) -> None:
     H.check(H.lib().rl_set_pool128_x(mode.encode()), "rl_set_pool128_x")
 
@@ -289,8 +329,16 @@
     return H.lib().rl_get_pool256_x().decode()
 
 
+def set_decoder_cat(mode: str) -> None:
+    H.check(H.lib().rl_set_decoder_cat(mode.encode()), "rl_set_decoder_cat")
+
+
+def get_decoder_cat() -> str:
+    return H.lib().rl_get_decoder_cat().decode()
+
+
 def _fill_a(d, a):
-    if isinstance(a, ConcatGather):
+    if isinstance(a, _CONCAT):
         u, g, idx = a.u, a.g, a.idx
         _dev_check(g.raw, g.scale, g.shift, idx)
         assert idx.dtype == torch.int32 and idx.numel() == u.rows and u.bstride == u.n and g.B == u.B
@@ -299,6 +347,8 @@
         M, _ = _fill_a(d, u)
         d.K = u.C + g.C
         d.a2_split, d.A2, d.lda2, d.a2_bstride, d.a2_idx = u.C, g.raw.data_ptr(), g.raw.shape[1], g.bstride, idx.data_ptr()
+        if a.first:
+            d.a2_split, d.a2_first = g.C, 1
         if g.scale is not None:
             assert g.scale.numel() == g.C and g.shift.numel() == g.C
             d.a2_scale, d.a2_shift, d.a2_act, d.a2_slope = g.scale.data_ptr(), g.shift.data_ptr(), g.act, g.slope
@@ -369,7 +419,7 @@
          wsplit: Optional[dict] = None, pivot: Optional[tuple] = None, bnb: Optional[Lazy] = None):
     d = H.GemmDesc()
     M, K = _fill_a(d, a)
-    cat = isinstance(a, ConcatGather)
+    cat = isinstance(a, _CONCAT)
     assert isinstance(a, Rpe) or (a.u.raw if cat else a.raw).dtype == F32, "rl_gemm reads fp32 rows"
     rows_per_batch = a.n * a.K if isinstance(a, Rpe) else a.n
     _dev_check(W, bias, out, stats)
@@ -430,7 +480,7 @@
     return (out, bnb_pre) if bnb is not None else out
 
 
-def gemm_concat_supported(a: ConcatGather, W: torch.Tensor, w_ks: int, w_ns: int, N: int, wsplit: Optional[dict]) -> bool:
+def gemm_concat_supported(a, W: torch.Tensor, w_ks: int, w_ns: int, N: int, wsplit: Optional[dict]) -> bool:
     if a.u.raw.dtype != F32 or a.g.raw.dtype != F32:
         return False
     d = H.GemmDesc()
@@ -440,6 +490,23 @@
     if planes is not None:
         d.W_split = planes.data_ptr()
     d.Y, d.ldy, d.y_bstride = W.data_ptr(), N, a.n
+    rc = H.lib().rl_gemm_concat_supported(C.byref(d))
+    if rc not in (0, H.ERR_UNSUPPORTED):
+        H.check(rc, "rl_gemm_concat_supported")
+    return rc == 0
+
+
+def gemm_split_supported(a: Lazy, W: torch.Tensor, w_ks: int, w_ns: int, N: int, split_col: int, wsplit: Optional[dict]) -> bool:
+    if a.raw.dtype != F32:
+        return False
+    d = H.GemmDesc()
+    M, K = _fill_a(d, a)
+    d.N, d.W, d.w_ks, d.w_ns = N, W.data_ptr(), w_ks, w_ns
+    planes = wsplit.get((W.data_ptr(), w_ks, w_ns, K, N)) if wsplit else None
+    if planes is not None:
+        d.W_split = planes.data_ptr()
+    d.Y, d.ldy, d.y_bstride = W.data_ptr(), split_col, a.n
+    d.out2, d.split_col = W.data_ptr(), split_col
     rc = H.lib().rl_gemm_concat_supported(C.byref(d))
     if rc not in (0, H.ERR_UNSUPPORTED):
         H.check(rc, "rl_gemm_concat_supported")
@@ -503,7 +570,7 @@
     _dev_check(dY, dW, dbias)
     rows_bf16 = dY.dtype == BF16
     assert dY.dtype in (F32, BF16) and dY.dim() == 2 and dY.shape[1] >= N
-    adt = F32 if isinstance(a, Rpe) else a.u.raw.dtype if isinstance(a, ConcatGather) else a.raw.dtype
+    adt = F32 if isinstance(a, Rpe) else a.u.raw.dtype if isinstance(a, _CONCAT) else a.raw.dtype
     assert isinstance(a, Rpe) or adt == dY.dtype, "A and dY must share their storage type"
     d.rows_bf16 = int(rows_bf16)
     assert dY.shape[0] >= (d.B - 1) * dy_bstride + rows_per_batch
@@ -516,7 +583,7 @@
     d.defer_reduce = 0 if pending is None else 1
     es = 2 if rows_bf16 else 4
     nbytes, flops = es * (M * (K if not isinstance(a, Rpe) else 6) + M * N) + 4 * K * N, 2 * M * K * N
-    if isinstance(a, ConcatGather):
+    if isinstance(a, _CONCAT):
         nbytes = 4 * (M * a.u.C + a.g.rows * a.g.C + M) + 4 * M * N + 4 * K * N
     kind = H.lib().rl_wgrad_batchable(C.byref(d)) if (batch is not None and pending is not None) else 0
     if kind:
diff --git a/include/rl_randlanet.h b/include/rl_randlanet.h
--- a/include/rl_randlanet.h
+++ b/include/rl_randlanet.h
@@ -99,6 +99,7 @@
     const float* a2_scale;
     const float* a2_shift;
     float a2_slope;
+    int32_t a2_first;
 } rl_gemm_desc;
 
 int rl_gemm_streams(const rl_gemm_desc* d);
@@ -157,6 +158,7 @@
     const float* a2_scale;
     const float* a2_shift;
     float a2_slope;
+    int32_t a2_first;
 } rl_wgrad_desc;
 
 int64_t rl_wgrad_slab_floats(int64_t M, int N, int K);
@@ -332,6 +334,8 @@
                        float* dS, float* dXa, void* stream);
 int rl_set_pool256_x(const char* mode);
 const char* rl_get_pool256_x(void);
+int rl_set_decoder_cat(const char* mode);
+const char* rl_get_decoder_cat(void);
 
 typedef struct rl_pool_desc {
     const float* U;
```
